# SAP/nested-hashing-psi

Measured on AMD Instinct MI355X. Metric: server PIE ciphertexts/sec, higher is better.
Workload: dtype u64

## Files before the change

### nested_hashing_psi_amd/csrc/kernels.hpp

```cpp
#pragma once
#include <hip/hip_runtime.h>

#include <atomic>
#include <vector>

#include "params.hpp"

namespace piehip {

struct PerDeviceOnce {
    std::atomic<unsigned long long> done{0};
    bool first_on_current_device()
    {
        int dev = 0;
        if (hipGetDevice(&dev) != hipSuccess || dev < 0 || dev > 63) return true;
        const unsigned long long bit = 1ULL << dev;
        return (done.fetch_or(bit) & bit) == 0;
    }
};

enum class NttKernel { radix2, blocked32, blocked16 };
struct NttRoute {
    NttKernel kernel;
    u32 s0;
    u32 global_stages;
    bool extra() const { return kernel != NttKernel::radix2 && !global_stages; }
};

struct NttPlan {
    const u64 *tables;
    const u64 *twp;
    const u64 *twc = nullptr;
    const u64 *twc_fold = nullptr;
    const u64 *twk16 = nullptr;
    const DevConsts *dc;
    u32 N, logN;
    u32 num_cus;
    u32 max_slots = 0;
    bool lane_order = false;
    bool fold = false;
    NttKernel lane_kernel = NttKernel::radix2;
    u32 lane_logn = 0;
    u32 lane_T = 0;
    u32 lane_kp = 16;
    bool small_moduli = false;
    bool xq_reuse = false;
    bool x_direct = false;
    bool fused_tensor = false;
    bool digits_with_d01 = false;
    bool digit_lift_lane = false;
    bool digit_lift_std = false;
    u32 transform_cus() const
    {
        if (!max_slots) return num_cus;
        const u32 c = (max_slots + 1) / 2;
        return c < num_cus ? (c ? c : 1u) : num_cus;
    }
};
void ntt_plan_decide(NttPlan &pl, bool lazy_ok, bool small_moduli);
NttRoute ntt_route(const NttPlan &pl, bool inverse, bool sigma, bool folded);

void build_twc_table(const u64 *nat_pairs, u32 logN, u32 s0, std::vector<u64> &out);
void build_twk16_table(const u64 *nat_pairs, u32 s0, u32 slice_log, std::vector<u64> &out);
void ntt_sigma_inverse_map(u32 logN, u32 s0, std::vector<u32> &map);
void ntt16_sigma_inverse_map(u32 logN, u32 s0, std::vector<u32> &map);
struct NttExtra {
    u64 *copy_out = nullptr;
    u32 copy_K = 1, copy_L = 1, copy_M = 1;
    u32 skip_L = 0, skip_M = 0;
    bool lazy_out = false;
    bool folded = false;
    bool x_lane_in = false;
};
void launch_ntt(const NttPlan &pl, u64 *data, u32 nlimbs, u32 mod_base, u32 mod_count, bool inverse, hipStream_t st,
                bool sigma = false, bool folded = false, const NttExtra *ex = nullptr);
void launch_ntt_fast(const NttPlan &pl, const u64 *twc, u32 s0, u64 *data, u32 nlimbs, u32 mod_base, u32 mod_count, bool inverse,
                     bool sigma, hipStream_t st, const u64 *lift_src = nullptr, u32 lift_L = 0, const NttExtra *ex = nullptr);
struct Ntt16Digits {
    const u64 *d2;
    size_t stride2;
    u64 *dig;
    u32 nb, L;
};
void launch_ntt16(const NttPlan &pl, u64 *data, u32 nlimbs, u32 mod_base, u32 mod_count, bool inverse, bool sigma, hipStream_t st,
                  const NttExtra *ex, const Ntt16Digits *dg = nullptr);
#ifndef PIEHIP_FUSE_TENSOR
#define PIEHIP_FUSE_TENSOR 1
#endif
void launch_ntt16_tensor(const NttPlan &pl, const u64 *e, u64 *d, u32 nb, u32 M, hipStream_t st);
void launch_ntt_digits(const NttPlan &pl, const u64 *d2, u64 *dig, u32 nb, u32 L, bool sigma, hipStream_t st);

struct StageAXOut {
    u64 *out = nullptr;
    u32 M = 0, logns = 0;
};
void launch_stage_a(const DevConsts *dc, u32 N, u32 L, u32 K, u32 b, u32 E, const u64 *idx, const u64 *minus,
                    const u64 *db, u64 *acc, hipStream_t st, bool small_moduli, u32 bstride = 0, u32 h0 = 0, u32 hn = 0, u32 nq = 1,
                    u32 q = 0, const StageAXOut *xo = nullptr);
static const u32 STAGE_A_MAX_QUERIES = 8;
struct StageAQueries {
    const u64 *idx[STAGE_A_MAX_QUERIES];
    const u64 *minus[STAGE_A_MAX_QUERIES];
};
void launch_stage_a_batch(const DevConsts *dc, u32 N, u32 L, u32 K, u32 b, u32 E, const StageAQueries &qs, u32 nq, const u64 *db,
                          u64 *acc, hipStream_t st, bool small_moduli, u32 bstride = 0, u32 h0 = 0, u32 hn = 0,
                          const StageAXOut *xo = nullptr);

void launch_expand_q_to_qp(const DevConsts *dc, u32 N, u32 L, const u64 *in, size_t in_stride_outer,
                           size_t in_stride_inner, u32 n_outer, u64 *out, u32 out_polys, u32 out_slot, hipStream_t st,
                           bool small_moduli, bool fold = false, bool skip_q = false);
void launch_scale_pq_expand(const DevConsts *dc, u32 N, u32 L, const u64 *in, size_t in_stride_outer,
                            size_t in_stride_inner, u32 n_outer, u64 *out, u32 out_polys, u32 out_slot, hipStream_t st,
                            bool small_moduli, bool fold = false);
void launch_expand_both(const DevConsts *dc, u32 N, u32 L, const u64 *x, size_t sx, const u64 *y, size_t sy, size_t si, u32 n_outer,
                        u64 *out, hipStream_t st, bool small_moduli, bool fold = false, bool skip_q = false);
void launch_tensor(const DevConsts *dc, u32 N, u32 M, const u64 *e, u64 *d, u32 nb, hipStream_t st, bool small_moduli);
void launch_scale_round(const DevConsts *dc, u32 N, u32 L, const u64 *d, u32 nb, u64 *out01, size_t stride01, u64 *out2,
                        size_t stride2, hipStream_t st, bool small_moduli, bool fold = false, bool fold_comp2 = false);
void launch_digits(const DevConsts *dc, u32 N, u32 L, const u64 *d2, size_t stride2, u32 nb, u64 *dig, hipStream_t st,
                   bool fold = false);
void launch_relin_mac(const DevConsts *dc, u32 N, u32 L, const u64 *d01, size_t stride01, const u64 *dig, const u64 *key,
                      const u64 *mask, u64 *out, u32 nb, hipStream_t st, bool small_moduli, const u32 *out_map = nullptr, size_t key_stride = 0,
                      u32 key_group = 1, u32 sigma_T = 0, u32 sigma_kp = 16, u32 mask_div = 1);
void launch_bcast_mul_plain(const DevConsts *dc, u32 N, u32 L, const u64 *x, size_t xs, u32 group, const u64 *pt, size_t ps_outer,
                            size_t ps_inner, u64 *out, u32 nct, hipStream_t st);
void launch_rot_prepare(const DevConsts *dc, u32 N, u32 L, const u64 *x, const u32 *maps, u32 map_group, bool acc, bool identity_first,
                        u64 *d01, u64 *d2, u32 nct, hipStream_t st);
void launch_sum_mul_plain(const DevConsts *dc, u32 N, u32 L, const u64 *x, u32 group, const u64 *pt, size_t pt_stride, u64 *out,
                          size_t out_stride, u32 ngroups, hipStream_t st);
void launch_host_flag(u64 *flag_dev, u64 value, hipStream_t st);
void launch_ct_add(const DevConsts *dc, u32 N, u32 L, const u64 *x, const u64 *y, u64 *out, u32 nct, hipStream_t st);
void launch_ct_mul_plain(const DevConsts *dc, u32 N, u32 L, const u64 *x, const u64 *pt, size_t pt_stride, u64 *out,
                         u32 nct, hipStream_t st, u32 pt_div = 1);
bool launch_limb_drop(const DevConsts *dc, u32 N, u32 L, u32 keep, const u64 *in, u64 *out, u32 npoly, hipStream_t st);
void launch_permute(u32 N, const u64 *in, const u32 *map, u64 *out, u32 nrows, hipStream_t st);
void launch_encode_scatter(const DevConsts *dc, u32 N, u32 M, const int64_t *slots, u32 B, const u32 *inv_pos, u64 *u,
                           u32 npt, hipStream_t st);
void launch_encode_lift(const DevConsts *dc, u32 N, u32 L, u32 M, const u64 *u, u64 *out, u32 npt, hipStream_t st);

size_t hash_sort_temp_bytes(u32 n, u32 e);
hipError_t launch_hash_build(const u64 *d_tab, const u64 *d_items, u32 n, u32 k, u32 e, u32 K, u32 b, u32 E, u64 evict_seed,
                             u64 shuffle_seed, u64 *d_tbl, u32 *d_keys, u32 *d_vals, u32 *d_start, void *d_temp, size_t temp_bytes,
                             u32 *d_fail, hipStream_t st);
void launch_shuffle_rows(u64 *d_tbl, u32 rows, u32 b, u32 E, u64 seed, hipStream_t st);
void launch_gather_slots(const u64 *d_tbl, u32 B, u32 K, u32 b, u32 E, u64 t, int64_t *d_slots, u32 *d_fail, hipStream_t st);
void launch_mask_slots(u64 t, u32 b, u32 B, u64 seed, int64_t *d_out, hipStream_t st);

void launch_enc_message(const DevConsts *dc, u32 N, u32 L, u32 M, const u64 *coeff_t, const int32_t *e, u64 *em, u32 nct, hipStream_t st);
void launch_enc_finish(const DevConsts *dc, u32 N, u32 L, const u64 *em, const u64 *sk, const u64 *a_in, u64 *out, u32 nct,
                       hipStream_t st);
void launch_ks_finish(const DevConsts *dc, u32 N, u32 L, const u64 *e, const u64 *sk, const u64 *s_from, u64 *ks, hipStream_t st);
void launch_square(const DevConsts *dc, u32 N, u32 L, const u64 *s, u64 *s2, hipStream_t st);
void launch_dec_dot(const DevConsts *dc, u32 N, u32 L, const u64 *ct, const u64 *sk, u64 *xs, u32 nct, hipStream_t st);
void launch_dec_round(const DevConsts *dc, u32 N, u32 L, u32 M, const u64 *xs, u64 *coeff_t, u32 nct, hipStream_t st);
void launch_decode_gather(const DevConsts *dc, u32 N, u32 M, const u64 *u, const u32 *slot_pos, u32 B, int64_t *slots, u32 nct,
                          hipStream_t st);

struct SeedJob {
    u64 *dst;
    u32 seed[8];
};
static const u32 SEED_MAX_JOBS_PER_LAUNCH = 65535;
void launch_expand_uniform(const DevConsts *dc, u32 N, u32 L, const SeedJob *jobs, u32 njobs, hipStream_t st);

}
```

### nested_hashing_psi_amd/csrc/kernels_ntt.hip

```cpp
#include "kernels.hpp"

#include <algorithm>
#include <cassert>

namespace piehip {

static const u32 NTT_LDS_MAX_LOG = 14;

struct NttArgs {
    u64 *data;
    const u64 *tables;
    const DevConsts *dc;
    u32 N, logN;
    u32 s0;
    u32 mod_base, mod_count;
};

template <bool INV>
__global__ void __launch_bounds__(1024) ntt_lds_generic(NttArgs a)
{
    extern __shared__ u64 s[];
    const u32 tid = threadIdx.x, nthr = blockDim.x;
    const u32 nl = a.N >> a.s0;
    const u32 limb = blockIdx.x >> a.s0, blk = blockIdx.x & ((1u << a.s0) - 1);
    const u32 mod = a.mod_base + limb % a.mod_count;
    const Mod m = a.dc->mod[mod];
    const u64 q = m.q, q2 = 2 * m.q;
    const u64 *tw = a.tables + (size_t)mod * 4 * a.N + (INV ? 2 * (size_t)a.N : 0);
    const u64 *tws = tw + a.N;
    u64 *g = a.data + (size_t)limb * a.N + (size_t)blk * nl;

    for (u32 i = tid; i < nl; i += nthr) s[i] = g[i];
    __syncthreads();

    if (!INV) {
        u32 logt = a.logN - a.s0 - 1;
        for (u32 ml = 1; ml < nl; ml <<= 1, logt--) {
            const u32 t = 1u << logt;
            for (u32 bi = tid; bi < nl / 2; bi += nthr) {
                const u32 i = bi >> logt, j = bi & (t - 1);
                const u32 x = (i << (logt + 1)) + j;
                const u32 k = (ml << a.s0) + blk * ml + i;
                const u64 w = tw[k], ws = tws[k];
                u64 u = s[x];
                u = u >= q2 ? u - q2 : u;
                const u64 v = mul_shoup_lazy(s[x + t], w, ws, q);
                s[x] = u + v;
                s[x + t] = u - v + q2;
            }
            __syncthreads();
        }
        for (u32 i = tid; i < nl; i += nthr) {
            u64 v = s[i];
            v = v >= q2 ? v - q2 : v;
            g[i] = v >= q ? v - q : v;
        }
    } else {
        u32 logt = 0;
        for (u32 hl = nl >> 1; hl >= 1; hl >>= 1, logt++) {
            const u32 t = 1u << logt;
            for (u32 bi = tid; bi < nl / 2; bi += nthr) {
                const u32 i = bi >> logt, j = bi & (t - 1);
                const u32 x = (i << (logt + 1)) + j;
                const u32 k = (hl << a.s0) + blk * hl + i;
                const u64 w = tw[k], ws = tws[k];
                const u64 u = s[x], v = s[x + t];
                const u64 sm = u + v;
                s[x] = sm >= q2 ? sm - q2 : sm;
                s[x + t] = mul_shoup_lazy(u - v + q2, w, ws, q);
            }
            __syncthreads();
        }
        if (a.s0 == 0) {
            for (u32 i = tid; i < nl; i += nthr) g[i] = mul_shoup(s[i], m.n_inv, m.n_inv_sh, q);
        } else {
            for (u32 i = tid; i < nl; i += nthr) {
                u64 v = s[i];
                g[i] = v >= q ? v - q : v;
            }
        }
    }
}

template <bool INV>
__global__ void __launch_bounds__(256) ntt_global_stage(NttArgs a, u32 mstage, u32 last_inverse)
{
    const u32 half = a.N >> 1;
    const u32 bi = blockIdx.x * 256 + threadIdx.x;
    const u32 limb = blockIdx.y;
    if (bi >= half) return;
    const u32 mod = a.mod_base + limb % a.mod_count;
    const Mod m = a.dc->mod[mod];
    const u64 q = m.q;
    const u64 *tw = a.tables + (size_t)mod * 4 * a.N + (INV ? 2 * (size_t)a.N : 0);
    const u64 *tws = tw + a.N;
    u32 logm = 0;
    while ((1u << logm) < mstage) logm++;
    const u32 logt = a.logN - 1 - logm, t = 1u << logt;
    const u32 i = bi >> logt, j = bi & (t - 1);
    const size_t x = (size_t)limb * a.N + ((size_t)i << (logt + 1)) + j;
    const u64 w = tw[mstage + i], ws = tws[mstage + i];
    const u64 u = a.data[x], v = a.data[x + t];
    if (!INV) {
        const u64 p = mul_shoup(v, w, ws, q);
        a.data[x] = addmod(u, p, q);
        a.data[x + t] = submod(u, p, q);
    } else {
        u64 sm = addmod(u, v, q);
        u64 df = mul_shoup(submod(u, v, q), w, ws, q);
        if (last_inverse) {
            sm = mul_shoup(sm, m.n_inv, m.n_inv_sh, q);
            df = mul_shoup(df, m.n_inv, m.n_inv_sh, q);
        }
        a.data[x] = sm;
        a.data[x + t] = df;
    }
}

static PerDeviceOnce g_attr_set[2];

NttRoute ntt_route(const NttPlan &pl, bool inverse, bool sigma, bool folded)
{
    assert((!sigma || pl.lane_order) && (!folded || pl.fold));
    const u32 s0 = pl.logN > NTT_LDS_MAX_LOG ? pl.logN - NTT_LDS_MAX_LOG : 0;
    if (!pl.lane_order) return {NttKernel::radix2, s0, s0};
    if (pl.lane_kernel == NttKernel::blocked16 && folded == pl.fold && (inverse || sigma)) return {NttKernel::blocked16, folded ? 1u : 0u, 0};
    if (folded) return {NttKernel::blocked32, 1, 0};
    return {NttKernel::blocked32, s0, s0};
}

void ntt_plan_decide(NttPlan &pl, bool lazy_ok, bool small_moduli)
{
    pl.lane_order = lazy_ok && pl.logN >= 12;
    pl.small_moduli = small_moduli;
    if (!pl.lane_order) return;
    const bool k16 = pl.logN >= 13 && pl.logN <= 15;
    pl.lane_kernel = k16 ? NttKernel::blocked16 : NttKernel::blocked32;
    pl.fold = pl.logN == 14 || pl.logN == 15;
    pl.lane_logn = pl.logN - ntt_route(pl, true, true, pl.fold).s0;
    pl.lane_T = (1u << pl.lane_logn) / (k16 ? 16 : 32);
    pl.lane_kp = k16 ? 8 : 16;
    pl.xq_reuse = ntt_route(pl, true, false, pl.fold).extra();
    pl.fused_tensor = PIEHIP_FUSE_TENSOR && k16 && small_moduli;
    pl.digits_with_d01 = k16 && small_moduli;
    pl.x_direct = pl.xq_reuse && k16 && small_moduli;
    const NttRoute std_fwd = ntt_route(pl, false, false, false);
    pl.digit_lift_std = std_fwd.kernel == NttKernel::blocked32 && std_fwd.s0 == 0;
    pl.digit_lift_lane = pl.digit_lift_std && !k16;
}

void launch_ntt_digits(const NttPlan &pl, const u64 *d2, u64 *dig, u32 nb, u32 L, bool sigma, hipStream_t st)
{
    assert(sigma ? pl.digit_lift_lane : pl.digit_lift_std);
    launch_ntt_fast(pl, pl.twc, 0, dig, nb * L * L, 0, L, false, sigma, st, d2, L);
}

void launch_ntt(const NttPlan &pl, u64 *data, u32 nlimbs, u32 mod_base, u32 mod_count, bool inverse, hipStream_t st, bool sigma,
                bool folded, const NttExtra *ex)
{
    if (!nlimbs) return;
    const NttRoute r = ntt_route(pl, inverse, sigma, folded);
    if (r.kernel == NttKernel::blocked16) {
        launch_ntt16(pl, data, nlimbs, mod_base, mod_count, inverse, sigma, st, ex);
        return;
    }
    if (folded) {
        NttExtra exf;
        if (ex) exf = *ex;
        exf.folded = true;
        launch_ntt_fast(pl, pl.twc_fold, 1, data, nlimbs, mod_base, mod_count, inverse, sigma, st, nullptr, 0, &exf);
        return;
    }
    NttArgs a;
    a.data = data;
    a.tables = pl.tables;
    a.dc = pl.dc;
    a.N = pl.N;
    a.logN = pl.logN;
    a.s0 = r.s0;
    a.mod_base = mod_base;
    a.mod_count = mod_count;
    const u32 nl = pl.N >> a.s0;
    const size_t lds = (size_t)nl * sizeof(u64);
    const u32 threads = std::min(std::max(nl / 2, 64u), 1024u);
    const bool radix2 = r.kernel == NttKernel::radix2;
    if (radix2 && g_attr_set[inverse ? 1 : 0].first_on_current_device())
        (void)hipFuncSetAttribute(inverse ? (const void *)ntt_lds_generic<true> : (const void *)ntt_lds_generic<false>,
                                  hipFuncAttributeMaxDynamicSharedMemorySize, (1 << NTT_LDS_MAX_LOG) * 8);
    const dim3 ggrid((pl.N / 2 + 255) / 256, nlimbs);
    if (!inverse) {
        for (u32 ms = 1; ms < (1u << r.global_stages); ms <<= 1)
            hipLaunchKernelGGL(ntt_global_stage<false>, ggrid, dim3(256), 0, st, a, ms, 0u);
        if (radix2) hipLaunchKernelGGL(ntt_lds_generic<false>, dim3(nlimbs << a.s0), dim3(threads), lds, st, a);
    } else if (radix2) {
        hipLaunchKernelGGL(ntt_lds_generic<true>, dim3(nlimbs << a.s0), dim3(threads), lds, st, a);
    }
    if (!radix2) launch_ntt_fast(pl, pl.twc, r.s0, data, nlimbs, mod_base, mod_count, inverse, sigma, st, nullptr, 0, ex);
    if (inverse)
        for (u32 ms = (1u << r.global_stages) >> 1; ms >= 1; ms >>= 1)
            hipLaunchKernelGGL(ntt_global_stage<true>, ggrid, dim3(256), 0, st, a, ms, ms == 1 ? 1u : 0u);
}

}
```

### nested_hashing_psi_amd/csrc/kernels_ntt16.hip

```cpp
#include <cassert>

#include "kernels.hpp"
#include "ntt16_kernel.h"

namespace piehip {

void build_twk16_table(const u64 *nat_pairs, u32 s0, u32 slice_log, std::vector<u64> &out)
{
    if (slice_log == 14)
        ntt16::build_twk_table_t<14>(nat_pairs, s0, out);
    else
        ntt16::build_twk_table_t<13>(nat_pairs, s0, out);
}

void ntt16_sigma_inverse_map(u32 logN, u32 s0, std::vector<u32> &map)
{
    const u32 N = 1u << logN, n = N >> s0;
    map.resize(N);
    for (u32 p = 0; p < N; p++) map[p] = (p / n) * n + ntt16::lane_to_std_t(p % n, n / 16);
}

template <u32 LOGNS>
static void launch_ntt16_t(const ntt16::Args &a, bool inverse, bool lift, u32 num_cus, hipStream_t st, bool tensor = false)
{
    typedef ntt16::Geo<LOGNS> G;
    constexpr size_t lds = (size_t)G::LDS_WORDS * sizeof(u64);
    static PerDeviceOnce attr[4];
    if (attr[tensor ? 3 : inverse ? 1 : (lift ? 2 : 0)].first_on_current_device()) {
        if (tensor)
            (void)hipFuncSetAttribute((const void *)ntt16::ntt16_kernel_t<LOGNS, true, false, true>, hipFuncAttributeMaxDynamicSharedMemorySize, (int)lds);
        else if (inverse)
            (void)hipFuncSetAttribute((const void *)ntt16::ntt16_kernel_t<LOGNS, true>, hipFuncAttributeMaxDynamicSharedMemorySize, (int)lds);
        else if (lift)
            (void)hipFuncSetAttribute((const void *)ntt16::ntt16_kernel_t<LOGNS, false, true>, hipFuncAttributeMaxDynamicSharedMemorySize, (int)lds);
        else
            (void)hipFuncSetAttribute((const void *)ntt16::ntt16_kernel_t<LOGNS, false>, hipFuncAttributeMaxDynamicSharedMemorySize, (int)lds);
    }
    const u32 slots = (LOGNS == 13 ? 2u : 1u) * num_cus;
    const u32 grid = a.nitems < slots ? a.nitems : slots;
    if (tensor)
        hipLaunchKernelGGL((ntt16::ntt16_kernel_t<LOGNS, true, false, true>), dim3(grid), dim3(G::T), lds, st, a);
    else if (inverse)
        hipLaunchKernelGGL((ntt16::ntt16_kernel_t<LOGNS, true>), dim3(grid), dim3(G::T), lds, st, a);
    else if (lift)
        hipLaunchKernelGGL((ntt16::ntt16_kernel_t<LOGNS, false, true>), dim3(grid), dim3(G::T), lds, st, a);
    else
        hipLaunchKernelGGL((ntt16::ntt16_kernel_t<LOGNS, false>), dim3(grid), dim3(G::T), lds, st, a);
}

void launch_ntt16(const NttPlan &pl, u64 *data, u32 nlimbs, u32 mod_base, u32 mod_count, bool inverse, bool sigma, hipStream_t st,
                  const NttExtra *ex, const Ntt16Digits *dg)
{
    const bool folded = pl.fold;
    const u32 s0 = folded ? 1u : 0u;
    assert(ntt_route(pl, inverse, sigma, folded).kernel == NttKernel::blocked16 && (!dg || pl.digits_with_d01));
    ntt16::Args a;
    a.data = data;
    a.twp = reinterpret_cast<const ntt16::u64x2 *>(pl.twp);
    a.twk = reinterpret_cast<const ntt16::u64x2 *>(pl.twk16);
    a.dc = pl.dc;
    a.N = pl.N;
    a.s0 = s0;
    a.nitems = nlimbs << s0;
    a.mod_base = mod_base;
    a.mod_count = mod_count;
    a.flags = 0;
    if (inverse && !sigma) a.flags |= ntt16::F_STD_IN;
    if (inverse && folded) a.flags |= ntt16::F_FOLDED;
    if (inverse && !sigma && ex && ex->copy_out && ex->x_lane_in) a.flags |= ntt16::F_X_LANE_IN;
    if (!inverse && ex && ex->lazy_out) a.flags |= ntt16::F_LAZY_OUT;
    a.skip_L = (ex && !inverse) ? ex->skip_L : 0;
    a.skip_M = ex ? ex->skip_M : 0;
    a.copy_out = (ex && inverse && !sigma) ? ex->copy_out : nullptr;
    a.copy_K = ex ? ex->copy_K : 1;
    a.copy_L = ex ? ex->copy_L : 1;
    a.copy_M = ex ? ex->copy_M : 1;
    a.lift_first = ~0u;
    a.data2 = nullptr;
    a.lift_src = nullptr;
    a.lift_stride = 0;
    a.lift_L = 1;
    a.tsrc = nullptr;
    if (dg && !inverse) {
        a.lift_first = a.nitems;
        a.nitems += (dg->nb * dg->L * dg->L) << s0;
        a.data2 = dg->dig;
        a.lift_src = dg->d2;
        a.lift_stride = dg->stride2;
        a.lift_L = dg->L;
    }
    const bool lift = a.lift_first != ~0u;
    if (pl.lane_logn == 14)
        launch_ntt16_t<14>(a, inverse, lift, pl.transform_cus(), st);
    else
        launch_ntt16_t<13>(a, inverse, lift, pl.transform_cus(), st);
}

void launch_ntt16_tensor(const NttPlan &pl, const u64 *e, u64 *d, u32 nb, u32 M, hipStream_t st)
{
    assert(pl.fused_tensor);
    const bool folded = pl.fold;
    const u32 s0 = folded ? 1u : 0u;
    ntt16::Args a = {};
    a.data = d;
    a.twp = reinterpret_cast<const ntt16::u64x2 *>(pl.twp);
    a.twk = reinterpret_cast<const ntt16::u64x2 *>(pl.twk16);
    a.dc = pl.dc;
    a.N = pl.N;
    a.s0 = s0;
    a.nitems = (nb * 3 * M) << s0;
    a.mod_base = 0;
    a.mod_count = M;
    a.flags = folded ? ntt16::F_FOLDED : 0;
    a.copy_K = a.copy_L = a.copy_M = 1;
    a.lift_first = ~0u;
    a.lift_L = 1;
    a.tsrc = e;
    if (pl.lane_logn == 14)
        launch_ntt16_t<14>(a, true, false, pl.transform_cus(), st, true);
    else
        launch_ntt16_t<13>(a, true, false, pl.transform_cus(), st, true);
}

}
```

### nested_hashing_psi_amd/csrc/kernels_pie.hip

```cpp
#include <stdlib.h>

#include <algorithm>

#include "kernels.hpp"
#include "madasm.h"

namespace piehip {

static const u32 TPB = 256;

typedef u64 u64x2 __attribute__((ext_vector_type(2)));

struct StageATile {
    u32 bx, l, hz, grp;
};
__device__ __forceinline__ bool stage_a_tile(u32 nx, u32 L, u32 tiles, u32 groups, StageATile &t)
{
    const u32 id = blockIdx.x, xcd = id & 7, slot = id >> 3;
    t.grp = slot % groups;
    const u32 tile = (slot / groups) * 8 + xcd;
    if (tile >= tiles) return false;
    t.bx = tile % nx;
    t.l = (tile / nx) % L;
    t.hz = tile / (nx * L);
    return true;
}
static dim3 stage_a_grid(u32 nx, u32 L, u32 hn, u32 groups) { return dim3(8 * ((nx * L * hn + 7) / 8) * groups); }

template <int BPT>
__global__ void __launch_bounds__(TPB) stage_a_kernel(const DevConsts *__restrict__ dc, u32 N, u32 L, u32 K, u32 b, u32 E,
                                                      const u64 *__restrict__ idx, const u64 *__restrict__ minus,
                                                      const u64 *__restrict__ db, u64 *__restrict__ acc, u32 bstride, u32 h0,
                                                      u32 nq, u32 q)
{
    const u32 n = 2 * (blockIdx.x * TPB + threadIdx.x);
    const u32 l = blockIdx.y;
    const u32 groups = b / BPT;
    const u32 h = h0 + blockIdx.z / groups, beta0 = (blockIdx.z % groups) * BPT;
    if (n >= N) return;
    const Mod m = dc->mod[l];
    const size_t LN = (size_t)L * N;
    const u64 *pi = idx + ((size_t)h * E) * 2 * LN + (size_t)l * N + n;
    const u64 *pd = db + (((size_t)h * bstride + beta0) * E) * LN + (size_t)l * N + n;
    const size_t bin_stride = (size_t)E * LN;
    U128 a[BPT][2][2];
#pragma unroll
    for (int t = 0; t < BPT; t++)
#pragma unroll
        for (int c = 0; c < 2; c++) a[t][c][0] = a[t][c][1] = U128{0, 0};
    for (u32 j = 0; j < E; j++) {
        const u64x2 i0 = *reinterpret_cast<const u64x2 *>(pi + (size_t)j * 2 * LN);
        const u64x2 i1 = *reinterpret_cast<const u64x2 *>(pi + (size_t)j * 2 * LN + LN);
        u64x2 d[BPT];
#pragma unroll
        for (int t = 0; t < BPT; t++) {
            typedef u64 u64v2 __attribute__((ext_vector_type(2)));
            const u64v2 v = __builtin_nontemporal_load(reinterpret_cast<const u64v2 *>(pd + (size_t)t * bin_stride + (size_t)j * LN));
            d[t].x = v.x, d[t].y = v.y;
        }
#pragma unroll
        for (int t = 0; t < BPT; t++) {
            mac128(a[t][0][0], i0.x, d[t].x);
            mac128(a[t][0][1], i0.y, d[t].y);
            mac128(a[t][1][0], i1.x, d[t].x);
            mac128(a[t][1][1], i1.y, d[t].y);
        }
        if ((j & 31) == 31) {
#pragma unroll
            for (int t = 0; t < BPT; t++)
#pragma unroll
                for (int c = 0; c < 2; c++)
#pragma unroll
                    for (int e = 0; e < 2; e++) a[t][c][e] = U128{reduce128(a[t][c][e], m), 0};
        }
    }
    const u64x2 m0 = *reinterpret_cast<const u64x2 *>(minus + (size_t)l * N + n);
    const u64x2 m1 = *reinterpret_cast<const u64x2 *>(minus + LN + (size_t)l * N + n);
#pragma unroll
    for (int t = 0; t < BPT; t++) {
        u64 *po = acc + ((((size_t)(beta0 + t) * nq + q) * K + h) * 2) * LN + (size_t)l * N + n;
        u64x2 r0, r1;
        r0.x = addmod(reduce128(a[t][0][0], m), m0.x, m.q);
        r0.y = addmod(reduce128(a[t][0][1], m), m0.y, m.q);
        r1.x = addmod(reduce128(a[t][1][0], m), m1.x, m.q);
        r1.y = addmod(reduce128(a[t][1][1], m), m1.y, m.q);
        *reinterpret_cast<u64x2 *>(po) = r0;
        *reinterpret_cast<u64x2 *>(po + LN) = r1;
    }
}

__device__ __forceinline__ u32 lane_home(u32 n, u32 logns)
{
    const u32 ns = 1u << logns, e = n & (ns - 1);
    return (n & ~(ns - 1)) + 2 * ((ns >> 4) * ((e >> 1) & 7) + (e >> 4)) + (e & 1);
}

__device__ __forceinline__ u64 addmod_nb(u64 a, u64 b, u64 q)
{
    const u64 s = a + b;
    u32 lo, hi;
    asm("v_lshl_add_u64 v[60:61], %[x], 0, %[nm]\n\t"
        "v_ashrrev_i32 v62, 31, v61\n\t"
        "v_bfi_b32 %[lo], v62, %[xl], v60\n\t"
        "v_bfi_b32 %[hi], v62, %[xh], v61"
        : [lo] "=&v"(lo), [hi] "=&v"(hi)
        : [x] "v"(s), [xl] "v"((u32)s), [xh] "v"((u32)(s >> 32)), [nm] "s"(0 - q)
        : "v62", "v60", "v61");
    return ((u64)hi << 32) | lo;
}

static const int SA_DEPTH = 4;
template <bool W124>
__device__ __forceinline__ u64 colacc_reduce(const ColAcc &a, const Mod &m, u64 nq);
__device__ __forceinline__ u64 colacc_reduce123_lazy(const ColAcc &a, const Mod &m, u64 nq);
template <int BPT>
__global__ void __launch_bounds__(TPB) stage_a_mad_kernel(const DevConsts *__restrict__ dc, u32 N, u32 L, u32 K, u32 b, u32 E,
                                                          const u64 *__restrict__ idx, const u64 *__restrict__ minus,
                                                          const u64 *__restrict__ db, u64 *__restrict__ acc, u32 bstride, u32 h0,
                                                          u32 nq, u32 q, StageAXOut xo)
{
    const u32 nl = threadIdx.x;
    const u32 n = blockIdx.x * TPB + nl;
    const u32 l = blockIdx.y;
    const u32 groups = b / BPT;
    const u32 h = h0 + blockIdx.z / groups, beta0 = (blockIdx.z % groups) * BPT;
    if (n >= N) return;
    const Mod m = dc->mod[l];
    const size_t LN = (size_t)L * N;
    const u64 *pi = idx + ((size_t)h * E) * 2 * LN + (size_t)l * N + blockIdx.x * TPB;
    const u64 *pd = db + (((size_t)h * bstride + beta0) * E) * LN + (size_t)l * N + blockIdx.x * TPB;
    const size_t bin_stride = (size_t)E * LN;
    ColAcc a[BPT][2];
#pragma unroll
    for (int t = 0; t < BPT; t++) a[t][0] = a[t][1] = ColAcc{0, 0, 0};
    auto load_term = [&](u32 j, u64 (&vi)[2], u64 (&vd)[BPT]) {
        const u64 *pij = pi + (size_t)j * 2 * LN, *pdj = pd + (size_t)j * LN;
        vi[0] = pij[nl];
        vi[1] = (pij + LN)[nl];
#pragma unroll
        for (int t = 0; t < BPT; t++) vd[t] = __builtin_nontemporal_load(pdj + (size_t)t * bin_stride + nl);
    };
    u64 qiv[SA_DEPTH][2], qdv[SA_DEPTH][BPT];
#pragma unroll
    for (int d = 0; d < SA_DEPTH; d++)
        if ((u32)d < E) load_term(d, qiv[d], qdv[d]);
    auto term = [&](u32 j, u64 (&vi)[2], u64 (&vd)[BPT]) {
        const Split30 i0 = split30(vi[0]), i1 = split30(vi[1]);
#pragma unroll
        for (int t = 0; t < BPT; t++) colacc_mac2(a[t][0], a[t][1], i0, i1, vd[t]);
        if (j + SA_DEPTH < E) load_term(j + SA_DEPTH, vi, vd);
        if ((j % COLACC_MAX_TERMS) == COLACC_MAX_TERMS - 1 && j + 1 < E) {
#pragma unroll
            for (int t = 0; t < BPT; t++) colacc_carry(a[t][0]), colacc_carry(a[t][1]);
        }
        if ((j % COLACC_MAX_TOTAL) == COLACC_MAX_TOTAL - 1 && j + 1 < E) {
#pragma unroll
            for (int t = 0; t < BPT; t++)
#pragma unroll
                for (int c = 0; c < 2; c++) {
                    const u64 r = reduce124(colacc_value(a[t][c]), m);
                    a[t][c] = ColAcc{r & 0x3FFFFFFFull, r >> 30, 0};
                }
        }
    };
    for (u32 j = 0; j < E; j += SA_DEPTH) {
#pragma unroll
        for (int d = 0; d < SA_DEPTH; d++)
            if (j + d < E) term(j + d, qiv[d], qdv[d]);
    }
    const bool xdir = h == 0 && xo.out != nullptr;
    const u32 noff = n + ((xdir ? ~0u : 0u) & (lane_home(n, xo.logns) - n));
#pragma unroll
    for (int t = 0; t < BPT; t++) {
        const size_t row = (size_t)(beta0 + t) * nq + q;
        u64 *const base = xdir ? xo.out + ((row * 4) * xo.M + l) * N : acc + ((row * K + h) * 2) * LN + (size_t)l * N;
        const size_t cstride = xdir ? (size_t)xo.M * N : LN;
        u64 *const po = base + noff;
#pragma unroll
        for (int c = 0; c < 2; c++)
            po[(size_t)c * cstride] = addmod_nb(colacc_reduce<true>(a[t][c], m, 0 - m.q), minus[(size_t)c * LN + (size_t)l * N + n], m.q);
    }
}

template <int BPT, int Q, int DEPTH>
__global__ void __launch_bounds__(TPB) stage_a_mad_batch_kernel(const DevConsts *__restrict__ dc, u32 N, u32 L, u32 K, u32 b, u32 E,
                                                                StageAQueries qs, const u64 *__restrict__ db, u64 *__restrict__ acc,
                                                                u32 bstride, u32 h0, u32 nq, u32 q0, u32 tiles, StageAXOut xo)
{
    StageATile tl;
    if (!stage_a_tile((N + TPB - 1) / TPB, L, tiles, (b + BPT - 1) / BPT, tl)) return;
    const u32 nl = threadIdx.x, n0 = tl.bx * TPB, l = tl.l, h = h0 + tl.hz, beta0 = tl.grp * BPT;
    const u32 n = n0 + nl;
    if (n >= N) return;
    const u32 tmax = __builtin_amdgcn_readfirstlane(min((u32)BPT, b - beta0) - 1);
    const Mod m = dc->mod[l];
    const size_t LN = (size_t)L * N;
    const size_t ioff = ((size_t)h * E) * 2 * LN + (size_t)l * N + n0;
    const u64 *pd = db + (((size_t)h * bstride + beta0) * E) * LN + (size_t)l * N + n0;
    const size_t bin_stride = (size_t)E * LN;
    ColAcc a[Q][BPT][2];
#pragma unroll
    for (int q = 0; q < Q; q++)
#pragma unroll
        for (int t = 0; t < BPT; t++) a[q][t][0] = a[q][t][1] = ColAcc{0, 0, 0};
    auto load_term = [&](u32 j, u64 (&vi)[Q][2], u64 (&vd)[BPT]) {
#pragma unroll
        for (int q = 0; q < Q; q++) {
            const u64 *pij = qs.idx[q] + ioff + (size_t)j * 2 * LN;
            vi[q][0] = pij[nl];
            vi[q][1] = (pij + LN)[nl];
        }
        const u64 *pdj = pd + (size_t)j * LN;
#pragma unroll
        for (int t = 0; t < BPT; t++) vd[t] = __builtin_nontemporal_load(pdj + (size_t)min((u32)t, tmax) * bin_stride + nl);
    };
    u64 qiv[DEPTH][Q][2], qdv[DEPTH][BPT];
#pragma unroll
    for (int d = 0; d < DEPTH; d++)
        if ((u32)d < E) load_term(d, qiv[d], qdv[d]);
    auto term = [&](u32 j, u64 (&vi)[Q][2], u64 (&vd)[BPT]) {
#pragma unroll
        for (int q = 0; q < Q; q++) {
            const Split30 i0 = split30(vi[q][0]), i1 = split30(vi[q][1]);
#pragma unroll
            for (int t = 0; t < BPT; t++) colacc_mac2(a[q][t][0], a[q][t][1], i0, i1, vd[t]);
        }
        if (j + DEPTH < E) load_term(j + DEPTH, vi, vd);
        if ((j % COLACC_MAX_TERMS) == COLACC_MAX_TERMS - 1 && j + 1 < E) {
#pragma unroll
            for (int q = 0; q < Q; q++)
#pragma unroll
                for (int t = 0; t < BPT; t++) colacc_carry(a[q][t][0]), colacc_carry(a[q][t][1]);
        }
        if ((j % COLACC_MAX_TOTAL) == COLACC_MAX_TOTAL - 1 && j + 1 < E) {
#pragma unroll
            for (int q = 0; q < Q; q++)
#pragma unroll
                for (int t = 0; t < BPT; t++)
#pragma unroll
                    for (int c = 0; c < 2; c++) {
                        const u64 r = colacc_reduce<true>(a[q][t][c], m, 0 - m.q);
                        a[q][t][c] = ColAcc{r & 0x3FFFFFFFull, r >> 30, 0};
                    }
        }
    };
    for (u32 j = 0; j < E; j += DEPTH) {
#pragma unroll
        for (int d = 0; d < DEPTH; d++)
            if (j + d < E) term(j + d, qiv[d], qdv[d]);
    }
    const bool xdir = h == 0 && xo.out != nullptr;
    const u32 noff = n + ((xdir ? ~0u : 0u) & (lane_home(n, xo.logns) - n));
#pragma unroll
    for (int q = 0; q < Q; q++) {
        u64 mi[2];
#pragma unroll
        for (int c = 0; c < 2; c++) mi[c] = qs.minus[q][(size_t)c * LN + (size_t)l * N + n];
#pragma unroll
        for (int t = 0; t < BPT; t++) {
            if ((u32)t > tmax) continue;
            const size_t row = (size_t)(beta0 + t) * nq + q0 + q;
            u64 *const base = xdir ? xo.out + ((row * 4) * xo.M + l) * N : acc + ((row * K + h) * 2) * LN + (size_t)l * N;
            const size_t cstride = xdir ? (size_t)xo.M * N : LN;
            u64 *const po = base + noff;
#pragma unroll
            for (int c = 0; c < 2; c++) po[(size_t)c * cstride] = addmod_nb(colacc_reduce<true>(a[q][t][c], m, 0 - m.q), mi[c], m.q);
        }
    }
}

static void launch_stage_a_uniform(const DevConsts *dc, u32 N, u32 L, u32 K, u32 b, u32 E, const u64 *idx, const u64 *minus,
                                   const u64 *db, u64 *acc, hipStream_t st, bool mad, u32 bstride, u32 h0, u32 hn, int bpt, u32 nq,
                                   u32 q, StageAXOut xo)
{
    const int cpt = mad ? 1 : 2;
    dim3 grid((N / cpt + TPB - 1) / TPB, L, hn * (b / bpt));
#define SA(B_)                                                                                                       \
    do {                                                                                                             \
        if (mad) hipLaunchKernelGGL(stage_a_mad_kernel<B_>, grid, dim3(TPB), 0, st, dc, N, L, K, b, E, idx, minus, db, acc, bstride, h0, nq, q, xo); \
        else hipLaunchKernelGGL(stage_a_kernel<B_>, grid, dim3(TPB), 0, st, dc, N, L, K, b, E, idx, minus, db, acc, bstride, h0, nq, q);  \
    } while (0)
    switch (bpt) {
        case 8: hipLaunchKernelGGL(stage_a_kernel<8>, grid, dim3(TPB), 0, st, dc, N, L, K, b, E, idx, minus, db, acc, bstride, h0, nq, q); break;
        case 7: SA(7); break;
        case 6: SA(6); break;
        case 5: SA(5); break;
        case 4: SA(4); break;
        case 3: SA(3); break;
        case 2: SA(2); break;
        default: SA(1); break;
    }
#undef SA
}

void launch_stage_a(const DevConsts *dc, u32 N, u32 L, u32 K, u32 b, u32 E, const u64 *idx, const u64 *minus,
                    const u64 *db, u64 *acc, hipStream_t st, bool small_moduli, u32 bstride, u32 h0, u32 hn, u32 nq, u32 q,
                    const StageAXOut *xop)
{
    StageAXOut xo;
    if (xop && small_moduli) xo = *xop;
    if (!bstride) bstride = b;
    if (!hn) hn = K - h0;
    if (!nq) nq = 1;
    const bool mad = small_moduli;
    const u32 cap = mad ? 7 : 8;
    u32 bpt = 0;
    for (u32 c = cap; c >= 4; c--)
        if (b % c == 0) {
            bpt = c;
            break;
        }
    if (b <= cap) bpt = b;
    const size_t LN = (size_t)L * N;
    if (bpt) {
        launch_stage_a_uniform(dc, N, L, K, b, E, idx, minus, db, acc, st, mad, bstride, h0, hn, (int)bpt, nq, q, xo);
        return;
    }
    const u32 full = (b / cap) * cap, rest = b - full;
    launch_stage_a_uniform(dc, N, L, K, full, E, idx, minus, db, acc, st, mad, bstride, h0, hn, (int)cap, nq, q, xo);
    StageAXOut xr = xo;
    if (xr.out) xr.out += (size_t)full * nq * 4 * xr.M * N;
    launch_stage_a_uniform(dc, N, L, K, rest, E, idx, minus, db + (size_t)full * E * LN, acc + (size_t)full * nq * K * 2 * LN, st, mad,
                           bstride, h0, hn, (int)rest, nq, q, xr);
}

template <int Q, int BPT>
static void launch_stage_a_batch_qb(const DevConsts *dc, u32 N, u32 L, u32 K, u32 nb, u32 E, const StageAQueries &qs, const u64 *db,
                                    u64 *acc, hipStream_t st, u32 bstride, u32 h0, u32 hn, u32 nq, u32 q0, StageAXOut xo)
{
    const u32 nx = (N + TPB - 1) / TPB;
    constexpr int DEPTH = (Q == 4 || Q * BPT >= 9) ? 2 : 3;
    hipLaunchKernelGGL((stage_a_mad_batch_kernel<BPT, Q, DEPTH>), stage_a_grid(nx, L, hn, (nb + BPT - 1) / BPT), dim3(TPB), 0, st, dc, N, L, K,
                       nb, E, qs, db, acc, bstride, h0, nq, q0, nx * L * hn, xo);
}
template <int Q>
static void launch_stage_a_batch_q(const DevConsts *dc, u32 N, u32 L, u32 K, u32 b, u32 E, const StageAQueries &qs, const u64 *db,
                                   u64 *acc, hipStream_t st, u32 bstride, u32 h0, u32 hn, u32 nq, u32 q0, StageAXOut xo)
{
    constexpr u32 cap = Q == 2 ? 4 : 3;
    u32 bpt = 1, best = ~0u;
    for (u32 g = 1; g <= cap && g <= b; g++) {
        const u32 loads = ((b + g - 1) / g) * (2 * Q + g);
        if (loads <= best) best = loads, bpt = g;
    }
    if constexpr (cap >= 4)
        if (bpt == 4) return launch_stage_a_batch_qb<Q, 4>(dc, N, L, K, b, E, qs, db, acc, st, bstride, h0, hn, nq, q0, xo);
    if constexpr (cap >= 3)
        if (bpt == 3) return launch_stage_a_batch_qb<Q, 3>(dc, N, L, K, b, E, qs, db, acc, st, bstride, h0, hn, nq, q0, xo);
    if (bpt == 2) return launch_stage_a_batch_qb<Q, 2>(dc, N, L, K, b, E, qs, db, acc, st, bstride, h0, hn, nq, q0, xo);
    return launch_stage_a_batch_qb<Q, 1>(dc, N, L, K, b, E, qs, db, acc, st, bstride, h0, hn, nq, q0, xo);
}
void launch_stage_a_batch(const DevConsts *dc, u32 N, u32 L, u32 K, u32 b, u32 E, const StageAQueries &qs, u32 nq, const u64 *db,
                          u64 *acc, hipStream_t st, bool small_moduli, u32 bstride, u32 h0, u32 hn, const StageAXOut *xop)
{
    StageAXOut xo;
    if (xop && small_moduli) xo = *xop;
    if (!bstride) bstride = b;
    if (!hn) hn = K - h0;
    u32 q0 = 0;
    while (small_moduli && nq - q0 >= 2) {
        const u32 left = nq - q0, g = left == 5 || left == 6 ? 3 : std::min(left, 4u);
        StageAQueries sub = {};
        for (u32 q = 0; q < g; q++) sub.idx[q] = qs.idx[q0 + q], sub.minus[q] = qs.minus[q0 + q];
        if (g == 2) launch_stage_a_batch_q<2>(dc, N, L, K, b, E, sub, db, acc, st, bstride, h0, hn, nq, q0, xo);
        else if (g == 3) launch_stage_a_batch_q<3>(dc, N, L, K, b, E, sub, db, acc, st, bstride, h0, hn, nq, q0, xo);
        else launch_stage_a_batch_q<4>(dc, N, L, K, b, E, sub, db, acc, st, bstride, h0, hn, nq, q0, xo);
        q0 += g;
    }
    for (; q0 < nq; q0++)
        launch_stage_a(dc, N, L, K, b, E, qs.idx[q0], qs.minus[q0], db, acc, st, small_moduli, bstride, h0, hn, nq, q0, xop);
}

#define PIE_ITER_FENCE() __builtin_amdgcn_sched_barrier(0)
typedef const __attribute__((address_space(4))) DevConsts *DcC;
__device__ __forceinline__ DcC dc_iter(const DevConsts *dc)
{
    u64 v = (u64)dc;
    asm volatile("" : "+s"(v));
    return (DcC)v;
}
__device__ __forceinline__ Mod ld_mod(DcC c, u32 i)
{
    Mod m;
    m.q = c->mod[i].q, m.r0 = c->mod[i].r0, m.r1 = c->mod[i].r1, m.n_inv = 0, m.n_inv_sh = 0;
    m.fconst = c->mod[i].fconst, m.fshift = c->mod[i].fshift, m.pad = 0;
    return m;
}

__device__ __forceinline__ u64 neg_u(u64 m)
{
    u64 n = 0 - m;
    asm("" : "+s"(n));
    return n;
}
__device__ __forceinline__ u64 sel_neg(u64 x, u64 t, u32 &mask)
{
    u32 lo, hi, k;
    asm("v_ashrrev_i32 %[k], 31, %[th]\n\t"
        "v_bfi_b32 %[lo], %[k], %[xl], %[tl]\n\t"
        "v_bfi_b32 %[hi], %[k], %[xh], %[th]"
        : [lo] "=&v"(lo), [hi] "=&v"(hi), [k] "=&v"(k)
        : [xl] "v"((u32)x), [xh] "v"((u32)(x >> 32)), [tl] "v"((u32)t), [th] "v"((u32)(t >> 32)));
    mask = k;
    return ((u64)hi << 32) | lo;
}
__device__ __forceinline__ u64 csub_u(u64 x, u64 negm)
{
    u32 k;
    return sel_neg(x, x + negm, k);
}
__device__ __forceinline__ u64 mul_shoup_lazy_u(u64 a, u64 w, u64 wsh, u64 q) { return a * w - mulhi(a, wsh) * q; }
__device__ __forceinline__ u64 mul_shoup_u(u64 a, u64 w, u64 wsh, u64 q, u64 negq) { return csub_u(mul_shoup_lazy_u(a, w, wsh, q), negq); }
__device__ __forceinline__ u64 fixfrac_u(u64 y, const Mod &m) { return mulhi(y << m.fshift, m.fconst) >> 3; }
__device__ __forceinline__ void divmod_shoup_u(u64 a, u64 w, u64 wsh, u64 q, u64 negq, u64 &quot, u64 &rem)
{
    const u64 qe = mulhi(a, wsh);
    const u64 r = a * w - qe * q;
    u32 k;
    rem = sel_neg(r, r + negq, k);
    quot = qe + 1 + (u64)(int64_t)(int32_t)k;
}
__device__ __forceinline__ u64 reduce123_u(U128 z, const Mod &m, u64 negq, u64 neg2q)
{
    const u64 mu = (m.r1 << 59) | (m.r0 >> 5);
    const u64 zh = (z.hi << 5) | (z.lo >> 59);
    const u64 qhat = mulhi(zh, mu);
    return csub_u(csub_u(z.lo - qhat * m.q, neg2q), negq);
}

#define PIE_ASM_CLOB "vcc", "v60", "v61", "v62", "v63", "v64", "v65", "v66", "v67", "v68", "v69", "v70", "v71"
#define PIE_SHOUP63_HEAD                                        \
    "v_mad_u64_u32 v[60:61], vcc, %[al], %[sh], 0\n\t"          \
    "v_mad_u64_u32 v[64:65], vcc, %[al], %[wl], 0\n\t"          \
    "v_mad_u64_u32 v[60:61], vcc, %[ah], %[sl], v[60:61]\n\t"   \
    "v_mad_u64_u32 v[66:67], vcc, %[al], %[wh], 0\n\t"          \
    "v_lshlrev_b32 v70, 1, %[ah]\n\t"                           \
    "v_mad_u64_u32 v[66:67], vcc, %[ah], %[wl], v[66:67]\n\t"   \
    "v_lshrrev_b64 v[60:61], 31, v[60:61]\n\t"                  \
    "v_mad_u64_u32 v[62:63], vcc, v70, %[sh], v[60:61]\n\t"     \
    "v_mad_u64_u32 v[66:67], vcc, v62, %[nqh], v[66:67]\n\t"    \
    "v_mad_u64_u32 v[66:67], vcc, v63, %[nql], v[66:67]\n\t"    \
    "v_add_u32 v65, v65, v66\n\t"
#define PIE_SHOUP63_IN(a, w, wsh, nq)                                                                                        \
    [al] "v"((u32)(a)), [ah] "v"((u32)((a) >> 32)), [wl] "s"((u32)(w)), [wh] "s"((u32)((w) >> 32)), [sl] "s"((u32)((wsh) >> 1)), \
        [sh] "s"((u32)((wsh) >> 33)), [nql] "s"((u32)(nq)), [nqh] "s"((u32)((nq) >> 32))
__device__ __forceinline__ u64 shoup63_lazy(u64 a, u64 w, u64 wsh, u64 nq)
{
    u64 r;
    asm(PIE_SHOUP63_HEAD
        "v_mad_u64_u32 %[r], vcc, v62, %[nql], v[64:65]"
        : [r] "=v"(r)
        : PIE_SHOUP63_IN(a, w, wsh, nq)
        : PIE_ASM_CLOB);
    return r;
}
__device__ __forceinline__ u64 shoup63(u64 a, u64 w, u64 wsh, u64 nq)
{
    u32 lo, hi;
    const u64 n2q = 2 * nq;
    asm(PIE_SHOUP63_HEAD
        "v_mad_u64_u32 v[64:65], vcc, v62, %[nql], v[64:65]\n\t"
        "v_lshl_add_u64 v[68:69], v[64:65], 0, %[n2q]\n\t"
        "v_ashrrev_i32 v71, 31, v69\n\t"
        "v_bfi_b32 v64, v71, v64, v68\n\t"
        "v_bfi_b32 v65, v71, v65, v69\n\t"
        "v_lshl_add_u64 v[68:69], v[64:65], 0, %[n1q]\n\t"
        "v_ashrrev_i32 v71, 31, v69\n\t"
        "v_bfi_b32 %[lo], v71, v64, v68\n\t"
        "v_bfi_b32 %[hi], v71, v65, v69"
        : [lo] "=v"(lo), [hi] "=v"(hi)
        : PIE_SHOUP63_IN(a, w, wsh, nq), [n2q] "s"(n2q), [n1q] "s"(nq)
        : PIE_ASM_CLOB);
    return ((u64)hi << 32) | lo;
}
__device__ __forceinline__ void divmod63(u64 a, u64 w, u64 wsh, u64 nq, u64 &quot, u64 &rem)
{
    u32 lo, hi;
    u64 qt;
    const u64 n2q = 2 * nq;
    asm(PIE_SHOUP63_HEAD
        "v_mad_u64_u32 v[64:65], vcc, v62, %[nql], v[64:65]\n\t"
        "v_lshl_add_u64 v[68:69], v[64:65], 0, %[n2q]\n\t"
        "v_ashrrev_i64 v[60:61], 63, v[68:69]\n\t"
        "v_bfi_b32 v64, v60, v64, v68\n\t"
        "v_bfi_b32 v65, v60, v65, v69\n\t"
        "v_lshl_add_u64 v[62:63], v[60:61], 1, v[62:63]\n\t"
        "v_lshl_add_u64 v[68:69], v[64:65], 0, %[n1q]\n\t"
        "v_ashrrev_i64 v[60:61], 63, v[68:69]\n\t"
        "v_bfi_b32 %[lo], v60, v64, v68\n\t"
        "v_bfi_b32 %[hi], v60, v65, v69\n\t"
        "v_lshl_add_u64 v[62:63], v[60:61], 0, v[62:63]\n\t"
        "v_lshl_add_u64 %[qt], v[62:63], 0, 3"
        : [lo] "=v"(lo), [hi] "=v"(hi), [qt] "=v"(qt)
        : PIE_SHOUP63_IN(a, w, wsh, nq), [n2q] "s"(n2q), [n1q] "s"(nq)
        : PIE_ASM_CLOB);
    quot = qt;
    rem = ((u64)hi << 32) | lo;
}
__device__ __forceinline__ u64 mulhi_sb(u64 a, u64 b)
{
    u64 r;
    asm("v_mul_hi_u32 v60, %[al], %[bl]\n\t"
        "v_mov_b32 v61, 0\n\t"
        "v_mad_u64_u32 v[62:63], vcc, %[al], %[bh], v[60:61]\n\t"
        "v_mad_u64_u32 v[62:63], vcc, %[ah], %[bl], v[62:63]\n\t"
        "v_mad_u64_u32 v[66:67], s[96:97], %[ah], %[bh], 0\n\t"
        "v_lshrrev_b64 v[64:65], 32, v[62:63]\n\t"
        "v_addc_co_u32 v65, vcc, 0, v65, vcc\n\t"
        "v_lshl_add_u64 %[r], v[66:67], 0, v[64:65]"
        : [r] "=v"(r)
        : [al] "v"((u32)a), [ah] "v"((u32)(a >> 32)), [bl] "s"((u32)b), [bh] "s"((u32)(b >> 32))
        : PIE_ASM_CLOB, "s96", "s97");
    return r;
}
#define PIE_COLACC123_TO_4Q \
    "v_lshrrev_b64 v[60:61], 30, %[c0]\n\t" \
    "v_lshl_add_u64 v[60:61], v[60:61], 0, %[c1]\n\t" \
    "v_lshrrev_b64 v[62:63], 30, v[60:61]\n\t" \
    "v_lshl_add_u64 v[62:63], v[62:63], 0, %[c2]\n\t" \
    "v_lshlrev_b64 v[64:65], 1, v[62:63]\n\t" \
    "v_bfe_u32 v68, v60, 29, 1\n\t" \
    "v_and_b32 v66, 0x3fffffff, %[c0l]\n\t" \
    "v_bfe_u32 v67, v60, 2, 28\n\t" \
    "v_or_b32 v64, v64, v68\n\t" \
    "v_lshl_or_b32 v66, v60, 30, v66\n\t" \
    "v_lshl_or_b32 v67, v62, 28, v67\n\t" \
    "v_mul_hi_u32 v68, v64, %[mul]\n\t" \
    "v_mov_b32 v69, 0\n\t" \
    "v_mad_u64_u32 v[68:69], vcc, v64, %[muh], v[68:69]\n\t" \
    "v_mad_u64_u32 v[68:69], vcc, v65, %[mul], v[68:69]\n\t" \
    "v_mad_u64_u32 v[70:71], s[96:97], v65, %[muh], 0\n\t" \
    "v_lshrrev_b64 v[68:69], 32, v[68:69]\n\t" \
    "v_addc_co_u32 v69, vcc, 0, v69, vcc\n\t" \
    "v_lshl_add_u64 v[68:69], v[70:71], 0, v[68:69]\n\t" \
    "v_mad_u64_u32 v[70:71], vcc, v68, %[nqh], 0\n\t" \
    "v_mad_u64_u32 v[70:71], vcc, v69, %[nql], v[70:71]\n\t" \
    "v_add_u32 v67, v67, v70\n\t" \
    "v_mad_u64_u32 v[66:67], vcc, v68, %[nql], v[66:67]\n\t"
__device__ __forceinline__ u64 colacc_reduce123_lazy(const ColAcc &a, const Mod &m, u64 nq)
{
    const u64 mu = (m.r1 << 59) | (m.r0 >> 5);
    u64 r;
    asm(PIE_COLACC123_TO_4Q
        "v_lshl_add_u64 %[r], v[66:67], 0, 0"
        : [r] "=v"(r)
        : [c0] "v"(a.c0), [c1] "v"(a.c1), [c2] "v"(a.c2), [c0l] "v"((u32)a.c0), [mul] "s"((u32)mu), [muh] "s"((u32)(mu >> 32)),
          [nql] "s"((u32)nq), [nqh] "s"((u32)(nq >> 32))
        : PIE_ASM_CLOB, "s96", "s97");
    return r;
}
template <bool W124>
__device__ __forceinline__ u64 colacc_reduce(const ColAcc &a, const Mod &m, u64 nq)
{
    const u64 mu = (m.r1 << 59) | (m.r0 >> 5);
    const u64 n2q = 2 * nq, n4q = 4 * nq;
    u64 r;
    if (!W124) {
        asm(PIE_COLACC123_TO_4Q
            "v_lshl_add_u64 v[60:61], v[66:67], 0, %[n2q]\n\t"
            "v_ashrrev_i32 v62, 31, v61\n\t"
            "v_bfi_b32 v66, v62, v66, v60\n\t"
            "v_bfi_b32 v67, v62, v67, v61\n\t"
            "v_lshl_add_u64 v[60:61], v[66:67], 0, %[n1q]\n\t"
            "v_ashrrev_i32 v62, 31, v61\n\t"
            "v_and_b32 v64, %[ql], v62\n\t"
            "v_and_b32 v65, %[qh], v62\n\t"
            "v_lshl_add_u64 %[r], v[60:61], 0, v[64:65]"
            : [r] "=v"(r)
            : [c0] "v"(a.c0), [c1] "v"(a.c1), [c2] "v"(a.c2), [c0l] "v"((u32)a.c0), [mul] "s"((u32)mu), [muh] "s"((u32)(mu >> 32)),
              [nql] "s"((u32)nq), [nqh] "s"((u32)(nq >> 32)), [n2q] "s"(n2q), [n1q] "s"(nq), [ql] "s"((u32)m.q), [qh] "s"((u32)(m.q >> 32))
            : PIE_ASM_CLOB, "s96", "s97");
    } else {
        asm("v_lshrrev_b64 v[60:61], 30, %[c0]\n\t"
            "v_lshl_add_u64 v[60:61], v[60:61], 0, %[c1]\n\t"
            "v_lshrrev_b64 v[64:65], 30, v[60:61]\n\t"
            "v_lshl_add_u64 v[64:65], v[64:65], 0, %[c2]\n\t"
            "v_and_b32 v66, 0x3fffffff, %[c0l]\n\t"
            "v_bfe_u32 v67, v60, 2, 28\n\t"
            "v_lshl_or_b32 v66, v60, 30, v66\n\t"
            "v_lshl_or_b32 v67, v64, 28, v67\n\t"
            "v_mul_hi_u32 v68, v64, %[mul]\n\t"
            "v_mov_b32 v69, 0\n\t"
            "v_mad_u64_u32 v[68:69], vcc, v64, %[muh], v[68:69]\n\t"
            "v_mad_u64_u32 v[68:69], vcc, v65, %[mul], v[68:69]\n\t"
            "v_mad_u64_u32 v[70:71], s[96:97], v65, %[muh], 0\n\t"
            "v_lshrrev_b64 v[68:69], 32, v[68:69]\n\t"
            "v_addc_co_u32 v69, vcc, 0, v69, vcc\n\t"
            "v_lshl_add_u64 v[68:69], v[70:71], 0, v[68:69]\n\t"
            "v_lshlrev_b64 v[68:69], 1, v[68:69]\n\t"
            "v_mad_u64_u32 v[70:71], vcc, v68, %[nqh], 0\n\t"
            "v_mad_u64_u32 v[70:71], vcc, v69, %[nql], v[70:71]\n\t"
            "v_add_u32 v67, v67, v70\n\t"
            "v_mad_u64_u32 v[66:67], vcc, v68, %[nql], v[66:67]\n\t"
            "v_lshl_add_u64 v[60:61], v[66:67], 0, %[n4q]\n\t"
            "v_ashrrev_i32 v62, 31, v61\n\t"
            "v_bfi_b32 v66, v62, v66, v60\n\t"
            "v_bfi_b32 v67, v62, v67, v61\n\t"
            "v_lshl_add_u64 v[60:61], v[66:67], 0, %[n2q]\n\t"
            "v_ashrrev_i32 v62, 31, v61\n\t"
            "v_bfi_b32 v66, v62, v66, v60\n\t"
            "v_bfi_b32 v67, v62, v67, v61\n\t"
            "v_lshl_add_u64 v[60:61], v[66:67], 0, %[n1q]\n\t"
            "v_ashrrev_i32 v62, 31, v61\n\t"
            "v_and_b32 v64, %[ql], v62\n\t"
            "v_and_b32 v65, %[qh], v62\n\t"
            "v_lshl_add_u64 %[r], v[60:61], 0, v[64:65]"
            : [r] "=v"(r)
            : [c0] "v"(a.c0), [c1] "v"(a.c1), [c2] "v"(a.c2), [c0l] "v"((u32)a.c0), [mul] "s"((u32)mu), [muh] "s"((u32)(mu >> 32)),
              [nql] "s"((u32)nq), [nqh] "s"((u32)(nq >> 32)), [n4q] "s"(n4q), [n2q] "s"(n2q), [n1q] "s"(nq), [ql] "s"((u32)m.q),
              [qh] "s"((u32)(m.q >> 32))
            : PIE_ASM_CLOB, "s96", "s97");
    }
    return r;
}
__device__ __forceinline__ void colacc_mac_small(ColAcc &a, u32 v, u64 c)
{
    const Split30 s = split30(c);
    a.c0 = mad_u(v, s.lo, a.c0);
    a.c1 = mad_u(v, s.hi, a.c1);
}

template <bool ASM>
__device__ __forceinline__ u64 mshoup(u64 a, u64 w, u64 wsh, u64 q, u64 negq)
{
    return ASM ? shoup63(a, w, wsh, negq) : mul_shoup_u(a, w, wsh, q, negq);
}
template <bool ASM>
__device__ __forceinline__ void mdivmod(u64 a, u64 w, u64 wsh, u64 q, u64 negq, u64 &quot, u64 &rem)
{
    if (ASM)
        divmod63(a, w, wsh, negq, quot, rem);
    else
        divmod_shoup_u(a, w, wsh, q, negq, quot, rem);
}
template <bool ASM>
__device__ __forceinline__ u64 mfixfrac(u64 y, const Mod &m)
{
    return ASM ? (mulhi_sb(y << m.fshift, m.fconst) >> 3) : fixfrac_u(y, m);
}

template <u32 NS, bool MAD>
__device__ __forceinline__ U128 dot128(const u64 *y, const u64 (&c)[NS])
{
    if (MAD) {
        ColAcc a = {0, 0, 0};
#pragma unroll
        for (u32 i = 0; i < NS; i++) colacc_mac(a, split30(y[i]), split30(c[i]));
        return colacc_value(a);
    }
    U128 acc = {0, 0};
#pragma unroll
    for (u32 i = 0; i < NS; i++) mac128(acc, y[i], c[i]);
    return acc;
}

template <u32 NS, bool MAD, bool LZ = false>
__device__ __forceinline__ u64 crt_out(const u64 *y, const u64 (&hat)[NS], u64 v, u64 prodmod, const Mod &tm, u64 negq, u64 neg2q)
{
    if (MAD && NS <= 7) {
        ColAcc a = {0, 0, 0};
#pragma unroll
        for (u32 i = 0; i < NS; i++) colacc_mac(a, split30(y[i]), split30(hat[i]));
        colacc_mac_small(a, (u32)v, tm.q - prodmod);
        return LZ ? colacc_reduce123_lazy(a, tm, negq) : colacc_reduce<false>(a, tm, negq);
    }
    U128 acc = dot128<NS, MAD>(y, hat);
    mac128(acc, v, tm.q - prodmod);
    return reduce128(acc, tm);
}

__device__ __forceinline__ void fold_load(const DevConsts *dc, u32 a, u64 u, u64 v, u64 &x0, u64 &x1)
{
    PIE_ITER_FENCE();
    const DcC c = dc_iter(dc);
    const u64 q = c->mod[a].q, nq = neg_u(q);
    x0 = shoup63(u + v, c->fold_ia[a], c->fold_ia_sh[a], nq);
    x1 = shoup63(u + (4 * q - v), c->fold_ib[a], c->fold_ib_sh[a], nq);
}
__device__ __forceinline__ void fold_store(const DevConsts *dc, u32 a, u64 u, u64 v, u64 &y0, u64 &y1)
{
    const DcC c = dc_iter(dc);
    const u64 q = c->mod[a].q;
    const u64 t = shoup63_lazy(v, c->fold_w[a], c->fold_w_sh[a], neg_u(q));
    y0 = u + t;
    y1 = u + (4 * q - t);
}

template <u32 L, bool MAD, bool YIN, int NP, bool LZ = false>
__device__ __forceinline__ void expand_core(const DevConsts *dc, const u64 (&x)[NP][L], u64 (&out)[NP][2 * L + 1])
{
    constexpr u32 Lp = L + 1;
    u64 y[NP][L];
    u64 fsum[NP];
#pragma unroll
    for (int p = 0; p < NP; p++) fsum[p] = 0;
#pragma unroll
    for (u32 i = 0; i < L; i++) {
        PIE_ITER_FENCE();
        const DcC c = dc_iter(dc);
        const Mod mi = ld_mod(c, i);
        const u64 w = c->qhat_inv[i], wsh = c->qhat_inv_sh[i], nq = neg_u(mi.q);
#pragma unroll
        for (int p = 0; p < NP; p++) {
            out[p][i] = x[p][i];
            y[p][i] = YIN ? x[p][i] : mshoup<MAD>(x[p][i], w, wsh, mi.q, nq);
            fsum[p] += mfixfrac<MAD>(y[p][i], mi);
        }
    }
#pragma unroll
    for (u32 j = 0; j < Lp; j++) {
        PIE_ITER_FENCE();
        const DcC c = dc_iter(dc);
        const Mod pj = ld_mod(c, L + j);
        u64 hat[L];
#pragma unroll
        for (u32 i = 0; i < L; i++) hat[i] = c->qhat_modp[i][j];
        const u64 prodmod = c->Q_modp[j], nq = neg_u(pj.q), n2q = neg_u(2 * pj.q);
#pragma unroll
        for (int p = 0; p < NP; p++) out[p][L + j] = crt_out<L, MAD, LZ>(y[p], hat, (fsum[p] + FIX_HALF) >> 60, prodmod, pj, nq, n2q);
    }
}

template <u32 L, bool MAD, bool YIN, int NP, bool LZ = false>
__device__ __forceinline__ void scale_pq_core(const DevConsts *dc, const u64 (&x)[NP][L], u64 (&out)[NP][2 * L + 1])
{
    constexpr u32 Lp = L + 1;
    u64 y[NP][L];
    u64 fsum[NP];
    U128 itot[NP];
#pragma unroll
    for (int p = 0; p < NP; p++) fsum[p] = 0, itot[p] = U128{0, 0};
#pragma unroll
    for (u32 i = 0; i < L; i++) {
        PIE_ITER_FENCE();
        const DcC c = dc_iter(dc);
        const Mod mi = ld_mod(c, i);
        const u64 w = c->qhat_inv[i], wsh = c->qhat_inv_sh[i], pw = c->P_modq[i], pwsh = c->P_modq_sh[i], nq = neg_u(mi.q);
#pragma unroll
        for (int p = 0; p < NP; p++) {
            y[p][i] = YIN ? x[p][i] : mshoup<MAD>(x[p][i], w, wsh, mi.q, nq);
            u64 fl, z;
            mdivmod<MAD>(y[p][i], pw, pwsh, mi.q, nq, fl, z);
            add128(itot[p], U128{fl, 0});
            fsum[p] += mfixfrac<MAD>(z, mi);
        }
    }
    u64 yp[NP][Lp];
    u64 fs2[NP];
#pragma unroll
    for (int p = 0; p < NP; p++) {
        add128(itot[p], U128{(fsum[p] + FIX_HALF) >> 60, 0});
        fs2[p] = 0;
    }
#pragma unroll
    for (u32 j = 0; j < Lp; j++) {
        PIE_ITER_FENCE();
        const DcC c = dc_iter(dc);
        const Mod pj = ld_mod(c, L + j);
        u64 col[L];
#pragma unroll
        for (u32 i = 0; i < L; i++) col[i] = c->PI_modp[i][j];
        const u64 w = c->phat_inv[j], wsh = c->phat_inv_sh[j], nq = neg_u(pj.q);
#pragma unroll
        for (int p = 0; p < NP; p++) {
            u64 r;
            if (MAD) {
                ColAcc a = {itot[p].lo, 0, 0};
#pragma unroll
                for (u32 i = 0; i < L; i++) colacc_mac(a, split30(y[p][i]), split30(col[i]));
                r = LZ ? colacc_reduce123_lazy(a, pj, nq) : colacc_reduce<false>(a, pj, nq);
            } else {
                U128 acc = dot128<L, MAD>(y[p], col);
                add128(acc, itot[p]);
                r = reduce128(acc, pj);
            }
            out[p][L + j] = r;
            yp[p][j] = mshoup<MAD>(r, w, wsh, pj.q, nq);
            fs2[p] += mfixfrac<MAD>(yp[p][j], pj);
        }
    }
#pragma unroll
    for (u32 i = 0; i < L; i++) {
        PIE_ITER_FENCE();
        const DcC c = dc_iter(dc);
        const Mod mi = ld_mod(c, i);
        u64 hat[Lp];
#pragma unroll
        for (u32 j = 0; j < Lp; j++) hat[j] = c->phat_modq[j][i];
        const u64 prodmod = c->P_modq[i], nq = neg_u(mi.q), n2q = neg_u(2 * mi.q);
#pragma unroll
        for (int p = 0; p < NP; p++) out[p][i] = crt_out<Lp, MAD, LZ>(yp[p], hat, (fs2[p] + FIX_HALF) >> 60, prodmod, mi, nq, n2q);
    }
}

template <bool SCALE, bool FOLD, u32 L, bool MAD, bool SKIPQ>
__device__ __forceinline__ void expand_body(const DevConsts *__restrict__ dc, u32 N, const u64 *__restrict__ in, size_t so, size_t si,
                                            u64 *__restrict__ out, u32 out_polys, u32 out_slot, u32 by)
{
    constexpr bool YIN = FOLD && (SCALE || SKIPQ);
    const u32 n = blockIdx.x * TPB + threadIdx.x;
    const u32 H = N / 2;
    if (n >= (FOLD ? H : N)) return;
    const u32 o = by >> 1, c = by & 1;
    constexpr u32 M = 2 * L + 1;
    const u64 *pin = in + (size_t)o * so + (size_t)c * si + n;
    u64 *pout = out + ((size_t)(o * out_polys + out_slot + c) * M) * N + n;
    constexpr int NP = FOLD ? 2 : 1;
    u64 x[NP][L], y[NP][M];
#pragma unroll
    for (u32 i = 0; i < L; i++) {
        if (YIN) {
            PIE_ITER_FENCE();
            const DcC c = dc_iter(dc);
            const u64 q = c->mod[i].q, nq = neg_u(q), u = pin[(size_t)i * N], v = pin[(size_t)i * N + H];
            x[0][i] = shoup63(u + v, c->fold_iaq[i], c->fold_iaq_sh[i], nq);
            x[NP - 1][i] = shoup63(u + (4 * q - v), c->fold_ibq[i], c->fold_ibq_sh[i], nq);
        } else if (FOLD) {
            fold_load(dc, i, pin[(size_t)i * N], pin[(size_t)i * N + H], x[0][i], x[NP - 1][i]);
        } else {
            x[0][i] = pin[(size_t)i * N];
        }
    }
    constexpr bool LZ = FOLD && MAD;
    if (SCALE)
        scale_pq_core<L, MAD, YIN, NP, LZ>(dc, x, y);
    else
        expand_core<L, MAD, YIN, NP, LZ>(dc, x, y);
#pragma unroll
    for (u32 a = 0; a < M; a++) {
        if (!SCALE && a < L && SKIPQ) continue;
        PIE_ITER_FENCE();
        if (FOLD) {
            u64 y0, y1;
            fold_store(dc, a, y[0][a], y[NP - 1][a], y0, y1);
            pout[(size_t)a * N] = y0;
            pout[(size_t)a * N + H] = y1;
        } else {
            pout[(size_t)a * N] = y[0][a];
        }
    }
}

template <bool SCALE, bool FOLD, u32 L, bool MAD, bool SKIPQ>
__global__ void __launch_bounds__(TPB) expand_kernel(const DevConsts *__restrict__ dc, u32 N, const u64 *__restrict__ in,
                                                     size_t so, size_t si, u64 *__restrict__ out, u32 out_polys, u32 out_slot)
{
    expand_body<SCALE, FOLD, L, MAD, SKIPQ>(dc, N, in, so, si, out, out_polys, out_slot, blockIdx.y);
}
template <bool FOLD, u32 L, bool MAD, bool SKIPQ>
__global__ void __launch_bounds__(TPB) expand_both_kernel(const DevConsts *__restrict__ dc, u32 N, const u64 *__restrict__ x, size_t sx,
                                                          const u64 *__restrict__ y, size_t sy, size_t si, u64 *__restrict__ out,
                                                          u32 n_outer)
{
    if (blockIdx.y < 2 * n_outer)
        expand_body<true, FOLD, L, MAD, false>(dc, N, y, sy, si, out, 4, 2, blockIdx.y);
    else
        expand_body<false, FOLD, L, MAD, SKIPQ>(dc, N, x, sx, si, out, 4, 0, blockIdx.y - 2 * n_outer);
}
void launch_expand_both(const DevConsts *dc, u32 N, u32 L, const u64 *x, size_t sx, const u64 *y, size_t sy, size_t si, u32 n_outer,
                        u64 *out, hipStream_t st, bool small_moduli, bool fold, bool skip_q)
{
    dim3 grid(((fold ? N / 2 : N) + TPB - 1) / TPB, n_outer * 4);
#define EB(F_, L_, M_, Q_) hipLaunchKernelGGL((expand_both_kernel<F_, L_, M_, Q_>), grid, dim3(TPB), 0, st, dc, N, x, sx, y, sy, si, out, n_outer)
#define EBL(L_)                                                                          \
    case L_:                                                                             \
        if (fold && small_moduli) { if (skip_q) EB(true, L_, true, true); else EB(true, L_, true, false); }      \
        else if (fold) { if (skip_q) EB(true, L_, false, true); else EB(true, L_, false, false); }                 \
        else if (small_moduli) { if (skip_q) EB(false, L_, true, true); else EB(false, L_, true, false); }       \
        else { if (skip_q) EB(false, L_, false, true); else EB(false, L_, false, false); }                         \
        break;
    switch (L) { EBL(1) EBL(2) EBL(3) EBL(4) EBL(5) EBL(6) EBL(7) }
#undef EBL
#undef EB
}

static void launch_expand_common(bool scale, bool fold, const DevConsts *dc, u32 N, u32 L, const u64 *in, size_t so, size_t si,
                                 u32 n_outer, u64 *out, u32 out_polys, u32 out_slot, hipStream_t st, bool small_moduli, bool skip_q = false)
{
    dim3 grid(((fold ? N / 2 : N) + TPB - 1) / TPB, n_outer * 2);
#define EX(S_, F_, L_, Q_)                                                                                                    \
    do {                                                                                                                      \
        if (small_moduli)                                                                                                   \
            hipLaunchKernelGGL((expand_kernel<S_, F_, L_, true, Q_>), grid, dim3(TPB), 0, st, dc, N, in, so, si, out, out_polys, out_slot); \
        else                                                                                                                  \
            hipLaunchKernelGGL((expand_kernel<S_, F_, L_, false, Q_>), grid, dim3(TPB), 0, st, dc, N, in, so, si, out, out_polys, out_slot); \
    } while (0)
#define EXL(L_)                                                         \
    case L_:                                                            \
        if (scale) {                                                    \
            if (fold) EX(true, true, L_, false); else EX(true, false, L_, false); \
        } else if (skip_q) {                                            \
            if (fold) EX(false, true, L_, true); else EX(false, false, L_, true); \
        } else {                                                        \
            if (fold) EX(false, true, L_, false); else EX(false, false, L_, false); \
        }                                                               \
        break;
    switch (L) { EXL(1) EXL(2) EXL(3) EXL(4) EXL(5) EXL(6) EXL(7) }
#undef EXL
#undef EX
}
void launch_expand_q_to_qp(const DevConsts *dc, u32 N, u32 L, const u64 *in, size_t so, size_t si, u32 n_outer, u64 *out,
                           u32 out_polys, u32 out_slot, hipStream_t st, bool small_moduli, bool fold, bool skip_q)
{
    launch_expand_common(false, fold, dc, N, L, in, so, si, n_outer, out, out_polys, out_slot, st, small_moduli, skip_q);
}
void launch_scale_pq_expand(const DevConsts *dc, u32 N, u32 L, const u64 *in, size_t so, size_t si, u32 n_outer, u64 *out,
                            u32 out_polys, u32 out_slot, hipStream_t st, bool small_moduli, bool fold)
{
    launch_expand_common(true, fold, dc, N, L, in, so, si, n_outer, out, out_polys, out_slot, st, small_moduli);
}

template <bool MAD>
__global__ void __launch_bounds__(TPB) tensor_kernel(const DevConsts *dc, u32 N, u32 M, const u64 *__restrict__ e,
                                                     u64 *__restrict__ d)
{
    const u32 n = 2 * (blockIdx.x * TPB + threadIdx.x);
    if (n >= N) return;
    const u32 a = blockIdx.y, bin = blockIdx.z;
    const Mod m = dc->mod[a];
    const size_t MN = (size_t)M * N;
    const u64 *pe = e + (size_t)bin * 4 * MN + (size_t)a * N + n;
    u64 *pd = d + (size_t)bin * 3 * MN + (size_t)a * N + n;
    const u64x2 va0 = *reinterpret_cast<const u64x2 *>(pe), va1 = *reinterpret_cast<const u64x2 *>(pe + MN),
                vb0 = *reinterpret_cast<const u64x2 *>(pe + 2 * MN), vb1 = *reinterpret_cast<const u64x2 *>(pe + 3 * MN);
    u64x2 r0, r1, r2;
#pragma unroll
    for (int k = 0; k < 2; k++) {
        u64 a0 = k ? va0.y : va0.x, a1 = k ? va1.y : va1.x, b0 = k ? vb0.y : vb0.x, b1 = k ? vb1.y : vb1.x;
        u64 d0, d1, d2;
        if (MAD) {
            const u64 nq = neg_u(m.q), n2q = neg_u(2 * m.q), n4q = neg_u(4 * m.q);
            a0 = csub_u(csub_u(a0, n4q), n2q), a1 = csub_u(csub_u(a1, n4q), n2q);
            b0 = csub_u(csub_u(b0, n4q), n2q), b1 = csub_u(csub_u(b1, n4q), n2q);
            const Split30 sa0 = split30(a0), sa1 = split30(a1), sb0 = split30(b0), sb1 = split30(b1);
            ColAcc c = {0, 0, 0};
            colacc_mac(c, sa0, sb0);
            d0 = colacc_reduce<false>(c, m, nq);
            c = ColAcc{0, 0, 0};
            colacc_mac(c, sa0, sb1);
            colacc_mac(c, sa1, sb0);
            d1 = colacc_reduce<false>(c, m, nq);
            c = ColAcc{0, 0, 0};
            colacc_mac(c, sa1, sb1);
            d2 = colacc_reduce<false>(c, m, nq);
        } else {
            d0 = mulmod(a0, b0, m);
            U128 x = mul128(a0, b1);
            mac128(x, a1, b0);
            d1 = reduce128(x, m);
            d2 = mulmod(a1, b1, m);
        }
        if (k) r0.y = d0, r1.y = d1, r2.y = d2;
        else r0.x = d0, r1.x = d1, r2.x = d2;
    }
    *reinterpret_cast<u64x2 *>(pd) = r0;
    *reinterpret_cast<u64x2 *>(pd + MN) = r1;
    *reinterpret_cast<u64x2 *>(pd + 2 * MN) = r2;
}
void launch_tensor(const DevConsts *dc, u32 N, u32 M, const u64 *e, u64 *d, u32 nb, hipStream_t st, bool small_moduli)
{
    dim3 grid((N / 2 + TPB - 1) / TPB, M, nb);
    if (small_moduli)
        hipLaunchKernelGGL(tensor_kernel<true>, grid, dim3(TPB), 0, st, dc, N, M, e, d);
    else
        hipLaunchKernelGGL(tensor_kernel<false>, grid, dim3(TPB), 0, st, dc, N, M, e, d);
}

template <u32 L, bool MAD, int NP, bool PRE = false>
__device__ __forceinline__ void scale_round_core(const DevConsts *dc, const u64 (&d)[NP][2 * L + 1], u64 (&out)[NP][L], bool lz = false)
{
    constexpr u32 Lp = L + 1;
    u64 yp[NP][Lp];
    u64 fsum[NP];
    U128 itot[NP];
#pragma unroll
    for (int p = 0; p < NP; p++) fsum[p] = 0, itot[p] = U128{0, 0};
#pragma unroll
    for (u32 j = 0; j < Lp; j++) {
        PIE_ITER_FENCE();
        const DcC c = dc_iter(dc);
        const Mod pj = ld_mod(c, L + j);
        const u64 w = c->qp_hat_inv[L + j], wsh = c->qp_hat_inv_sh[L + j], tw = c->tQ_modp[j], twsh = c->tQ_modp_sh[j], nq = neg_u(pj.q);
#pragma unroll
        for (int p = 0; p < NP; p++) {
            yp[p][j] = PRE ? d[p][L + j] : mshoup<MAD>(d[p][L + j], w, wsh, pj.q, nq);
            u64 fl, z;
            mdivmod<MAD>(yp[p][j], tw, twsh, pj.q, nq, fl, z);
            add128(itot[p], U128{fl, 0});
            fsum[p] += mfixfrac<MAD>(z, pj);
        }
    }
#pragma unroll
    for (int p = 0; p < NP; p++) add128(itot[p], U128{(fsum[p] + FIX_HALF) >> 60, 0});
#pragma unroll
    for (u32 k = 0; k < L; k++) {
        PIE_ITER_FENCE();
        const DcC c = dc_iter(dc);
        const Mod qk = ld_mod(c, k);
        u64 col[Lp];
#pragma unroll
        for (u32 j = 0; j < Lp; j++) col[j] = c->tQF_modq[j][k];
        const u64 tp = c->tPinv_modq[k], nq = neg_u(qk.q);
#pragma unroll
        for (int p = 0; p < NP; p++) {
            if (MAD && L <= 6) {
                ColAcc a = {itot[p].lo, 0, 0};
#pragma unroll
                for (u32 j = 0; j < Lp; j++) colacc_mac(a, split30(yp[p][j]), split30(col[j]));
                if (PRE)
                    a.c0 += d[p][k];
                else
                    colacc_mac(a, split30(d[p][k]), split30(tp));
                out[p][k] = (L <= 5 && lz) ? colacc_reduce123_lazy(a, qk, nq) : colacc_reduce<(L > 5)>(a, qk, nq);
            } else {
                U128 acc = dot128<Lp, MAD>(yp[p], col);
                if (PRE)
                    add128(acc, U128{d[p][k], 0});
                else
                    mac128(acc, d[p][k], tp);
                add128(acc, itot[p]);
                out[p][k] = reduce128(acc, qk);
            }
        }
    }
}

template <bool FOLD, u32 L, bool MAD>
__global__ void __launch_bounds__(TPB) scale_round_kernel(const DevConsts *__restrict__ dc, u32 N, const u64 *__restrict__ d,
                                                          u64 *__restrict__ out01, size_t stride01,
                                                          u64 *__restrict__ out2, size_t stride2, u32 fold_comp2)
{
    const u32 n = blockIdx.x * TPB + threadIdx.x;
    const u32 H = N / 2;
    if (n >= (FOLD ? H : N)) return;
    const u32 comp = blockIdx.y, bin = blockIdx.z;
    constexpr u32 M = 2 * L + 1;
    const u64 *pin = d + ((size_t)(bin * 3 + comp) * M) * N + n;
    u64 *pout = comp < 2 ? out01 + (size_t)bin * stride01 + (size_t)comp * L * N + n : out2 + (size_t)bin * stride2 + n;
    constexpr int NP = FOLD ? 2 : 1;
    u64 x[NP][M], y[NP][L];
#pragma unroll
    for (u32 a = 0; a < M; a++) {
        if (FOLD) {
            PIE_ITER_FENCE();
            const DcC c = dc_iter(dc);
            const u32 ak = a < L ? a : 0, aj = a < L ? 0 : a - L;
            const u64 q = c->mod[a].q, nq = neg_u(q), u = pin[(size_t)a * N], v = pin[(size_t)a * N + H];
            const u64 wa = a < L ? c->fold_iat[ak] : c->fold_iap[aj], was = a < L ? c->fold_iat_sh[ak] : c->fold_iap_sh[aj];
            const u64 wb = a < L ? c->fold_ibt[ak] : c->fold_ibp[aj], wbs = a < L ? c->fold_ibt_sh[ak] : c->fold_ibp_sh[aj];
            x[0][a] = shoup63(u + v, wa, was, nq);
            x[NP - 1][a] = shoup63(u + (4 * q - v), wb, wbs, nq);
        } else {
            x[0][a] = pin[(size_t)a * N];
        }
    }
    scale_round_core<L, MAD, NP, FOLD>(dc, x, y, FOLD && MAD && comp < 2 && !fold_comp2);
#pragma unroll
    for (u32 k = 0; k < L; k++) {
        PIE_ITER_FENCE();
        if (FOLD) {
            u64 y0 = y[0][k], y1 = y[NP - 1][k];
            if (comp < 2 || fold_comp2) fold_store(dc, k, y[0][k], y[NP - 1][k], y0, y1);
            pout[(size_t)k * N] = y0;
            pout[(size_t)k * N + H] = y1;
        } else {
            pout[(size_t)k * N] = y[0][k];
        }
    }
}
void launch_scale_round(const DevConsts *dc, u32 N, u32 L, const u64 *d, u32 nb, u64 *out01, size_t stride01, u64 *out2,
                        size_t stride2, hipStream_t st, bool small_moduli, bool fold, bool fold_comp2)
{
    dim3 grid(((fold ? N / 2 : N) + TPB - 1) / TPB, 3, nb);
#define SRL(L_)                                                                                                              \
    case L_:                                                                                                                 \
        if (fold && small_moduli)                                                                                          \
            hipLaunchKernelGGL((scale_round_kernel<true, L_, true>), grid, dim3(TPB), 0, st, dc, N, d, out01, stride01, out2, stride2, \
                               fold_comp2 ? 1u : 0u);                                                                        \
        else if (fold)                                                                                                       \
            hipLaunchKernelGGL((scale_round_kernel<true, L_, false>), grid, dim3(TPB), 0, st, dc, N, d, out01, stride01, out2, stride2, \
                               fold_comp2 ? 1u : 0u);                                                                        \
        else if (small_moduli)                                                                                             \
            hipLaunchKernelGGL((scale_round_kernel<false, L_, true>), grid, dim3(TPB), 0, st, dc, N, d, out01, stride01, out2, stride2, 0u); \
        else                                                                                                                 \
            hipLaunchKernelGGL((scale_round_kernel<false, L_, false>), grid, dim3(TPB), 0, st, dc, N, d, out01, stride01, out2, stride2, 0u); \
        break;
    switch (L) { SRL(1) SRL(2) SRL(3) SRL(4) SRL(5) SRL(6) SRL(7) }
#undef SRL
}

__device__ __forceinline__ u64 digit_lift(const DevConsts *dc, u32 i, u32 j, u64 v)
{
    const Mod &mj = dc->mod[j];
    const u64 qi = dc->mod[i].q;
    u64 r = (qi < 2 * mj.q) ? (v >= mj.q ? v - mj.q : v) : barrett128(0, v, mj);
    if (v > qi / 2) r = submod(r, dc->qi_modqj[i][j], mj.q);
    return r;
}
template <bool FOLD>
__global__ void __launch_bounds__(TPB) digits_kernel(const DevConsts *__restrict__ dc, u32 N, u32 L, const u64 *__restrict__ d2,
                                                     size_t stride2, u64 *__restrict__ dig)
{
    const u32 n = blockIdx.x * TPB + threadIdx.x;
    const u32 H = N / 2;
    if (n >= (FOLD ? H : N)) return;
    const u32 i = blockIdx.y / L, j = blockIdx.y % L, bin = blockIdx.z;
    const u64 *pin = d2 + (size_t)bin * stride2 + (size_t)i * N + n;
    u64 *pout = dig + (((size_t)bin * L + i) * L + j) * N + n;
    if (FOLD) {
        u64 y0, y1;
        fold_store(dc, j, digit_lift(dc, i, j, pin[0]), digit_lift(dc, i, j, pin[H]), y0, y1);
        pout[0] = y0;
        pout[H] = y1;
    } else {
        pout[0] = digit_lift(dc, i, j, pin[0]);
    }
}
void launch_digits(const DevConsts *dc, u32 N, u32 L, const u64 *d2, size_t stride2, u32 nb, u64 *dig, hipStream_t st, bool fold)
{
    dim3 grid(((fold ? N / 2 : N) + TPB - 1) / TPB, L * L, nb);
    if (fold)
        hipLaunchKernelGGL(digits_kernel<true>, grid, dim3(TPB), 0, st, dc, N, L, d2, stride2, dig);
    else
        hipLaunchKernelGGL(digits_kernel<false>, grid, dim3(TPB), 0, st, dc, N, L, d2, stride2, dig);
}

template <bool MAD, int KP, int RPT = 1>
__global__ void __launch_bounds__(TPB) relin_mac_kernel(const DevConsts *__restrict__ dc, u32 N, u32 L, const u64 *__restrict__ d01,
                                                        size_t stride01, const u64 *__restrict__ dig,
                                                        const u64 *__restrict__ key0, const u64 *__restrict__ mask,
                                                        u64 *__restrict__ out, const u32 *__restrict__ out_map,
                                                        size_t key_stride, u32 key_group, u32 T, u32 mask_div, u32 nb)
{
    static_assert(RPT == 1 || MAD, "two rows per thread: the column-accumulator path");
    constexpr bool TILE = KP > 0;
    constexpr u32 TT = TILE ? TPB / (KP ? KP : 1) : 1;
    __shared__ u64x2 s_tile[TILE ? 2 * RPT : 1][TILE ? TPB : 1];
    u32 n = 2 * (blockIdx.x * TPB + threadIdx.x);
    u32 std_pair = 0;
    if (TILE) {
        const u32 tiles = T / TT, slice = blockIdx.x / tiles, tau0 = (blockIdx.x % tiles) * TT;
        const u32 k = threadIdx.x / TT, tt = threadIdx.x % TT;
        n = 2 * (slice * KP * T + k * T + tau0 + tt);
        std_pair = slice * KP * T + KP * tau0;
    }
    if (n >= N) return;
    const u32 j = blockIdx.y;
    u32 rows[RPT];
    bool has[RPT];
    if (RPT == 1) {
        rows[0] = blockIdx.z, has[0] = true;
    } else {
        const u32 k = blockIdx.z / key_group, q = blockIdx.z % key_group;
        rows[0] = 2 * k * key_group + q, has[0] = rows[0] < nb;
        rows[RPT - 1] = rows[0] + key_group, has[RPT - 1] = rows[RPT - 1] < nb;
        if (!has[0]) return;
    }
    const u32 bin = rows[0];
    const u64 *key = key0 + (size_t)(bin % key_group) * key_stride;
    const Mod m = dc->mod[j];
    const size_t LN = (size_t)L * N;
    const u32 po = TILE ? 0 : (out_map ? out_map[n] : n);
    u64x2 res[RPT][2];
    if (MAD) {
        ColAcc a[RPT][2][2];
#pragma unroll
        for (int r = 0; r < RPT; r++)
#pragma unroll
            for (int c = 0; c < 2; c++) a[r][c][0] = a[r][c][1] = ColAcc{0, 0, 0};
        for (u32 i = 0; i < L; i++) {
            const u64x2 k0 = *reinterpret_cast<const u64x2 *>(key + (((size_t)i * 2 + 0) * L + j) * N + n);
            const u64x2 k1 = *reinterpret_cast<const u64x2 *>(key + (((size_t)i * 2 + 1) * L + j) * N + n);
            const Split30 k0x = split30(k0.x), k0y = split30(k0.y), k1x = split30(k1.x), k1y = split30(k1.y);
#pragma unroll
            for (int r = 0; r < RPT; r++) {
                if (r && !has[r]) continue;
                const u64x2 d = *reinterpret_cast<const u64x2 *>(dig + (((size_t)rows[r] * L + i) * L + j) * N + n);
                const Split30 dx = split30(d.x), dy = split30(d.y);
                colacc_mac(a[r][0][0], dx, k0x);
                colacc_mac(a[r][0][1], dy, k0y);
                colacc_mac(a[r][1][0], dx, k1x);
                colacc_mac(a[r][1][1], dy, k1y);
            }
        }
        const u64 nq = 0 - m.q;
#pragma unroll
        for (int r = 0; r < RPT; r++) {
            if (r && !has[r]) continue;
            u64x2 mk;
            if (mask) mk = *reinterpret_cast<const u64x2 *>(mask + (size_t)(rows[r] / mask_div) * LN + (size_t)j * N + n);
#pragma unroll
            for (int c = 0; c < 2; c++) {
                const u64x2 s = *reinterpret_cast<const u64x2 *>(d01 + (size_t)rows[r] * stride01 + (size_t)c * LN + (size_t)j * N + n);
                a[r][c][0].c0 += s.x;
                a[r][c][1].c0 += s.y;
                res[r][c].x = colacc_reduce<false>(a[r][c][0], m, nq);
                res[r][c].y = colacc_reduce<false>(a[r][c][1], m, nq);
                if (mask) {
                    ColAcc p0 = {0, 0, 0}, p1 = {0, 0, 0};
                    colacc_mac(p0, split30(res[r][c].x), split30(mk.x));
                    colacc_mac(p1, split30(res[r][c].y), split30(mk.y));
                    res[r][c].x = colacc_reduce<false>(p0, m, nq);
                    res[r][c].y = colacc_reduce<false>(p1, m, nq);
                }
            }
        }
    } else {
        u64x2 mk;
        if (mask) mk = *reinterpret_cast<const u64x2 *>(mask + (size_t)(bin / mask_div) * LN + (size_t)j * N + n);
        U128 acc[2][2];
#pragma unroll
        for (int c = 0; c < 2; c++)
#pragma unroll
            for (int e = 0; e < 2; e++) acc[c][e] = U128{0, 0};
        for (u32 i = 0; i < L; i++) {
            const u64x2 d = *reinterpret_cast<const u64x2 *>(dig + (((size_t)bin * L + i) * L + j) * N + n);
            const u64x2 k0 = *reinterpret_cast<const u64x2 *>(key + (((size_t)i * 2 + 0) * L + j) * N + n);
            const u64x2 k1 = *reinterpret_cast<const u64x2 *>(key + (((size_t)i * 2 + 1) * L + j) * N + n);
            mac128(acc[0][0], d.x, k0.x);
            mac128(acc[0][1], d.y, k0.y);
            mac128(acc[1][0], d.x, k1.x);
            mac128(acc[1][1], d.y, k1.y);
        }
#pragma unroll
        for (int c = 0; c < 2; c++) {
            const u64x2 s = *reinterpret_cast<const u64x2 *>(d01 + (size_t)bin * stride01 + (size_t)c * LN + (size_t)j * N + n);
            add128(acc[c][0], U128{s.x, 0});
            add128(acc[c][1], U128{s.y, 0});
            res[0][c].x = reduce128(acc[c][0], m);
            res[0][c].y = reduce128(acc[c][1], m);
            if (mask) {
                res[0][c].x = mulmod(res[0][c].x, mk.x, m);
                res[0][c].y = mulmod(res[0][c].y, mk.y, m);
            }
        }
    }
#pragma unroll
    for (int r = 0; r < RPT; r++)
#pragma unroll
        for (int c = 0; c < 2; c++) {
            if (r && !has[r]) continue;
            const u64x2 v = res[r][c];
            if (TILE)
                s_tile[2 * r + c][KP * (threadIdx.x % TT) + threadIdx.x / TT] = v;
            else
                *reinterpret_cast<u64x2 *>(out + ((size_t)rows[r] * 2 + c) * LN + (size_t)j * N + po) = v;
        }
    if (TILE) {
        __syncthreads();
#pragma unroll
        for (int r = 0; r < RPT; r++)
#pragma unroll
            for (int c = 0; c < 2; c++) {
                if (r && !has[r]) continue;
                *reinterpret_cast<u64x2 *>(out + ((size_t)rows[r] * 2 + c) * LN + (size_t)j * N + 2 * (std_pair + threadIdx.x)) = s_tile[2 * r + c][threadIdx.x];
            }
    }
}
void launch_relin_mac(const DevConsts *dc, u32 N, u32 L, const u64 *d01, size_t stride01, const u64 *dig, const u64 *key,
                      const u64 *mask, u64 *out, u32 nb, hipStream_t st, bool small_moduli, const u32 *out_map, size_t key_stride,
                      u32 key_group, u32 sigma_T, u32 sigma_kp, u32 mask_div)
{
    if (!key_group) key_group = 1;
    if (!mask_div) mask_div = 1;
    const bool tile = out_map && (sigma_kp == 16 || sigma_kp == 8) && sigma_T >= TPB / sigma_kp && sigma_T % (TPB / sigma_kp) == 0 &&
                      (N / 2) % TPB == 0;
    const int kp = tile ? (int)sigma_kp : 0;
    const bool two = small_moduli && nb >= 2 * key_group;
    const u32 zrows = two ? ((nb + 2 * key_group - 1) / (2 * key_group)) * key_group : nb;
    dim3 grid((N / 2 + TPB - 1) / TPB, L, zrows);
#define RM(M_, K_, R_)                                                                                                              \
    hipLaunchKernelGGL((relin_mac_kernel<M_, K_, R_>), grid, dim3(TPB), 0, st, dc, N, L, d01, stride01, dig, key, mask, out, out_map, \
                       key_stride, key_group, sigma_T, mask_div, nb)
    if (two) {
        if (kp == 16) RM(true, 16, 2); else if (kp == 8) RM(true, 8, 2); else RM(true, 0, 2);
    } else if (small_moduli) {
        if (kp == 16) RM(true, 16, 1); else if (kp == 8) RM(true, 8, 1); else RM(true, 0, 1);
    } else {
        if (kp == 16) RM(false, 16, 1); else if (kp == 8) RM(false, 8, 1); else RM(false, 0, 1);
    }
#undef RM
}

__global__ void host_flag_kernel(volatile u64 *flag, u64 value)
{
    *flag = value;
    __threadfence_system();
}
void launch_host_flag(u64 *flag_dev, u64 value, hipStream_t st)
{
    hipLaunchKernelGGL(host_flag_kernel, dim3(1), dim3(1), 0, st, (volatile u64 *)flag_dev, value);
}

__global__ void __launch_bounds__(TPB) ct_add_kernel(const DevConsts *dc, u32 N, u32 L, const u64 *__restrict__ x,
                                                     const u64 *__restrict__ y, u64 *__restrict__ out)
{
    const u32 n = blockIdx.x * TPB + threadIdx.x;
    if (n >= N) return;
    const u32 l = blockIdx.y % L;
    const size_t o = ((size_t)blockIdx.z * 2 * L + blockIdx.y) * N + n;
    out[o] = addmod(x[o], y[o], dc->mod[l].q);
}
void launch_ct_add(const DevConsts *dc, u32 N, u32 L, const u64 *x, const u64 *y, u64 *out, u32 nct, hipStream_t st)
{
    dim3 grid((N + TPB - 1) / TPB, 2 * L, nct);
    hipLaunchKernelGGL(ct_add_kernel, grid, dim3(TPB), 0, st, dc, N, L, x, y, out);
}
__global__ void __launch_bounds__(TPB) ct_mul_plain_kernel(const DevConsts *dc, u32 N, u32 L, const u64 *__restrict__ x,
                                                           const u64 *__restrict__ pt, size_t pt_stride,
                                                           u64 *__restrict__ out, u32 pt_div)
{
    const u32 n = blockIdx.x * TPB + threadIdx.x;
    if (n >= N) return;
    const u32 l = blockIdx.y % L;
    const size_t o = ((size_t)blockIdx.z * 2 * L + blockIdx.y) * N + n;
    out[o] = mulmod(x[o], pt[(size_t)(blockIdx.z / pt_div) * pt_stride + (size_t)l * N + n], dc->mod[l]);
}
void launch_ct_mul_plain(const DevConsts *dc, u32 N, u32 L, const u64 *x, const u64 *pt, size_t pt_stride, u64 *out,
                         u32 nct, hipStream_t st, u32 pt_div)
{
    dim3 grid((N + TPB - 1) / TPB, 2 * L, nct);
    hipLaunchKernelGGL(ct_mul_plain_kernel, grid, dim3(TPB), 0, st, dc, N, L, x, pt, pt_stride, out, pt_div ? pt_div : 1);
}

template <int L, int KEEP>
__global__ void __launch_bounds__(TPB) limb_drop_kernel(const DevConsts *__restrict__ dc, u32 N, u32 blocks_per_poly,
                                                        const u64 *__restrict__ in, u64 *__restrict__ out)
{
    const u32 poly = blockIdx.x / blocks_per_poly;
    const u32 n = (blockIdx.x % blocks_per_poly) * TPB + threadIdx.x;
    if (n >= N) return;
    const u64 *pin = in + (size_t)poly * L * N + n;
    u64 c[L];
#pragma unroll
    for (int i = 0; i < L; i++) c[i] = pin[(size_t)i * N];
#pragma unroll
    for (int l = L - 1; l >= KEEP; l--) {
        const u64 ql = dc->mod[l].q;
        const u64 v = c[l];
        const u64 s = (u64)((int64_t)((ql >> 1) - v) >> 63);
#pragma unroll
        for (int i = 0; i < l; i++) {
            const u64 off = dc->drop_off[l][i];
            const u64 x = c[i] - v + off + (s & (ql - off));
            c[i] = mul_shoup_u(x, dc->drop_inv[l][i], dc->drop_inv_sh[l][i], dc->mod[i].q, dc->drop_negq[i]);
        }
    }
    u64 *pout = out + (size_t)poly * KEEP * N + n;
#pragma unroll
    for (int i = 0; i < KEEP; i++) pout[(size_t)i * N] = c[i];
}
bool launch_limb_drop(const DevConsts *dc, u32 N, u32 L, u32 keep, const u64 *in, u64 *out, u32 npoly, hipStream_t st)
{
    if (keep < 1 || keep >= L || L > MAX_L || !npoly) return false;
    const u32 bpp = (N + TPB - 1) / TPB;
    const dim3 grid(bpp * npoly), block(TPB);
#define DROP_(L_, K_)                                                                                          \
    case (L_) * 8 + (K_):                                                                                      \
        hipLaunchKernelGGL((limb_drop_kernel<L_, K_>), grid, block, 0, st, dc, N, bpp, in, out);               \
        return true
    switch (L * 8 + keep) {
        DROP_(2, 1);
        DROP_(3, 1); DROP_(3, 2);
        DROP_(4, 1); DROP_(4, 2); DROP_(4, 3);
        DROP_(5, 1); DROP_(5, 2); DROP_(5, 3); DROP_(5, 4);
        DROP_(6, 1); DROP_(6, 2); DROP_(6, 3); DROP_(6, 4); DROP_(6, 5);
        DROP_(7, 1); DROP_(7, 2); DROP_(7, 3); DROP_(7, 4); DROP_(7, 5); DROP_(7, 6);
    }
#undef DROP_
    return false;
}

__global__ void __launch_bounds__(TPB) permute_kernel(u32 N, const u64 *__restrict__ in, const u32 *__restrict__ map,
                                                      u64 *__restrict__ out)
{
    const u32 p = blockIdx.x * TPB + threadIdx.x;
    if (p >= N) return;
    const size_t r = (size_t)blockIdx.y * N;
    out[r + p] = in[r + map[p]];
}
void launch_permute(u32 N, const u64 *in, const u32 *map, u64 *out, u32 nrows, hipStream_t st)
{
    dim3 grid((N + TPB - 1) / TPB, nrows);
    hipLaunchKernelGGL(permute_kernel, grid, dim3(TPB), 0, st, N, in, map, out);
}

__global__ void __launch_bounds__(TPB) bcast_mul_plain_kernel(const DevConsts *dc, u32 N, u32 L, const u64 *__restrict__ x,
                                                              size_t xs, u32 group, const u64 *__restrict__ pt, size_t ps_outer,
                                                              size_t ps_inner, u64 *__restrict__ out)
{
    const u32 n = blockIdx.x * TPB + threadIdx.x;
    if (n >= N) return;
    const u32 l = blockIdx.y % L, i = blockIdx.z, g = i / group, r = i % group;
    const size_t LN = (size_t)L * N;
    const size_t o = (size_t)blockIdx.y * N + n;
    out[(size_t)i * 2 * LN + o] = mulmod(x[(size_t)g * xs + o], pt[(size_t)g * ps_outer + (size_t)r * ps_inner + (size_t)l * N + n], dc->mod[l]);
}
void launch_bcast_mul_plain(const DevConsts *dc, u32 N, u32 L, const u64 *x, size_t xs, u32 group, const u64 *pt, size_t ps_outer,
                            size_t ps_inner, u64 *out, u32 nct, hipStream_t st)
{
    dim3 grid((N + TPB - 1) / TPB, 2 * L, nct);
    hipLaunchKernelGGL(bcast_mul_plain_kernel, grid, dim3(TPB), 0, st, dc, N, L, x, xs, group, pt, ps_outer, ps_inner, out);
}
__global__ void __launch_bounds__(TPB) rot_prepare_kernel(const DevConsts *dc, u32 N, u32 L, const u64 *__restrict__ x,
                                                          const u32 *__restrict__ maps, u32 map_group, u32 acc, u32 identity_first,
                                                          u64 *__restrict__ d01, u64 *__restrict__ d2)
{
    const u32 p = blockIdx.x * TPB + threadIdx.x;
    if (p >= N) return;
    const u32 l = blockIdx.y, i = blockIdx.z, r = i % map_group;
    const size_t LN = (size_t)L * N;
    const u64 *c0 = x + (size_t)i * 2 * LN + (size_t)l * N, *c1 = c0 + LN;
    u64 *o0 = d01 + (size_t)i * 2 * LN + (size_t)l * N, *o1 = o0 + LN, *o2 = d2 + (size_t)i * LN + (size_t)l * N;
    if (identity_first && r == 0) {
        o0[p] = c0[p];
        o1[p] = c1[p];
        o2[p] = 0;
        return;
    }
    const u32 s = maps[(size_t)r * N + p];
    const u64 q = dc->mod[l].q;
    o0[p] = acc ? addmod(c0[p], c0[s], q) : c0[s];
    o1[p] = acc ? c1[p] : 0;
    o2[p] = c1[s];
}
void launch_rot_prepare(const DevConsts *dc, u32 N, u32 L, const u64 *x, const u32 *maps, u32 map_group, bool acc, bool identity_first,
                        u64 *d01, u64 *d2, u32 nct, hipStream_t st)
{
    dim3 grid((N + TPB - 1) / TPB, L, nct);
    hipLaunchKernelGGL(rot_prepare_kernel, grid, dim3(TPB), 0, st, dc, N, L, x, maps, map_group ? map_group : 1u, acc ? 1u : 0u,
                       identity_first ? 1u : 0u, d01, d2);
}
__global__ void __launch_bounds__(TPB) sum_mul_plain_kernel(const DevConsts *dc, u32 N, u32 L, const u64 *__restrict__ x, u32 group,
                                                            const u64 *__restrict__ pt, size_t pt_stride, u64 *__restrict__ out,
                                                            size_t out_stride)
{
    const u32 n = blockIdx.x * TPB + threadIdx.x;
    if (n >= N) return;
    const u32 l = blockIdx.y % L, g = blockIdx.z;
    const size_t LN = (size_t)L * N;
    const size_t o = (size_t)blockIdx.y * N + n;
    const Mod m = dc->mod[l];
    u64 s = 0;
    for (u32 r = 0; r < group; r++) s = addmod(s, x[((size_t)g * group + r) * 2 * LN + o], m.q);
    out[(size_t)g * out_stride + o] = mulmod(s, pt[(size_t)g * pt_stride + (size_t)l * N + n], m);
}
void launch_sum_mul_plain(const DevConsts *dc, u32 N, u32 L, const u64 *x, u32 group, const u64 *pt, size_t pt_stride, u64 *out,
                          size_t out_stride, u32 ngroups, hipStream_t st)
{
    dim3 grid((N + TPB - 1) / TPB, 2 * L, ngroups);
    hipLaunchKernelGGL(sum_mul_plain_kernel, grid, dim3(TPB), 0, st, dc, N, L, x, group, pt, pt_stride, out, out_stride);
}

__global__ void __launch_bounds__(TPB) encode_scatter_kernel(const DevConsts *dc, u32 N, u32 M,
                                                             const int64_t *__restrict__ slots, u32 B,
                                                             const u32 *__restrict__ inv_pos, u64 *__restrict__ u)
{
    const u32 p = blockIdx.x * TPB + threadIdx.x;
    if (p >= N) return;
    const u64 t = dc->mod[M].q;
    const u32 s = inv_pos[p];
    u64 val = 0;
    if (s < B) {
        const int64_t v = slots[(size_t)blockIdx.y * B + s];
        const u64 mag = v < 0 ? (u64)(-v) : (u64)v;
        val = v < 0 ? (mag ? t - mag : 0) : mag;
    }
    u[(size_t)blockIdx.y * N + p] = val;
}
void launch_encode_scatter(const DevConsts *dc, u32 N, u32 M, const int64_t *slots, u32 B, const u32 *inv_pos, u64 *u,
                           u32 npt, hipStream_t st)
{
    dim3 grid((N + TPB - 1) / TPB, npt);
    hipLaunchKernelGGL(encode_scatter_kernel, grid, dim3(TPB), 0, st, dc, N, M, slots, B, inv_pos, u);
}
__global__ void __launch_bounds__(TPB) encode_lift_kernel(const DevConsts *dc, u32 N, u32 L, u32 M,
                                                          const u64 *__restrict__ u, u64 *__restrict__ out)
{
    const u32 n = blockIdx.x * TPB + threadIdx.x;
    if (n >= N) return;
    const u64 t = dc->mod[M].q;
    const u64 v = u[(size_t)blockIdx.z * N + n];
    const u64 q = dc->mod[blockIdx.y].q;
    out[((size_t)blockIdx.z * L + blockIdx.y) * N + n] = v > t / 2 ? q - (t - v) : v;
}
void launch_encode_lift(const DevConsts *dc, u32 N, u32 L, u32 M, const u64 *u, u64 *out, u32 npt, hipStream_t st)
{
    dim3 grid((N + TPB - 1) / TPB, L, npt);
    hipLaunchKernelGGL(encode_lift_kernel, grid, dim3(TPB), 0, st, dc, N, L, M, u, out);
}

}
```

### nested_hashing_psi_amd/csrc/ntt16_kernel.h

```cpp
#pragma once
#include <vector>

#include "madasm.h"
#include "params.hpp"

namespace piehip {
namespace ntt16 {

typedef u64 u64x2 __attribute__((ext_vector_type(2)));

template <u32 LOGNS>
struct Geo {
    static constexpr u32 LOGN = LOGNS;
    static constexpr u32 NS = 1u << LOGNS;
    static constexpr u32 T = NS / 16;
    static constexpr u32 W = T / 64;
    static constexpr u32 R = NS / 1024;
    static constexpr u32 LOGR = LOGNS - 10;
    static constexpr u32 CPT = 16 / R;
    static constexpr u32 LDS_WORDS = NS + NS / 16;
    static constexpr u32 TWK_PER_SLICE = W * 15 * 16 + W * 12 * 64;
};
static constexpr u32 LOGN = Geo<13>::LOGN, NS = Geo<13>::NS, T = Geo<13>::T, LDS_WORDS = Geo<13>::LDS_WORDS,
                     TWK_PER_SLICE = Geo<13>::TWK_PER_SLICE;

__device__ __forceinline__ u32 phi(u32 e) { return e + 2 * (e >> 5); }

struct Tw {
    u32 wl, wh, sl, sh, sh2;
};
__device__ __forceinline__ Tw make_tw(u64x2 p)
{
    Tw t;
    t.wl = (u32)p.x, t.wh = (u32)(p.x >> 32), t.sl = (u32)p.y, t.sh = (u32)(p.y >> 32);
    t.sh2 = t.sh << 1;
    return t;
}

struct ModC {
    u32 nql, nqh;
    u64 nq4;
    u64 q4;
};

#define NTT16_S(x) "s"(x)
#define NTT16_V(x) "v"(x)
#include "ntt16_bfly.inc"

#ifndef NTT16_INV_H2
#define NTT16_INV_H2 1
#endif
template <bool INV, bool SC, bool H2 = SC && (!INV || NTT16_INV_H2)>
__device__ __forceinline__ void bfly(u64 &x0, u64 &y0, const Tw &t0, const ModC &m)
{
    const u64 a0 = x0, b0 = y0;
    if (INV) {
        u32 aol0, aoh0;
        u64 bo0;
        if (SC && H2)
            NTT16_GS1H(NTT16_S);
        else if (SC)
            NTT16_GS1(NTT16_S);
        else if (H2)
            NTT16_GS1H(NTT16_V);
        else
            NTT16_GS1(NTT16_V);
        x0 = ((u64)aoh0 << 32) | aol0, y0 = bo0;
    } else {
        u64 ao0;
        u32 bol0, boh0;
        if (SC && H2)
            NTT16_CT1H(NTT16_S);
        else if (SC)
            NTT16_CT1(NTT16_S);
        else if (H2)
            NTT16_CT1H(NTT16_V);
        else
            NTT16_CT1(NTT16_V);
        x0 = ao0, y0 = ((u64)boh0 << 32) | bol0;
    }
}
template <bool INV, bool SC, bool H2 = SC && !INV>
__device__ __forceinline__ void bfly2(u64 &x0, u64 &y0, const Tw &t0, u64 &x1, u64 &y1, const Tw &t1, const ModC &m)
{
    bfly<INV, SC, H2>(x0, y0, t0, m);
    bfly<INV, SC, H2>(x1, y1, t1, m);
}
__device__ __forceinline__ constexpr int bfly_lo(int m, int d) { return ((m & ~(d - 1)) << 1) | (m & (d - 1)); }

typedef const __attribute__((address_space(4))) u64x2 *TwS;
typedef const __attribute__((address_space(4))) DevConsts *DcS;
__device__ __forceinline__ u64 uniform_addr(const void *p)
{
    const u64 v = (u64)p;
    const u32 lo = __builtin_amdgcn_readfirstlane((u32)v), hi = __builtin_amdgcn_readfirstlane((u32)(v >> 32));
    return ((u64)hi << 32) | lo;
}

__device__ __forceinline__ u64 csub_neg(u64 x, u64 negm)
{
    u32 lo, hi;
    asm("v_lshl_add_u64 v[126:127], %[x], 0, %[nm]\n\t"
        "v_ashrrev_i32 v125, 31, v127\n\t"
        "v_bfi_b32 %[lo], v125, %[xl], v126\n\t"
        "v_bfi_b32 %[hi], v125, %[xh], v127"
        : [lo] "=&v"(lo), [hi] "=&v"(hi)
        : [x] "v"(x), [xl] "v"((u32)x), [xh] "v"((u32)(x >> 32)), [nm] "s"(negm)
        : "v125", "v126", "v127");
    return ((u64)hi << 32) | lo;
}

__device__ __forceinline__ const u64 *at_bytes(const u64 *ubase, u32 boff)
{
    return reinterpret_cast<const u64 *>(reinterpret_cast<const char *>(ubase) + boff);
}
__device__ __forceinline__ u64 *at_bytes(u64 *ubase, u32 boff) { return reinterpret_cast<u64 *>(reinterpret_cast<char *>(ubase) + boff); }
__device__ __forceinline__ const u64x2 *at_bytes(const u64x2 *ubase, u32 boff)
{
    return reinterpret_cast<const u64x2 *>(reinterpret_cast<const char *>(ubase) + boff);
}

template <u32 CPT>
__device__ __forceinline__ void row_get(u64 *x, int r, const u64 *p)
{
    if (CPT == 2) {
        const u64x2 v = *reinterpret_cast<const u64x2 *>(p);
        x[2 * r] = v.x, x[2 * r + 1] = v.y;
    } else {
        x[r] = *p;
    }
}
template <u32 CPT>
__device__ __forceinline__ void row_put(const u64 *x, int r, u64 *p)
{
    if (CPT == 2) {
        u64x2 v;
        v.x = x[2 * r], v.y = x[2 * r + 1];
        *reinterpret_cast<u64x2 *>(p) = v;
    } else {
        *p = x[r];
    }
}
typedef __attribute__((address_space(1))) u64 g_u64;
typedef __attribute__((address_space(1))) u64x2 g_u64x2;
__device__ __forceinline__ u64x2 pair_get_global(const u64 *p) { return *(const g_u64x2 *)p; }
__device__ __forceinline__ void pair_put_global(u64x2 v, u64 *p) { *(g_u64x2 *)p = v; }
template <u32 CPT>
__device__ __forceinline__ void row_put_global(const u64 *x, int r, u64 *p)
{
    if (CPT == 2) {
        u64x2 v;
        v.x = x[2 * r], v.y = x[2 * r + 1];
        pair_put_global(v, p);
    } else {
        *(g_u64 *)p = x[r];
    }
}
template <u32 CPT>
__device__ __forceinline__ void row_get_global(u64 *x, int r, const u64 *p)
{
    if (CPT == 2) {
        const u64x2 v = pair_get_global(p);
        x[2 * r] = v.x, x[2 * r + 1] = v.y;
    } else {
        x[r] = *(const g_u64 *)p;
    }
}

__device__ __forceinline__ void wave_sync()
{
    asm volatile("s_waitcnt lgkmcnt(0)" ::: "memory");
    __builtin_amdgcn_wave_barrier();
}

struct Args {
    u64 *data;
    const u64x2 *twp;
    const u64x2 *twk;
    const DevConsts *dc;
    u32 N;
    u32 s0;
    u32 nitems;
    u32 mod_base, mod_count;
    u32 flags;
    u32 skip_L, skip_M;
    u64 *copy_out;
    u32 copy_K, copy_L, copy_M;
    u64 *data2;
    const u64 *lift_src;
    size_t lift_stride;
    u32 lift_first, lift_L;
    const u64 *tsrc;
};
enum : u32 {
    F_STD_IN = 1,
    F_LAZY_OUT = 2,
    F_FOLDED = 4,
    F_X_LANE_IN = 8,
};

template <u32 LOGNS>
inline void build_twk_table_t(const u64 *nat, u32 s0, std::vector<u64> &out)
{
    typedef Geo<LOGNS> G;
    out.assign((size_t)(1u << s0) * G::TWK_PER_SLICE * 2, 0);
    for (u32 blk = 0; blk < (1u << s0); blk++) {
        u64 *o = &out[(size_t)blk * G::TWK_PER_SLICE * 2];
        auto put = [&](size_t dst, size_t src) {
            o[2 * dst] = nat[2 * src];
            o[2 * dst + 1] = nat[2 * src + 1];
        };
        for (u32 w = 0; w < G::W; w++) {
            for (u32 sc = 0; sc < 4; sc++)
                for (u32 jj = 0; jj < (1u << sc); jj++)
                    for (u32 la = 0; la < 16; la++) {
                        const u32 ml = (16 * G::W) << sc;
                        put(((size_t)w * 15 + ((1u << sc) - 1 + jj)) * 16 + la, ((size_t)ml << s0) + (size_t)blk * ml + (((16 * w + la) << sc) + jj));
                    }
            for (u32 l = 0; l < 64; l++) {
                const u32 m11 = 256 * G::W, m12 = 512 * G::W;
                for (u32 jj = 0; jj < 4; jj++)
                    put(G::W * 15 * 16 + ((size_t)w * 12 + jj) * 64 + l, ((size_t)m11 << s0) + (size_t)blk * m11 + 256 * w + 4 * l + jj);
                for (u32 jj = 0; jj < 8; jj++)
                    put(G::W * 15 * 16 + ((size_t)w * 12 + 4 + jj) * 64 + l, ((size_t)m12 << s0) + (size_t)blk * m12 + 512 * w + 8 * l + jj);
            }
        }
    }
}
inline void build_twk_table(const u64 *nat, u32 s0, std::vector<u64> &out) { build_twk_table_t<13>(nat, s0, out); }
inline u32 lane_to_std_t(u32 p, u32 threads)
{
    const u32 tau = (p >> 1) % threads, j = (p >> 1) / threads;
    return 16 * tau + 2 * j + (p & 1);
}
inline u32 lane_to_std(u32 p) { return lane_to_std_t(p, T); }

#ifndef NTT16_STAMP
#define NTT16_STAMP(i)
#endif

#define NTT16_TWL(ml, i) tw[(((u32)(ml)) << a.s0) + blk * (u32)(ml) + (i)]
#define NTT16_FENCE() __builtin_amdgcn_sched_barrier(0)
#define NTT16_PASS_PRIO(p) __builtin_amdgcn_s_setprio(p)
#ifndef NTT16_PF
#define NTT16_PF 3, 0, 3, 2, 1
#endif
#ifndef NTT16_PI
#define NTT16_PI 3, 3, 2, 0, 1
#endif
#define NTT16_PRIO_PICK_(i, a0, a1, a2, a3, a4) ((i) == 0 ? (a0) : (i) == 1 ? (a1) : (i) == 2 ? (a2) : (i) == 3 ? (a3) : (a4))
#define NTT16_PRIO_PICK(i, ...) NTT16_PRIO_PICK_(i, __VA_ARGS__)
#define NTT16_PRIO_F(i) NTT16_PASS_PRIO(NTT16_PRIO_PICK(i, NTT16_PF))
#define NTT16_PRIO_I(i) NTT16_PASS_PRIO(NTT16_PRIO_PICK(i, NTT16_PI))

#ifndef NTT16_LIFT_XCD
#define NTT16_LIFT_XCD 1
#endif
#ifndef NTT16_TENSOR_XCD
#define NTT16_TENSOR_XCD 1
#endif
__device__ __forceinline__ u64 csub2_neg(u64 x, u64 negm4, u64 negm2)
{
    u32 lo, hi;
    asm("v_lshl_add_u64 v[126:127], %[x], 0, %[n4]\n\t"
        "v_ashrrev_i32 v125, 31, v127\n\t"
        "v_bfi_b32 v122, v125, %[xl], v126\n\t"
        "v_bfi_b32 v123, v125, %[xh], v127\n\t"
        "v_lshl_add_u64 v[126:127], v[122:123], 0, %[n2]\n\t"
        "v_ashrrev_i32 v125, 31, v127\n\t"
        "v_bfi_b32 %[lo], v125, v122, v126\n\t"
        "v_bfi_b32 %[hi], v125, v123, v127"
        : [lo] "=&v"(lo), [hi] "=&v"(hi)
        : [x] "v"(x), [xl] "v"((u32)x), [xh] "v"((u32)(x >> 32)), [n4] "s"(negm4), [n2] "s"(negm2)
        : "v122", "v123", "v125", "v126", "v127");
    return ((u64)hi << 32) | lo;
}
__device__ __forceinline__ u64 colacc123_to_4q(u64 c0, u64 c1, u64 c2, u64 mu, u64 nq)
{
    u64 r;
    asm("v_lshrrev_b64 v[118:119], 30, %[c0]\n\t"
        "v_lshl_add_u64 v[118:119], v[118:119], 0, %[c1]\n\t"
        "v_lshrrev_b64 v[120:121], 30, v[118:119]\n\t"
        "v_lshl_add_u64 v[120:121], v[120:121], 0, %[c2]\n\t"
        "v_lshlrev_b64 v[122:123], 1, v[120:121]\n\t"
        "v_bfe_u32 v126, v118, 29, 1\n\t"
        "v_and_b32 v124, 0x3fffffff, %[c0l]\n\t"
        "v_bfe_u32 v125, v118, 2, 28\n\t"
        "v_or_b32 v122, v122, v126\n\t"
        "v_lshl_or_b32 v124, v118, 30, v124\n\t"
        "v_lshl_or_b32 v125, v120, 28, v125\n\t"
        "v_mul_hi_u32 v126, v122, %[mul]\n\t"
        "v_mov_b32 v127, 0\n\t"
        "v_mad_u64_u32 v[126:127], vcc, v122, %[muh], v[126:127]\n\t"
        "v_mad_u64_u32 v[126:127], vcc, v123, %[mul], v[126:127]\n\t"
        "v_mad_u64_u32 v[118:119], s[96:97], v123, %[muh], 0\n\t"
        "v_lshrrev_b64 v[126:127], 32, v[126:127]\n\t"
        "v_addc_co_u32 v127, vcc, 0, v127, vcc\n\t"
        "v_lshl_add_u64 v[126:127], v[118:119], 0, v[126:127]\n\t"
        "v_mad_u64_u32 v[118:119], vcc, v126, %[nqh], 0\n\t"
        "v_mad_u64_u32 v[118:119], vcc, v127, %[nql], v[118:119]\n\t"
        "v_add_u32 v125, v125, v118\n\t"
        "v_mad_u64_u32 %[r], vcc, v126, %[nql], v[124:125]"
        : [r] "=v"(r)
        : [c0] "v"(c0), [c1] "v"(c1), [c2] "v"(c2), [c0l] "v"((u32)c0), [mul] "s"((u32)mu), [muh] "s"((u32)(mu >> 32)),
          [nql] "s"((u32)nq), [nqh] "s"((u32)(nq >> 32))
        : "vcc", "s96", "s97", "v118", "v119", "v120", "v121", "v122", "v123", "v124", "v125", "v126", "v127");
    return r;
}
#ifndef NTT16_TENSOR_DEPTH
#define NTT16_TENSOR_DEPTH 3
#endif
template <u32 T, bool TWO>
__device__ __forceinline__ void tensor_load(u64 (&x)[16], const u64 *pa, const u64 *pb, const u64 *pc, const u64 *pd, u32 voffb, u64 q,
                                            u64 mu)
{
    constexpr int DEPTH = NTT16_TENSOR_DEPTH;
    const u64 nq = 0 - q, nq2 = 0 - 2 * q, nq4 = 0 - 4 * q;
    u64x2 va[8], vb[8], vc[8], vd[8];
#define NTT16_TLOAD(j)                                                           \
    do {                                                                         \
        va[j] = pair_get_global(at_bytes(pa + 2 * T * (j), voffb));              \
        vb[j] = pair_get_global(at_bytes(pb + 2 * T * (j), voffb));              \
        if (TWO) {                                                               \
            vc[j] = pair_get_global(at_bytes(pc + 2 * T * (j), voffb));          \
            vd[j] = pair_get_global(at_bytes(pd + 2 * T * (j), voffb));          \
        }                                                                        \
    } while (0)
#pragma unroll
    for (int j = 0; j < DEPTH; j++) NTT16_TLOAD(j);
#pragma unroll
    for (int j = 0; j < 8; j++) {
        NTT16_FENCE();
#pragma unroll
        for (int k = 0; k < 2; k++) {
            const u64 fa = csub2_neg(k ? va[j].y : va[j].x, nq4, nq2);
            const u64 fb = TWO ? csub2_neg(k ? vb[j].y : vb[j].x, nq4, nq2) : csub_neg(k ? vb[j].y : vb[j].x, nq4);
            const Split30 sa = split30(fa), sb = split30(fb);
            ColAcc c;
            c.c0 = mul_u(sa.lo, sb.lo);
            c.c1 = mad_u(sa.hi, sb.lo, mul_u(sa.lo, sb.hi));
            c.c2 = mul_u(sa.hi, sb.hi);
            if (TWO) {
                const u64 fc = csub2_neg(k ? vc[j].y : vc[j].x, nq4, nq2);
                const u64 fd = csub2_neg(k ? vd[j].y : vd[j].x, nq4, nq2);
                colacc_mac(c, split30(fc), split30(fd));
            }
            x[2 * j + k] = colacc123_to_4q(c.c0, c.c1, c.c2, mu, nq);
        }
        NTT16_FENCE();
        if (j + DEPTH < 8) NTT16_TLOAD(j + DEPTH);
    }
#undef NTT16_TLOAD
}

template <u32 LOGNS, bool INV, bool LIFT = false, bool TENSOR = false>
__global__ void __launch_bounds__(Geo<LOGNS>::T, 4) ntt16_kernel_t(Args a)
{
    typedef Geo<LOGNS> G;
    constexpr u32 NS = G::NS, T = G::T, R = G::R, LOGR = G::LOGR, CPT = G::CPT, TWK_PER_SLICE = G::TWK_PER_SLICE;
    extern __shared__ __attribute__((aligned(16))) u64 lds[];
    const u32 tau = threadIdx.x;
    const u32 w = __builtin_amdgcn_readfirstlane(tau >> 6), l = tau & 63;
    const u32 la = l >> 2, lc = l & 3;
    u64 *const p1 = lds + phi(CPT * tau);
    u64 *const p2 = lds + phi(1024 * w + l);
    u64 *const p3 = lds + 1088 * w + 68 * la + lc;
    u64 *const p4 = lds + phi(1024 * w + 16 * l);

    u64 x[16];
    auto limb_of = [&](u32 it) -> u32 {
        u32 lb = it >> a.s0;
        if (!INV && a.skip_L) {
            const u32 P = a.skip_M - a.skip_L, per = 2 * P + 2 * a.skip_M;
            const u32 cb = lb / per, r = lb % per;
            lb = cb * 4 * a.skip_M + (r < 2 * P ? (r / P) * a.skip_M + a.skip_L + r % P : 2 * a.skip_M + (r - 2 * P));
        }
        return lb;
    };
    for (u32 item = blockIdx.x; item < a.nitems; item += gridDim.x) {
        u32 tau_ = tau;
        asm volatile("" : "+v"(tau_));
        const u32 voffb = 16 * tau_;
        const u32 coffb = 8 * CPT * tau_;
        const u32 lab = 4 * (tau_ & 60), lb = 16 * (tau_ & 63);
        const bool lift = LIFT && !INV && item >= a.lift_first;
        u32 item_l = item;
        if (lift) {
            item_l = item - a.lift_first;
#if NTT16_LIFT_XCD
            const u32 G = a.lift_L << a.s0, blk8 = 8 * G, within = item_l % blk8;
            if (item_l - within + blk8 <= a.nitems - a.lift_first) item_l = item_l - within + (within & 7) * G + (within >> 3);
#endif
        }
        u32 t_d = 0, t_row = 0, t_blk = 0, t_limb = 0;
        if (TENSOR) {
            const u32 M_ = a.mod_count;
#if NTT16_TENSOR_XCD
            u32 il = item;
            const u32 within = il % 24;
            if (il - within + 24 <= a.nitems) il = il - within + (within & 7) * 3 + (within >> 3);
            const u32 u = il / 3, lm = u >> a.s0;
            t_d = il % 3, t_blk = u & ((1u << a.s0) - 1), t_row = lm / M_;
            t_limb = (t_row * 3 + t_d) * M_ + lm % M_;
#else
            t_limb = item >> a.s0, t_blk = item & ((1u << a.s0) - 1);
            t_row = t_limb / (3 * M_), t_d = (t_limb / M_) % 3;
#endif
            t_d = __builtin_amdgcn_readfirstlane(t_d), t_row = __builtin_amdgcn_readfirstlane(t_row);
            t_blk = __builtin_amdgcn_readfirstlane(t_blk), t_limb = __builtin_amdgcn_readfirstlane(t_limb);
        }
        const u32 blk = TENSOR ? t_blk : item_l & ((1u << a.s0) - 1);
        const u32 limb = TENSOR ? t_limb : lift ? item_l >> a.s0 : limb_of(item);
        u64 *g = (lift ? a.data2 : a.data) + (((size_t)limb << a.s0) + blk) * NS;
        asm("" : "+s"(g));
        const u32 mod = __builtin_amdgcn_readfirstlane(a.mod_base + limb % a.mod_count);
        const DcS dcs = (DcS)(u64)a.dc;
        const u64 q = dcs->mod[mod].q;
        const u64 q2 = 2 * q, q4 = 4 * q;
        ModC mc;
        mc.nql = (u32)(0 - q), mc.nqh = (u32)((0 - q) >> 32), mc.nq4 = 0 - q4, mc.q4 = q4;
        const TwS tw = (TwS)(u64)(a.twp + ((size_t)mod * 2 + (INV ? 1 : 0)) * a.N);
        const u64x2 *__restrict__ twk = a.twk + (((size_t)mod * 2 + (INV ? 1 : 0)) << a.s0) * TWK_PER_SLICE + (size_t)blk * TWK_PER_SLICE;
        const u64x2 *__restrict__ tw3 = twk + (size_t)w * 15 * 16;
        const u64x2 *__restrict__ tw4 = twk + G::W * 15 * 16 + (size_t)w * 12 * 64;
        u64x2 t7[1], t8[2], t9[4], t10[8], t11[4], t12[8];
#define NTT16_LOAD3(dst, sc)                                                       \
    _Pragma("unroll") for (int j_ = 0; j_ < (1 << (sc)); j_++) dst[j_] = *at_bytes(tw3 + 16 * ((1 << (sc)) - 1 + j_), lab)
#define NTT16_LOAD3H(dst, sc, from)                                                \
    _Pragma("unroll") for (int j_ = (from); j_ < (from) + 4; j_++) dst[j_] = *at_bytes(tw3 + 16 * ((1 << (sc)) - 1 + j_), lab)
#define NTT16_LOAD4(dst, first, n)                                                 \
    _Pragma("unroll") for (int j_ = 0; j_ < (n); j_++) dst[j_] = *at_bytes(tw4 + 64 * ((first) + j_), lb)

        if (!INV) {
            NTT16_STAMP(0);
            NTT16_PRIO_F(0);
            if (lift) {
                const u32 LL = a.lift_L, li = __builtin_amdgcn_readfirstlane((limb / LL) % LL), lj = __builtin_amdgcn_readfirstlane(limb % LL);
                const u64 *src = a.lift_src + (size_t)(limb / (LL * LL)) * a.lift_stride + (size_t)li * a.N;
                const u64 qi = dcs->mod[li].q;
                const u64 nqh1 = 0 - (qi / 2 + 1), dq = q - qi;
                auto lift1 = [&](u64 v) -> u64 {
                    u64 r;
                    asm("v_lshl_add_u64 v[126:127], %[v], 0, %[nqh1]\n\t"
                        "v_ashrrev_i32 v125, 31, v127\n\t"
                        "v_bfi_b32 v126, v125, 0, %[dql]\n\t"
                        "v_bfi_b32 v127, v125, 0, %[dqh]\n\t"
                        "v_lshl_add_u64 %[r], %[v], 0, v[126:127]"
                        : [r] "=v"(r)
                        : [v] "v"(v), [nqh1] "s"(nqh1), [dql] "s"((u32)dq), [dqh] "s"((u32)(dq >> 32))
                        : "v125", "v126", "v127");
                    return r;
                };
                if (a.s0 == 1) {
                    u64x2 fw;
                    fw.x = dcs->fold_w[lj];
                    fw.y = dcs->fold_w_sh[lj] >> 1;
                    const Tw t = make_tw(fw);
                    u64 y[16];
#pragma unroll
                    for (int r = 0; r < (int)R; r++) {
                        row_get_global<CPT>(x, r, at_bytes(src + 1024 * r, coffb));
                        row_get_global<CPT>(y, r, at_bytes(src + NS + 1024 * r, coffb));
                    }
#pragma unroll
                    for (int k = 0; k < 16; k++) {
                        u64 u0 = lift1(x[k]), v0 = lift1(y[k]);
                        bfly<false, true>(u0, v0, t, mc);
                        x[k] = blk ? v0 : u0;
                    }
                } else {
#pragma unroll
                    for (int r = 0; r < (int)R; r++) row_get_global<CPT>(x, r, at_bytes(src + 1024 * r, coffb));
#pragma unroll
                    for (int k = 0; k < 16; k++) x[k] = lift1(x[k]);
                }
            } else {
#pragma unroll
                for (int r = 0; r < (int)R; r++) row_get_global<CPT>(x, r, at_bytes(g + 1024 * r, coffb));
            }
            NTT16_PRIO_F(1);
#pragma unroll
            for (int s = 0; s < (int)LOGR; s++) {
                const int d = (int)(R >> 1) >> s;
#pragma unroll
                for (int r = 0; r < (int)R; r++) {
                    if (r & d) continue;
                    const Tw t = make_tw(NTT16_TWL(1u << s, (u32)r >> (LOGR - s)));
#pragma unroll
                    for (int c = 0; c < (int)CPT; c++) bfly<false, true>(x[CPT * r + c], x[CPT * (r + d) + c], t, mc);
                }
            }
            NTT16_STAMP(1);
            __syncthreads();
            NTT16_STAMP(2);
#pragma unroll
            for (int r = 0; r < (int)R; r++) row_put<CPT>(x, r, p1 + 1088 * r);
            NTT16_STAMP(3);
            __syncthreads();
            NTT16_STAMP(4);
            NTT16_PRIO_F(2);
#pragma unroll
            for (int k = 0; k < 16; k++) x[k] = p2[68 * k];
#pragma unroll
            for (int sb = 0; sb < 4; sb++) {
                const int d = 8 >> sb;
#pragma unroll
                for (int mm = 0; mm < 8; mm += 2) {
                    const int k0 = bfly_lo(mm, d), k1 = bfly_lo(mm + 1, d);
                    const Tw t0 = make_tw(NTT16_TWL(G::W << sb, (w << sb) + ((u32)k0 >> (4 - sb))));
                    const Tw t1 = make_tw(NTT16_TWL(G::W << sb, (w << sb) + ((u32)k1 >> (4 - sb))));
                    bfly2<false, true>(x[k0], x[k0 + d], t0, x[k1], x[k1 + d], t1, mc);
                }
            }
            NTT16_LOAD3(t7, 0);
            NTT16_LOAD3(t8, 1);
#pragma unroll
            for (int k = 0; k < 16; k++) p2[68 * k] = x[k];
            NTT16_STAMP(5);
            wave_sync();
            NTT16_PRIO_F(3);
#pragma unroll
            for (int k = 0; k < 16; k++) x[k] = p3[4 * k + 2 * (k >> 3)];
            NTT16_LOAD3(t9, 2);
            NTT16_FENCE();
            {
                const Tw t = make_tw(t7[0]);
#pragma unroll
                for (int k = 0; k < 8; k += 2) bfly2<false, false, true>(x[k], x[k + 8], t, x[k + 1], x[k + 9], t, mc);
            }
            NTT16_LOAD3H(t10, 3, 0);
            NTT16_FENCE();
#pragma unroll
            for (int mm = 0; mm < 8; mm += 2) {
                const int k0 = bfly_lo(mm, 4), k1 = bfly_lo(mm + 1, 4);
                bfly2<false, false, true>(x[k0], x[k0 + 4], make_tw(t8[k0 >> 3]), x[k1], x[k1 + 4], make_tw(t8[k1 >> 3]), mc);
            }
            NTT16_LOAD3H(t10, 3, 4);
            NTT16_FENCE();
#pragma unroll
            for (int mm = 0; mm < 8; mm += 2) {
                const int k0 = bfly_lo(mm, 2), k1 = bfly_lo(mm + 1, 2);
                bfly2<false, false>(x[k0], x[k0 + 2], make_tw(t9[k0 >> 2]), x[k1], x[k1 + 2], make_tw(t9[k1 >> 2]), mc);
            }
            NTT16_LOAD4(t11, 0, 4);
            NTT16_FENCE();
#pragma unroll
            for (int k = 0; k < 16; k += 4)
                bfly2<false, false>(x[k], x[k + 1], make_tw(t10[k >> 1]), x[k + 2], x[k + 3], make_tw(t10[(k >> 1) + 1]), mc);
#pragma unroll
            for (int k = 0; k < 16; k++) p3[4 * k + 2 * (k >> 3)] = x[k];
            NTT16_STAMP(6);
            wave_sync();
            NTT16_PRIO_F(4);
#pragma unroll
            for (int j = 0; j < 8; j++) {
                const u64x2 v = *reinterpret_cast<const u64x2 *>(p4 + 2 * j);
                x[2 * j] = v.x;
                x[2 * j + 1] = v.y;
            }
            NTT16_LOAD4(t12, 4, 4);
            NTT16_FENCE();
#pragma unroll
            for (int g4 = 0; g4 < 4; g4++) {
                const Tw t = make_tw(t11[g4]);
                bfly2<false, false>(x[4 * g4], x[4 * g4 + 2], t, x[4 * g4 + 1], x[4 * g4 + 3], t, mc);
                if (g4 == 1) {
                    NTT16_FENCE();
                    _Pragma("unroll") for (int j_ = 4; j_ < 8; j_++) t12[j_] = *at_bytes(tw4 + 64 * (4 + j_), lb);
                    NTT16_FENCE();
                }
            }
            NTT16_FENCE();
#pragma unroll
            for (int k = 0; k < 16; k += 4)
                bfly2<false, false>(x[k], x[k + 1], make_tw(t12[k >> 1]), x[k + 2], x[k + 3], make_tw(t12[(k >> 1) + 1]), mc);
            NTT16_STAMP(7);
            const bool lazy = (a.flags & F_LAZY_OUT) != 0 && !lift;
            if (!lazy) {
#pragma unroll
                for (int k = 0; k < 16; k++) x[k] = csub_neg(csub_neg(csub_neg(x[k], 0 - q4), 0 - q2), 0 - q);
            }
#pragma unroll
            for (int j = 0; j < 8; j++) {
                u64x2 v;
                v.x = x[2 * j], v.y = x[2 * j + 1];
                pair_put_global(v, at_bytes(g + 2 * T * j, voffb));
            }
            NTT16_STAMP(8);
        } else {
            NTT16_STAMP(0);
            NTT16_PRIO_I(0);
            NTT16_LOAD4(t12, 4, 4);
            const bool is_x = !TENSOR && (a.flags & F_STD_IN) && a.copy_out && (limb / (2 * a.copy_L)) % a.copy_K == 0;
            u64 *co = nullptr;
            if (is_x) {
                const u32 bin = limb / (2 * a.copy_L * a.copy_K), cc = (limb / a.copy_L) & 1, i = limb % a.copy_L;
                co = a.copy_out + (((((size_t)bin * 4 + cc) * a.copy_M + i) << a.s0) + blk) * NS;
                asm("" : "+s"(co));
            }
            const bool x_in = is_x && (a.flags & F_X_LANE_IN);
            if (!TENSOR && (a.flags & F_STD_IN) && !x_in) {
                u64 yv[16];
                const u64 *gw = g + 1024 * w;
#pragma unroll
                for (int j = 0; j < 8; j++) {
                    const u64x2 v = pair_get_global(at_bytes(gw + 128 * j, lb));
                    yv[2 * j] = v.x, yv[2 * j + 1] = v.y;
                }
                {
                    u64 *const pw = lds + phi(1024 * w + 2 * l);
#pragma unroll
                    for (int j = 0; j < 8; j++) {
                        u64x2 v;
                        v.x = yv[2 * j], v.y = yv[2 * j + 1];
                        *reinterpret_cast<u64x2 *>(pw + 136 * j) = v;
                    }
                }
                wave_sync();
#pragma unroll
                for (int j = 0; j < 8; j++) {
                    const u64x2 v = *reinterpret_cast<const u64x2 *>(p4 + 2 * j);
                    x[2 * j] = v.x;
                    x[2 * j + 1] = v.y;
                }
                if (is_x) {
#pragma unroll
                    for (int j = 0; j < 8; j++) {
                        u64x2 v;
                        v.x = x[2 * j], v.y = x[2 * j + 1];
                        pair_put_global(v, at_bytes(co + 2 * T * j, voffb));
                    }
                }
            } else if (TENSOR) {
                const u32 M_ = a.mod_count;
                const size_t ss = ((size_t)M_ << a.s0) * NS;
                const u64 *e0 = a.tsrc + ((((size_t)t_row * 4 * M_ + limb % M_) << a.s0) + blk) * NS;
                const u64 *pa = e0 + (t_d == 2 ? ss : 0), *pb = e0 + (t_d == 0 ? 2 : 3) * ss, *pc = e0 + ss, *pd = e0 + 2 * ss;
                asm("" : "+s"(pa), "+s"(pb), "+s"(pc), "+s"(pd));
                const u64 mu = (dcs->mod[mod].r1 << 59) | (dcs->mod[mod].r0 >> 5);
                if (t_d == 1)
                    tensor_load<T, true>(x, pa, pb, pc, pd, voffb, q, mu);
                else
                    tensor_load<T, false>(x, pa, pb, pc, pd, voffb, q, mu);
            } else {
                const u64 *src = x_in ? co : g;
                asm("" : "+s"(src));
#pragma unroll
                for (int j = 0; j < 8; j++) {
                    const u64x2 v = pair_get_global(at_bytes(src + 2 * T * j, voffb));
                    x[2 * j] = v.x, x[2 * j + 1] = v.y;
                }
            }
            NTT16_FENCE();
            _Pragma("unroll") for (int j_ = 4; j_ < 8; j_++) t12[j_] = *at_bytes(tw4 + 64 * (4 + j_), lb);
            NTT16_FENCE();
            NTT16_PRIO_I(1);
#pragma unroll
            for (int k = 0; k < 16; k += 4) {
                bfly2<true, false>(x[k], x[k + 1], make_tw(t12[k >> 1]), x[k + 2], x[k + 3], make_tw(t12[(k >> 1) + 1]), mc);
                if (k == 4) {
                    NTT16_FENCE();
                    NTT16_LOAD4(t11, 0, 4);
                    NTT16_FENCE();
                }
            }
            NTT16_LOAD3(t10, 3);
            NTT16_FENCE();
#pragma unroll
            for (int g4 = 0; g4 < 4; g4++) {
                const Tw t = make_tw(t11[g4]);
                bfly2<true, false>(x[4 * g4], x[4 * g4 + 2], t, x[4 * g4 + 1], x[4 * g4 + 3], t, mc);
            }
            NTT16_STAMP(1);
            NTT16_STAMP(2);
#pragma unroll
            for (int j = 0; j < 8; j++) {
                u64x2 v;
                v.x = x[2 * j];
                v.y = x[2 * j + 1];
                *reinterpret_cast<u64x2 *>(p4 + 2 * j) = v;
            }
            wave_sync();
            NTT16_STAMP(3);
            NTT16_PRIO_I(2);
#pragma unroll
            for (int k = 0; k < 16; k++) x[k] = p3[4 * k + 2 * (k >> 3)];
            NTT16_LOAD3(t9, 2);
            NTT16_FENCE();
#pragma unroll
            for (int k = 0; k < 16; k += 4)
                bfly2<true, false>(x[k], x[k + 1], make_tw(t10[k >> 1]), x[k + 2], x[k + 3], make_tw(t10[(k >> 1) + 1]), mc);
            NTT16_LOAD3(t8, 1);
            NTT16_LOAD3(t7, 0);
            NTT16_FENCE();
#pragma unroll
            for (int mm = 0; mm < 8; mm += 2) {
                const int k0 = bfly_lo(mm, 2), k1 = bfly_lo(mm + 1, 2);
                bfly2<true, false>(x[k0], x[k0 + 2], make_tw(t9[k0 >> 2]), x[k1], x[k1 + 2], make_tw(t9[k1 >> 2]), mc);
            }
            NTT16_FENCE();
#pragma unroll
            for (int mm = 0; mm < 8; mm += 2) {
                const int k0 = bfly_lo(mm, 4), k1 = bfly_lo(mm + 1, 4);
                bfly2<true, false>(x[k0], x[k0 + 4], make_tw(t8[k0 >> 3]), x[k1], x[k1 + 4], make_tw(t8[k1 >> 3]), mc);
            }
            {
                const Tw t = make_tw(t7[0]);
#pragma unroll
                for (int k = 0; k < 8; k += 2) bfly2<true, false>(x[k], x[k + 8], t, x[k + 1], x[k + 9], t, mc);
            }
#pragma unroll
            for (int k = 0; k < 16; k++) p3[4 * k + 2 * (k >> 3)] = x[k];
            wave_sync();
            NTT16_STAMP(4);
            NTT16_PRIO_I(3);
#pragma unroll
            for (int k = 0; k < 16; k++) x[k] = p2[68 * k];
#pragma unroll
            for (int sb = 3; sb >= 0; sb--) {
                const int d = 8 >> sb;
#pragma unroll
                for (int mm = 0; mm < 8; mm += 2) {
                    const int k0 = bfly_lo(mm, d), k1 = bfly_lo(mm + 1, d);
                    const Tw t0 = make_tw(NTT16_TWL(G::W << sb, (w << sb) + ((u32)k0 >> (4 - sb))));
                    const Tw t1 = make_tw(NTT16_TWL(G::W << sb, (w << sb) + ((u32)k1 >> (4 - sb))));
                    bfly2<true, true>(x[k0], x[k0 + d], t0, x[k1], x[k1 + d], t1, mc);
                }
            }
#pragma unroll
            for (int k = 0; k < 16; k++) p2[68 * k] = x[k];
            NTT16_STAMP(5);
            __syncthreads();
            NTT16_STAMP(6);
            NTT16_PRIO_I(4);
#pragma unroll
            for (int r = 0; r < (int)R; r++) row_get<CPT>(x, r, p1 + 1088 * r);
            __syncthreads();
#pragma unroll
            for (int s = (int)LOGR - 1; s >= 0; s--) {
                const int d = (int)(R >> 1) >> s;
#pragma unroll
                for (int r = 0; r < (int)R; r++) {
                    if (r & d) continue;
                    const Tw t = make_tw(NTT16_TWL(1u << s, (u32)r >> (LOGR - s)));
#pragma unroll
                    for (int c = 0; c < (int)CPT; c++) bfly<true, true>(x[CPT * r + c], x[CPT * (r + d) + c], t, mc);
                }
            }
            NTT16_STAMP(7);
            const u64 n_inv = dcs->mod[mod].n_inv, n_inv_sh = dcs->mod[mod].n_inv_sh;
            if (!(a.flags & F_FOLDED)) {
#pragma unroll
                for (int k = 0; k < 16; k++) {
                    if (a.s0 == 0)
                        x[k] = csub_neg(mul_shoup_lazy(x[k], n_inv, n_inv_sh, q), 0 - q);
                    else
                        x[k] = csub_neg(csub_neg(x[k], 0 - q2), 0 - q);
                }
            }
#pragma unroll
            for (int r = 0; r < (int)R; r++) row_put_global<CPT>(x, r, at_bytes(g + 1024 * r, coffb));
            NTT16_STAMP(8);
        }
    }
}
#undef NTT16_LOAD3
#undef NTT16_LOAD3H
#undef NTT16_LOAD4
#undef NTT16_FENCE
#undef NTT16_TWL

}
}
```

### nested_hashing_psi_amd/csrc/params.cpp

```cpp
#include "params.hpp"

#include <string.h>

namespace piehip {

typedef unsigned __int128 u128;

static inline u64 mm(u64 a, u64 b, u64 q) { return (u64)(((u128)a * b) % q); }

u64 powmod(u64 a, u64 e, u64 q)
{
    u64 r = 1 % q;
    a %= q;
    for (; e; e >>= 1) {
        if (e & 1) r = mm(r, a, q);
        a = mm(a, a, q);
    }
    return r;
}
u64 invmod(u64 a, u64 q) { return powmod(a % q, q - 2, q); }

u32 bitrev32(u32 x, u32 bits)
{
    u32 r = 0;
    for (u32 i = 0; i < bits; i++, x >>= 1) r = (r << 1) | (x & 1);
    return r;
}

bool is_prime_u64(u64 n)
{
    static const u64 B[] = {2, 3, 5, 7, 11, 13, 17, 19, 23, 29, 31, 37};
    if (n < 2) return false;
    for (u64 b : B) {
        if (n == b) return true;
        if (n % b == 0) return false;
    }
    u64 d = n - 1;
    int s = 0;
    for (; !(d & 1); d >>= 1) s++;
    for (u64 b : B) {
        u64 x = powmod(b, d, n);
        if (x == 1 || x == n - 1) continue;
        bool witness = true;
        for (int r = 1; r < s && witness; r++) {
            x = mm(x, x, n);
            if (x == n - 1) witness = false;
        }
        if (witness) return false;
    }
    return true;
}

bool prime_chain(u32 N, u64 below, u32 count, u64 *out)
{
    const u64 step = 2ULL * N;
    if (below <= step + 1) return false;
    u64 c = ((below - 2) / step) * step + 1;
    u32 got = 0;
    for (; got < count && c > step; c -= step)
        if (is_prime_u64(c)) out[got++] = c;
    return got == count;
}

u64 min_primitive_root(u64 q, u32 N)
{
    const u64 m = 2ULL * N;
    if ((q - 1) % m) return 0;
    u64 root = 0;
    for (u64 g = 2; g < 1000 && !root; g++) {
        u64 x = powmod(g, (q - 1) / m, q);
        if (powmod(x, N, q) == q - 1) root = x;
    }
    if (!root) return 0;
    const u64 sq = mm(root, root, q);
    u64 cur = root, best = root;
    for (u32 k = 1; k < N; k++) {
        cur = mm(cur, sq, q);
        if (cur < best) best = cur;
    }
    return best;
}

static inline u64 shoup(u64 w, u64 q) { return (u64)(((u128)w << 64) / q); }

static Mod make_mod(u64 q, u32 N)
{
    Mod m;
    memset(&m, 0, sizeof(m));
    m.q = q;
    u128 ratio = (~(u128)0) / q;
    m.r0 = (u64)ratio;
    m.r1 = (u64)(ratio >> 64);
    m.fshift = (u32)__builtin_clzll(q);
    m.fconst = (u64)((((u128)1) << (127 - m.fshift)) / q);
    m.n_inv = invmod(N, q);
    m.n_inv_sh = shoup(m.n_inv, q);
    return m;
}

static u64 prod_mod(const u64 *ms, u32 n, int skip, u64 q)
{
    u64 r = 1 % q;
    for (u32 k = 0; k < n; k++)
        if ((int)k != skip) r = mm(r, ms[k] % q, q);
    return r;
}

std::string HostParams::init(u32 N_, u32 L_, u64 t_, const u64 *q, const u64 *p)
{
    if (N_ < 8 || (N_ & (N_ - 1)) || N_ > (1u << 16)) return "N must be a power of two in [8, 65536]";
    if (L_ < 1 || L_ > MAX_L) return "L must be in [1, 7]";
    if ((t_ - 1) % (2ULL * N_) || !is_prime_u64(t_)) return "plaintext modulus t must be prime and = 1 (mod 2N)";
    N = N_;
    L = L_;
    M = 2 * L + 1;
    t = t_;
    logN = 0;
    while ((1u << logN) < N) logN++;
    moduli.assign(M + 1, 0);
    if (q && p) {
        for (u32 i = 0; i < L; i++) moduli[i] = q[i];
        for (u32 j = 0; j <= L; j++) moduli[L + j] = p[j];
    } else if (!q && !p) {
        if (!prime_chain(N, 1ULL << 60, M, moduli.data())) return "prime chain exhausted";
    } else {
        return "pass both q and p, or neither";
    }
    moduli[M] = t;
    for (u32 a = 0; a < M; a++) {
        const u64 m = moduli[a];
        if (m >> 61) return "RNS primes must be < 2^61";
        if (m <= t) return "RNS primes must exceed the plaintext modulus";
        if ((m - 1) % (2ULL * N) || !is_prime_u64(m)) return "RNS moduli must be prime and = 1 (mod 2N)";
        for (u32 b = 0; b < a; b++)
            if (moduli[b] == m) return "RNS moduli must be distinct";
    }

    psi.assign(M + 1, 0);
    tw.assign(M + 1, {});
    tw_sh.assign(M + 1, {});
    itw.assign(M + 1, {});
    itw_sh.assign(M + 1, {});
    memset(&dc, 0, sizeof(dc));
    dc.N = N;
    dc.logN = logN;
    dc.L = L;
    dc.M = M;
    for (u32 a = 0; a <= M; a++) {
        const u64 m = moduli[a];
        dc.mod[a] = make_mod(m, N);
        psi[a] = min_primitive_root(m, N);
        if (!psi[a]) return "no primitive 2N-th root";
        const u64 ipsi = invmod(psi[a], m);
        tw[a].assign(N, 0);
        itw[a].assign(N, 0);
        tw_sh[a].assign(N, 0);
        itw_sh[a].assign(N, 0);
        u64 pw = 1, ipw = 1;
        for (u32 e = 0; e < N; e++) {
            const u32 k = bitrev32(e, logN);
            tw[a][k] = pw;
            itw[a][k] = ipw;
            tw_sh[a][k] = shoup(pw, m);
            itw_sh[a][k] = shoup(ipw, m);
            pw = mm(pw, psi[a], m);
            ipw = mm(ipw, ipsi, m);
        }
        dc.fold_w[a] = tw[a][1];
        dc.fold_w_sh[a] = tw_sh[a][1];
        dc.fold_ia[a] = dc.mod[a].n_inv;
        dc.fold_ia_sh[a] = dc.mod[a].n_inv_sh;
        dc.fold_ib[a] = mm(itw[a][1], dc.mod[a].n_inv, m);
        dc.fold_ib_sh[a] = shoup(dc.fold_ib[a], m);
    }

    slot_pos.assign(N, 0);
    {
        const u64 m2 = 2ULL * N;
        u64 e = 1;
        for (u32 i = 0; i < N / 2; i++) {
            slot_pos[i] = bitrev32((u32)((e - 1) / 2), logN);
            slot_pos[N / 2 + i] = bitrev32((u32)((m2 - e - 1) / 2), logN);
            e = (e * 5) % m2;
        }
    }

    const u64 *Q = moduli.data();
    const u64 *P = moduli.data() + L;
    const u32 Lp = L + 1;
    for (u32 i = 0; i < L; i++) {
        const u64 qi = Q[i];
        dc.qhat_inv[i] = invmod(prod_mod(Q, L, (int)i, qi), qi);
        dc.qhat_inv_sh[i] = shoup(dc.qhat_inv[i], qi);
        dc.P_modq[i] = prod_mod(P, Lp, -1, qi);
        dc.P_modq_sh[i] = shoup(dc.P_modq[i], qi);
        dc.tPinv_modq[i] = mm(t % qi, invmod(dc.P_modq[i], qi), qi);
        for (u32 j = 0; j < Lp; j++) {
            const u64 pj = P[j];
            dc.qhat_modp[i][j] = prod_mod(Q, L, (int)i, pj);
            const u64 v = mm(dc.P_modq[i] % pj, invmod(qi, pj), pj);
            dc.PI_modp[i][j] = v ? pj - v : 0;
        }
        for (u32 j = 0; j < L; j++) dc.qi_modqj[i][j] = qi % Q[j];
        dc.t_inv_modq[i] = invmod(t % qi, qi);
        dc.fold_iaq[i] = mm(dc.fold_ia[i], dc.qhat_inv[i], qi);
        dc.fold_iaq_sh[i] = shoup(dc.fold_iaq[i], qi);
        dc.fold_ibq[i] = mm(dc.fold_ib[i], dc.qhat_inv[i], qi);
        dc.fold_ibq_sh[i] = shoup(dc.fold_ibq[i], qi);
        dc.t_modq_sh[i] = shoup(t % qi, qi);
    }
    for (u32 j = 0; j < Lp; j++) {
        const u64 pj = P[j];
        dc.Q_modp[j] = prod_mod(Q, L, -1, pj);
        dc.phat_inv[j] = invmod(prod_mod(P, Lp, (int)j, pj), pj);
        dc.phat_inv_sh[j] = shoup(dc.phat_inv[j], pj);
        dc.tQ_modp[j] = mm(t % pj, dc.Q_modp[j], pj);
        dc.tQ_modp_sh[j] = shoup(dc.tQ_modp[j], pj);
        for (u32 i = 0; i < L; i++) {
            const u64 qi = Q[i];
            dc.phat_modq[j][i] = prod_mod(P, Lp, (int)j, qi);
            const u64 v = mm(dc.tQ_modp[j] % qi, invmod(pj, qi), qi);
            dc.tQF_modq[j][i] = v ? qi - v : 0;
        }
    }
    dc.Q_modt = prod_mod(Q, L, -1, t);
    for (u32 a = 0; a < M; a++) {
        dc.qp_hat_inv[a] = invmod(prod_mod(moduli.data(), M, (int)a, moduli[a]), moduli[a]);
        dc.qp_hat_inv_sh[a] = shoup(dc.qp_hat_inv[a], moduli[a]);
    }
    for (u32 j = 0; j < Lp; j++) {
        const u64 pj = P[j];
        dc.fold_iap[j] = mm(dc.fold_ia[L + j], dc.qp_hat_inv[L + j], pj);
        dc.fold_iap_sh[j] = shoup(dc.fold_iap[j], pj);
        dc.fold_ibp[j] = mm(dc.fold_ib[L + j], dc.qp_hat_inv[L + j], pj);
        dc.fold_ibp_sh[j] = shoup(dc.fold_ibp[j], pj);
    }
    for (u32 k = 0; k < L; k++) {
        const u64 qk = Q[k];
        dc.fold_iat[k] = mm(dc.fold_ia[k], dc.tPinv_modq[k], qk);
        dc.fold_iat_sh[k] = shoup(dc.fold_iat[k], qk);
        dc.fold_ibt[k] = mm(dc.fold_ib[k], dc.tPinv_modq[k], qk);
        dc.fold_ibt_sh[k] = shoup(dc.fold_ibt[k], qk);
    }
    for (u32 l = 0; l < L; l++) {
        const u64 half = (Q[l] - 1) / 2;
        dc.drop_negq[l] = 0 - Q[l];
        for (u32 i = 0; i < l; i++) {
            const u64 qi = Q[i];
            dc.drop_inv[l][i] = invmod(Q[l] % qi, qi);
            dc.drop_inv_sh[l][i] = shoup(dc.drop_inv[l][i], qi);
            dc.drop_off[l][i] = (half + qi - 1) / qi * qi;
        }
    }
    return "";
}

std::vector<u32> HostParams::automorph_map(u32 g) const
{
    std::vector<u32> map(N);
    const u64 m2 = 2ULL * N;
    for (u32 p = 0; p < N; p++) {
        const u64 e = ((2ULL * bitrev32(p, logN) + 1) * g) % m2;
        map[p] = bitrev32((u32)((e - 1) / 2), logN);
    }
    return map;
}

}
```

### nested_hashing_psi_amd/csrc/params.hpp

```cpp
#pragma once
#include <stdint.h>

#include <string>
#include <vector>

#include "modarith.h"

namespace piehip {

static const u32 MAX_L = 7;
static const u32 MAX_M = 2 * MAX_L + 1;

struct DevConsts {
    Mod mod[MAX_M + 1];
    u64 qhat_inv[8];
    u64 qhat_inv_sh[8];
    u64 qhat_modp[8][8];
    u64 Q_modp[8];
    u64 P_modq[8];
    u64 P_modq_sh[8];
    u64 PI_modp[8][8];
    u64 phat_inv[8];
    u64 phat_inv_sh[8];
    u64 phat_modq[8][8];
    u64 qp_hat_inv[16];
    u64 qp_hat_inv_sh[16];
    u64 tPinv_modq[8];
    u64 tQ_modp[8];
    u64 tQ_modp_sh[8];
    u64 tQF_modq[8][8];
    u64 qi_modqj[8][8];
    u64 fold_w[MAX_M + 1], fold_w_sh[MAX_M + 1];
    u64 fold_ia[MAX_M + 1], fold_ia_sh[MAX_M + 1];
    u64 fold_ib[MAX_M + 1], fold_ib_sh[MAX_M + 1];
    u64 fold_iaq[8], fold_iaq_sh[8], fold_ibq[8], fold_ibq_sh[8];
    u64 fold_iap[8], fold_iap_sh[8], fold_ibp[8], fold_ibp_sh[8];
    u64 fold_iat[8], fold_iat_sh[8], fold_ibt[8], fold_ibt_sh[8];
    u64 t_inv_modq[8];
    u64 t_modq_sh[8];
    u64 Q_modt;
    u64 drop_inv[8][8], drop_inv_sh[8][8];
    u64 drop_off[8][8];
    u64 drop_negq[8];
    u32 N, logN, L, M;
};

struct HostParams {
    u32 N = 0, logN = 0, L = 0, M = 0;
    u64 t = 0;
    std::vector<u64> moduli;
    std::vector<u64> psi;
    std::vector<std::vector<u64>> tw, tw_sh, itw, itw_sh;
    std::vector<u32> slot_pos;
    DevConsts dc;

    std::string init(u32 N, u32 L, u64 t, const u64 *q, const u64 *p);
    std::vector<u32> automorph_map(u32 g) const;
};

bool is_prime_u64(u64 n);
bool prime_chain(u32 N, u64 below, u32 count, u64 *out);
u64 min_primitive_root(u64 q, u32 N);
u64 powmod(u64 a, u64 e, u64 q);
u64 invmod(u64 a, u64 q);
u32 bitrev32(u32 x, u32 bits);

}
```

### nested_hashing_psi_amd/csrc/piehip_ctx.hpp

```cpp
#pragma once
#include "../../include/piehip.h"

#include <hip/hip_runtime.h>
#include <stdio.h>
#include <stdlib.h>
#include <string.h>

#include <algorithm>
#include <map>
#include <memory>
#include <string>
#include <vector>

#include "kernels.hpp"
#include "params.hpp"

namespace piehip {
int fail(int code, const std::string &msg);
}
#define HIPCHK(expr)                                                                                   \
    do {                                                                                               \
        hipError_t e_ = (expr);                                                                        \
        if (e_ != hipSuccess)                                                                          \
            return piehip::fail(PIEHIP_EHIP, std::string(#expr) + ": " + hipGetErrorString(e_));       \
    } while (0)
struct piehip_ctx;
namespace piehip {
void join_pending(piehip_ctx *h);
void mark_dirty(piehip_ctx *h);
}
#define NEED_RO(h)                                                       \
    do {                                                                 \
        if (!(h)) return piehip::fail(PIEHIP_EINVAL, "null handle");     \
        piehip::join_pending(h);                                         \
    } while (0)
#define NEED(h)                                                 \
    do {                                                        \
        NEED_RO(h);                                             \
        piehip::mark_dirty(h);                                  \
    } while (0)

namespace piehip {

struct ProfRec {
    hipEvent_t a, b;
    int k;
    double bytes;
};

struct MulWs {
    u32 nb = 0;
    u64 *eqp = nullptr;
    u64 *dqp = nullptr;
    u64 *d01 = nullptr;
    u64 *d2c = nullptr;
    u64 *dig = nullptr;
};

struct Query {
    const u64 *idx = nullptr, *minus = nullptr;
    u64 *idx_own = nullptr, *minus_own = nullptr;
    u64 *pin_idx = nullptr, *pin_minus = nullptr;
    std::vector<bool> rows;
    std::vector<bool> cts;
    bool minus_staged = false;
    std::vector<bool> seeded;
    std::vector<u32> seeds;
};

}
using piehip::u32;
using piehip::u64;

struct piehip_ctx {
    piehip::HostParams hp;
    int device = 0;
    hipStream_t stream = nullptr;
    bool own_stream = false;
    std::vector<hipStream_t> side_streams;
    std::vector<hipEvent_t> ev_join;
    hipEvent_t ev_fork = nullptr;
    hipEvent_t ev_chain = nullptr;
    bool chain_armed = false;
    u32 run_streams = 0;
    bool inputs_dirty = true;
    hipEvent_t wait_before_results = nullptr;
    bool pending_join = false;
    bool use_graph = false;
    hipGraphExec_t gexec = nullptr;
    const void *g_idx = nullptr, *g_minus = nullptr, *g_res = nullptr;
    u32 g_ng = 0;
    bool stage_open = false;
    u64 *pin_up_flag = nullptr;
    u64 up_seq = 0;
    u64 up_turn_wait_ns = 0;
    u64 up_turn_wait_total_ns = 0, up_turn_waits = 0;
    bool hp_timing = false;
    hipEvent_t hp_ev[3] = {nullptr, nullptr, nullptr};
    int hp_ev_state = 0;
    u64 *host_results = nullptr;
    piehip::SeedJob *pin_seed_jobs = nullptr;
    piehip::SeedJob *d_seed_jobs = nullptr;
    size_t seed_jobs_cap = 0;
    u64 *pin_res = nullptr;
    size_t pin_idx_words = 0, pin_res_words = 0;
    piehip::DevConsts *d_dc = nullptr;
    std::vector<void *> dev_tables;
    u32 *d_inv_pos = nullptr;
    u32 *d_sigma_inv = nullptr;
    u64 *d_evk_sigma = nullptr, *d_masks_sigma = nullptr;
    u64 *d_hash_tbl = nullptr;
    size_t hash_tbl_words = 0;
    u64 *arena = nullptr;
    size_t arena_words = 0, arena_used = 0;
    u32 hk = 0, he = 0, hb = 0;
    piehip::NttPlan plan;
    bool db_borrowed = false;
    piehip_ctx *db_owner = nullptr;
    u32 db_borrowers = 0;
    u64 *d_evk = nullptr;
    u32 K = 0, b = 0, E = 0;
    u64 *d_db = nullptr, *d_masks = nullptr;
    piehip::Query query[piehip::STAGE_A_MAX_QUERIES];
    u32 nq = 1;
    u32 mask_div = 1;
    u32 key_group = 1;
    u64 *d_evkq = nullptr, *d_evkq_sigma = nullptr;
    u32 evkq_n = 0, evkq_loaded = 0;
    u64 *d_acc = nullptr;
    u64 *d_prod = nullptr;
    u64 *d_out = nullptr;
    u32 res_limbs = 0;
    u64 *d_full = nullptr;
    piehip::MulWs ws;
    size_t ws_cap_rows = 0;
    u32 ws_cap_K = 0;
    void *comm = nullptr;
    bool comm_owned = false;
    int comm_ranks = 0, comm_rank = 0;
    u64 *d_gather = nullptr, *pin_gather = nullptr;
    size_t gather_words = 0;
    std::map<int32_t, u64 *> rotkeys;
    std::map<int32_t, u32 *> rotmaps;
    u32 fp_npie = 0, fp_K = 0, fp_b = 0, fp_E = 0;
    u64 *fp_pt = nullptr;
    u64 *fp_mask = nullptr;
    u64 *fp_e0 = nullptr;
    u64 *fp_idx = nullptr;
    u64 *fp_out = nullptr;
    u64 *fp_negkeys = nullptr;
    u32 *fp_negmaps = nullptr;
    bool profiling = false;
    std::vector<piehip::ProfRec> recs;
    std::vector<hipEvent_t> pool;
    size_t pool_used = 0;

    size_t LN() const { return (size_t)hp.L * hp.N; }
    size_t res_ct_words() const { return 2 * (size_t)res_limbs * hp.N; }
};

namespace piehip {

inline bool run_keys_loaded(const piehip_ctx *h)
{
    return h->K <= 1 || h->d_evk || (h->d_evkq && h->evkq_n == h->nq && h->evkq_loaded == (1u << h->nq) - 1);
}

hipEvent_t prof_event(piehip_ctx *h);
struct ProfScope {
    piehip_ctx *h;
    ProfRec r;
    bool on;
    ProfScope(piehip_ctx *h_, int k, double bytes) : h(h_), on(h_->profiling)
    {
        if (!on) return;
        r.k = k;
        r.bytes = bytes;
        r.a = prof_event(h);
        r.b = prof_event(h);
        if (!r.a || !r.b) {
            on = false;
            return;
        }
        (void)hipEventRecord(r.a, h->stream);
    }
    ~ProfScope()
    {
        if (!on) return;
        (void)hipEventRecord(r.b, h->stream);
        h->recs.push_back(r);
    }
};

void drop_graph(piehip_ctx *h);
int dev_alloc(u64 **p, size_t words);
void dev_free(u64 **p);

struct Tmp {
    piehip_ctx *h = nullptr;
    size_t mark = 0;
    std::vector<u64 *> ptrs;
    Tmp() {}
    explicit Tmp(piehip_ctx *h_) : h(h_), mark(h_->arena_used) {}
    ~Tmp()
    {
        for (u64 *p : ptrs) (void)hipFree(p);
        if (h) h->arena_used = mark;
    }
    u64 *get(size_t words)
    {
        if (!words) words = 1;
        const size_t w32 = (words + 31) & ~(size_t)31;
        if (h && h->arena && h->arena_used + w32 <= h->arena_words) {
            u64 *p = h->arena + h->arena_used;
            h->arena_used += w32;
            return p;
        }
        u64 *p = nullptr;
        if (hipMalloc((void **)&p, words * sizeof(u64)) != hipSuccess) return nullptr;
        ptrs.push_back(p);
        return p;
    }
};
#define TMPGET(var, words)                                          \
    piehip::u64 *var = tmp.get(words);                              \
    if (!var) return piehip::fail(PIEHIP_ENOMEM, "hipMalloc failed (scratch)")

int ws_alloc(piehip_ctx *h, MulWs &w, u32 nb);
void ws_free(MulWs &w);

void ntt(piehip_ctx *h, u64 *data, u32 nlimbs, u32 mod_base, u32 mod_count, bool inv, bool sigma = false, bool fold = false,
         const NttExtra *ex = nullptr);
void enqueue_keyswitch(piehip_ctx *h, MulWs &w, u32 nb, const u64 *key, const u64 *mask, u64 *out, bool lane = false,
                       size_t key_stride = 0, u32 key_group = 1, bool out_is_result = false, bool digits_ready = false);
void enqueue_mul(piehip_ctx *h, MulWs &w, const u64 *x, size_t sx, const u64 *y, size_t sy, u32 nb, bool relin,
                 const u64 *mask, u64 *out, bool xq_ready = false, bool out_is_result = false);
int encode_on_device(piehip_ctx *h, const int64_t *d_slots, u32 npt, u32 B, u64 *d_out);
void enqueue_mod_reduce(piehip_ctx *h, u64 *full, u32 rows, u32 keep, u64 *out, bool out_is_result = false);
int ensure_full_rows(piehip_ctx *h);
int query_input_buffers(piehip_ctx *h, u32 q, u64 **d_idx, u64 **d_minus);
void use_owned_inputs(piehip_ctx *h);
void free_host_path(piehip_ctx *h);
int expand_seeded_sync(piehip_ctx *h, const std::vector<SeedJob> &jobs);
SeedJob seed_job(u64 *dst, const uint8_t *seed);
bool stage_has_seeded(const piehip_ctx *h);
u32 run_queue_count(const piehip_ctx *h);
int ensure_run_queues(piehip_ctx *h, u32 ng);
u32 run_group_size(u32 b, u32 ng, u32 g);

}
```

### nested_hashing_psi_amd/csrc/piehip_run.cpp

```cpp
#include "piehip_ctx.hpp"

using namespace piehip;

namespace piehip {

void ntt(piehip_ctx *h, u64 *data, u32 nlimbs, u32 mod_base, u32 mod_count, bool inv, bool sigma, bool fold, const NttExtra *ex)
{
    ProfScope ps(h, inv ? PIEHIP_K_NTT_INV : PIEHIP_K_NTT_FWD, 16.0 * h->hp.N * nlimbs);
    launch_ntt(h->plan, data, nlimbs, mod_base, mod_count, inv, h->stream, sigma && h->plan.lane_order, fold && h->plan.fold, ex);
}

void enqueue_keyswitch(piehip_ctx *h, MulWs &w, u32 nb, const u64 *key, const u64 *mask, u64 *out, bool lane, size_t key_stride,
                       u32 key_group, bool out_is_result, bool digits_ready)
{
    const NttPlan &pl = h->plan;
    const u32 N = h->hp.N, L = h->hp.L;
    const size_t LN = h->LN();
    const double W = 8.0 * N;
    lane = lane && pl.lane_order;
    if (digits_ready) {
    } else if (lane ? pl.digit_lift_lane : pl.digit_lift_std) {
        ProfScope ps(h, PIEHIP_K_NTT_FWD, 16.0 * N * nb * L * L);
        launch_ntt_digits(pl, w.d2c, w.dig, nb, L, lane, h->stream);
    } else {
        {
            ProfScope ps(h, PIEHIP_K_DIGITS, W * nb * (L + (double)L * L));
            launch_digits(h->d_dc, N, L, w.d2c, LN, nb, w.dig, h->stream, lane && pl.fold);
        }
        ntt(h, w.dig, nb * L * L, 0, L, false, lane, lane);
    }
    {
        if (h->wait_before_results && out_is_result) (void)hipStreamWaitEvent(h->stream, h->wait_before_results, 0);
        if (h->chain_armed && out_is_result) {
            h->chain_armed = false;
            (void)hipEventRecord(h->ev_chain, h->stream);
        }
        ProfScope ps(h, PIEHIP_K_RELIN, W * (nb * ((double)L * L + 2 * L + 2 * L + (mask ? L : 0)) + 2.0 * L * L));
        launch_relin_mac(h->d_dc, N, L, w.d01, 2 * LN, w.dig, key, mask, out, nb, h->stream, pl.small_moduli,
                         lane ? h->d_sigma_inv : nullptr, key_stride, key_group, lane ? pl.lane_T : 0, pl.lane_kp, mask ? h->mask_div : 1);
    }
}

struct RunKey {
    const u64 *key;
    size_t stride;
    u32 group;
};
static RunKey run_key(const piehip_ctx *h)
{
    const bool lane = h->plan.lane_order;
    if (h->key_group > 1) return {lane ? h->d_evkq_sigma : h->d_evkq, (size_t)h->hp.L * 2 * h->LN(), h->key_group};
    return {lane ? h->d_evk_sigma : h->d_evk, 0, 1};
}

void enqueue_mul(piehip_ctx *h, MulWs &w, const u64 *x, size_t sx, const u64 *y, size_t sy, u32 nb, bool relin,
                 const u64 *mask, u64 *out, bool xq_ready, bool out_is_result)
{
    const u32 N = h->hp.N, L = h->hp.L, M = h->hp.M;
    const size_t LN = h->LN();
    const double W = 8.0 * N;
    const NttPlan &pl = h->plan;
    {
        ProfScope ps(h, PIEHIP_K_EXPAND, W * nb * (4.0 * L + 4.0 * M));
        launch_expand_both(h->d_dc, N, L, x, sx, y, sy, LN, nb, w.eqp, h->stream, pl.small_moduli, pl.fold, xq_ready);
    }
    {
        NttExtra ex;
        ex.lazy_out = true;
        if (xq_ready) {
            ex.skip_L = L;
            ex.skip_M = M;
        }
        ntt(h, w.eqp, nb * (xq_ready ? 4 * M - 2 * L : 4 * M), 0, M, false, true, true, &ex);
    }
    if (pl.fused_tensor) {
        ProfScope ps(h, PIEHIP_K_TENSOR_NTT_INV, W * nb * 7.0 * M);
        launch_ntt16_tensor(pl, w.eqp, w.dqp, nb, M, h->stream);
    } else {
        {
            ProfScope ps(h, PIEHIP_K_TENSOR, W * nb * 7.0 * M);
            launch_tensor(h->d_dc, N, M, w.eqp, w.dqp, nb, h->stream, pl.small_moduli);
        }
        ntt(h, w.dqp, nb * 3 * M, 0, M, true, true, true);
    }
    if (relin) {
        {
            ProfScope ps(h, PIEHIP_K_SCALE, W * nb * (3.0 * M + 3.0 * L));
            launch_scale_round(h->d_dc, N, L, w.dqp, nb, w.d01, 2 * LN, w.d2c, LN, h->stream, pl.small_moduli, pl.fold, false);
        }
        NttExtra ex;
        ex.lazy_out = true;
        if (pl.digits_with_d01) {
            ProfScope ps(h, PIEHIP_K_NTT_FWD, 16.0 * N * nb * (2.0 * L + (double)L * L));
            Ntt16Digits dg = {w.d2c, LN, w.dig, nb, L};
            launch_ntt16(pl, w.d01, nb * 2 * L, 0, L, false, true, h->stream, &ex, &dg);
        } else {
            ntt(h, w.d01, nb * 2 * L, 0, L, false, true, true, &ex);
        }
        const RunKey k = run_key(h);
        enqueue_keyswitch(h, w, nb, k.key, mask, out, true, k.stride, k.group, out_is_result, pl.digits_with_d01);
    } else {
        {
            ProfScope ps(h, PIEHIP_K_SCALE, W * nb * (3.0 * M + 3.0 * L));
            launch_scale_round(h->d_dc, N, L, w.dqp, nb, out, 3 * LN, out + 2 * LN, 3 * LN, h->stream, pl.small_moduli, pl.fold, true);
        }
        ntt(h, out, nb * 3 * L, 0, L, false, false, true);
    }
}

void enqueue_mod_reduce(piehip_ctx *h, u64 *full, u32 rows, u32 keep, u64 *out, bool out_is_result)
{
    const u32 N = h->hp.N, L = h->hp.L;
    const double W = 8.0 * N;
    {
        ProfScope ps(h, PIEHIP_K_RESULT_NTT_INV, 2 * W * rows * 2 * L);
        launch_ntt(h->plan, full, rows * 2 * L, 0, L, true, h->stream);
    }
    if (out_is_result) {
        if (h->wait_before_results) (void)hipStreamWaitEvent(h->stream, h->wait_before_results, 0);
        if (h->chain_armed) {
            h->chain_armed = false;
            (void)hipEventRecord(h->ev_chain, h->stream);
        }
    }
    {
        ProfScope ps(h, PIEHIP_K_LIMB_DROP, W * rows * 2 * (L + keep));
        launch_limb_drop(h->d_dc, N, L, keep, full, out, rows * 2, h->stream);
    }
    {
        ProfScope ps(h, PIEHIP_K_RESULT_NTT_FWD, 2 * W * rows * 2 * keep);
        launch_ntt(h->plan, out, rows * 2 * keep, 0, keep, false, h->stream);
    }
}

static const u32 MAX_RUN_QUEUES = 2;
u32 run_queue_count(const piehip_ctx *h)
{
    const u32 want = h->run_streams ? h->run_streams : (h->b >= 8 ? 2u : 1u);
    return std::min(want, std::min(MAX_RUN_QUEUES, h->b));
}

int ensure_run_queues(piehip_ctx *h, u32 ng)
{
    while (h->side_streams.size() < ng) {
        hipStream_t s = nullptr;
        hipEvent_t e = nullptr;
        HIPCHK(hipStreamCreateWithFlags(&s, hipStreamNonBlocking));
        h->side_streams.push_back(s);
        HIPCHK(hipEventCreateWithFlags(&e, hipEventDisableTiming));
        h->ev_join.push_back(e);
    }
    return PIEHIP_OK;
}

u32 run_group_size(u32 b, u32 ng, u32 g)
{
    if (ng == 2) {
        const u32 first = (4 * b + 3) / 7;
        return g == 0 ? first : b - first;
    }
    return b / ng + (g < b % ng ? 1 : 0);
}

}

extern "C" {

static void enqueue_run_bins_full(piehip_ctx *h, u32 b0, u32 nb, u64 *results);
static void enqueue_run_bins(piehip_ctx *h, u32 b0, u32 nb, u64 *results)
{
    const u32 keep = h->res_limbs, nq = h->nq;
    if (keep >= h->hp.L) {
        enqueue_run_bins_full(h, b0, nb, results);
        return;
    }
    const hipEvent_t wait = h->wait_before_results;
    const bool chain = h->chain_armed;
    h->wait_before_results = nullptr;
    h->chain_armed = false;
    enqueue_run_bins_full(h, b0, nb, h->d_full);
    h->wait_before_results = wait;
    h->chain_armed = chain;
    const size_t r0 = (size_t)b0 * nq;
    enqueue_mod_reduce(h, h->d_full + r0 * 2 * h->LN(), nb * nq, keep, results + r0 * h->res_ct_words(), true);
}
static void enqueue_run_bins_full(piehip_ctx *h, u32 b0, u32 nb, u64 *results)
{
    const u32 N = h->hp.N, L = h->hp.L, M = h->hp.M, K = h->K, b = h->b, E = h->E, nq = h->nq;
    const size_t LN = h->LN();
    const double W = 8.0 * N;
    const size_t r0 = (size_t)b0 * nq;
    const u32 layers = nb;
    nb *= nq;
    MulWs w = h->ws;
    w.nb = nb;
    w.eqp += r0 * 4 * M * N;
    w.dqp += r0 * 3 * M * N;
    w.d01 += r0 * 2 * LN;
    w.d2c += r0 * LN;
    w.dig += r0 * L * LN;
    u64 *acc = h->d_acc + r0 * K * 2 * LN;
    u64 *prod = h->d_prod ? h->d_prod + r0 * 2 * LN : nullptr;
    u64 *out = results + r0 * 2 * LN;
    const u64 *masks = (h->plan.lane_order ? h->d_masks_sigma : h->d_masks) + (size_t)b0 * LN;
    struct MaskDiv {
        piehip_ctx *h;
        ~MaskDiv() { h->mask_div = h->key_group = 1; }
    } mask_div_scope{h};
    h->mask_div = nq;
    h->key_group = (nq > 1 && h->d_evkq && h->evkq_n == nq) ? nq : 1;
    const bool x_direct = K > 1 && nq > 1 && h->plan.x_direct;
    if (h->profiling) {
        ProfScope ps(h, PIEHIP_K_EVENT_PAIR, 0.0);
    }
    {
        ProfScope ps(h, PIEHIP_K_STAGE_A, W * ((double)layers * K * E * L + nq * ((double)K * E * 2 * L + 2.0 * L + (double)layers * K * 2 * L)));
        StageAQueries qs = {};
        for (u32 q = 0; q < nq; q++) qs.idx[q] = h->query[q].idx, qs.minus[q] = h->query[q].minus;
        const u64 *db = h->d_db + (size_t)b0 * E * LN;
        StageAXOut xo;
        if (x_direct) xo.out = w.eqp, xo.M = M, xo.logns = h->plan.lane_logn;
        if (nq > 1) {
            launch_stage_a_batch(h->d_dc, N, L, K, layers, E, qs, nq, db, acc, h->stream, h->plan.small_moduli, b, 0, 0, x_direct ? &xo : nullptr);
        } else {
            launch_stage_a(h->d_dc, N, L, K, nb, E, qs.idx[0], qs.minus[0], db, acc, h->stream, h->plan.small_moduli, b, 0, 0, 1, 0,
                           x_direct ? &xo : nullptr);
        }
    }
    if (K == 1) {
        if (h->wait_before_results) (void)hipStreamWaitEvent(h->stream, h->wait_before_results, 0);
        ProfScope ps(h, PIEHIP_K_MASK, W * nb * 5.0 * L);
        launch_ct_mul_plain(h->d_dc, N, L, acc, h->d_masks + (size_t)b0 * LN, LN, out, nb, h->stream, nq);
        return;
    }
    const bool xq = h->plan.xq_reuse;
    NttExtra ex;
    ex.copy_out = w.eqp;
    ex.copy_K = K;
    ex.copy_L = L;
    ex.copy_M = M;
    ex.x_lane_in = x_direct;
    ntt(h, acc, nb * K * 2 * L, 0, L, true, false, true, xq ? &ex : nullptr);
    ex.x_lane_in = false;
    const u64 *x = acc;
    size_t sx = (size_t)K * 2 * LN;
    for (u32 hf = 1; hf < K; hf++) {
        const bool last = hf + 1 == K;
        u64 *dst = last ? out : prod;
        enqueue_mul(h, w, x, sx, acc + (size_t)hf * 2 * LN, (size_t)K * 2 * LN, nb, true, last ? masks : nullptr, dst, xq, last);
        if (!last) {
            ex.copy_K = 1;
            ntt(h, prod, nb * 2 * L, 0, L, true, false, true, xq ? &ex : nullptr);
            x = prod;
            sx = 2 * LN;
        }
    }
}

static hipError_t download_rows(piehip_ctx *h, const u64 *d_results, u32 b0, u32 nb)
{
    const size_t row = (size_t)h->nq * h->res_ct_words();
    return hipMemcpyAsync(h->host_results + (size_t)b0 * row, d_results + (size_t)b0 * row, (size_t)nb * row * sizeof(u64),
                          hipMemcpyDeviceToHost, h->stream);
}

int piehip_run_into(piehip_handle h, void *d_results)
{
    if (!h) return fail(PIEHIP_EINVAL, "null handle");
    if (!d_results) return fail(PIEHIP_EINVAL, "null result buffer");
    if (!h->K || !h->d_db) return fail(PIEHIP_ESTATE, "run: database not loaded");
    if (!h->d_acc || !h->ws.eqp) return fail(PIEHIP_ESTATE, "run: no workspace (an earlier allocation failed: piehip_set_query_batch / load)");
    if (!run_keys_loaded(h)) return fail(PIEHIP_ESTATE, "run: relinearisation key not loaded");
    if (h->res_limbs < h->hp.L && !h->d_full) return fail(PIEHIP_ESTATE, "run: no rows for the result reduction (an earlier allocation failed: piehip_set_result_limbs)");
    for (u32 q = 0; q < h->nq; q++) {
        if (h->query[q].idx && h->query[q].minus) continue;
        if (q) return fail(PIEHIP_ESTATE, "run: a query of the batch has no index matrix or minus element");
        return fail(PIEHIP_ESTATE, "run: setIndex / setMinusCompareElement not called");
    }
    HIPCHK(hipSetDevice(h->device));
    const u32 b = h->b;
    h->recs.clear();
    h->pool_used = 0;
    const u32 ng = run_queue_count(h);
    if (ng > 1) {
        const int qrc = ensure_run_queues(h, ng);
        if (qrc) return qrc;
    }
    if (h->use_graph && !h->profiling && !h->host_results && h->nq == 1) {
        if (!h->gexec || h->g_idx != h->query[0].idx || h->g_minus != h->query[0].minus || h->g_res != d_results || h->g_ng != ng) {
            drop_graph(h);
            join_pending(h);
            struct Restore {
                piehip_ctx *h;
                hipStream_t s;
                ~Restore() { h->stream = s; }
            } restore{h, h->stream};
            hipGraph_t graph = nullptr;
            HIPCHK(hipStreamBeginCapture(restore.s, hipStreamCaptureModeThreadLocal));
            hipError_t ce = hipSuccess;
            if (ng > 1) {
                ce = hipEventRecord(h->ev_fork, restore.s);
                u32 b0 = 0;
                for (u32 g = 0; g < ng && ce == hipSuccess; g++) {
                    const u32 nb = run_group_size(b, ng, g);
                    ce = hipStreamWaitEvent(h->side_streams[g], h->ev_fork, 0);
                    h->stream = h->side_streams[g];
                    enqueue_run_bins(h, b0, nb, (u64 *)d_results);
                    if (ce == hipSuccess) ce = hipEventRecord(h->ev_join[g], h->side_streams[g]);
                    if (ce == hipSuccess) ce = hipStreamWaitEvent(restore.s, h->ev_join[g], 0);
                    b0 += nb;
                }
                h->stream = restore.s;
            } else {
                enqueue_run_bins(h, 0, b, (u64 *)d_results);
            }
            const hipError_t ee = hipStreamEndCapture(restore.s, &graph);
            if (ce != hipSuccess || ee != hipSuccess || !graph) {
                if (graph) (void)hipGraphDestroy(graph);
                return fail(PIEHIP_EHIP, std::string("run: graph capture failed: ") + hipGetErrorString(ce != hipSuccess ? ce : ee));
            }
            const hipError_t ie = hipGraphInstantiate(&h->gexec, graph, nullptr, nullptr, 0);
            (void)hipGraphDestroy(graph);
            if (ie != hipSuccess) {
                h->gexec = nullptr;
                return fail(PIEHIP_EHIP, std::string("run: hipGraphInstantiate: ") + hipGetErrorString(ie));
            }
            h->g_idx = h->query[0].idx, h->g_minus = h->query[0].minus, h->g_res = d_results, h->g_ng = ng;
        }
        join_pending(h);
        HIPCHK(hipGraphLaunch(h->gexec, h->stream));
        mark_dirty(h);
        return PIEHIP_OK;
    }
    if (ng > 1) {
        struct Restore {
            piehip_ctx *h;
            hipStream_t s;
            ~Restore()
            {
                h->stream = s;
                h->wait_before_results = nullptr;
            }
        } restore{h, h->stream};
        HIPCHK(hipEventRecord(h->ev_fork, restore.s));
        u32 b0 = 0;
        for (u32 g = 0; g < ng; g++) {
            const u32 nb = run_group_size(b, ng, g);
            if (h->inputs_dirty) HIPCHK(hipStreamWaitEvent(h->side_streams[g], h->ev_fork, 0));
            h->stream = h->side_streams[g];
            h->wait_before_results = h->inputs_dirty ? nullptr : h->ev_fork;
            if (h->host_results && g > 0) HIPCHK(hipStreamWaitEvent(h->side_streams[g], h->ev_chain, 0));
            if (h->host_results && g + 1 < ng) {
                if (!h->ev_chain) HIPCHK(hipEventCreateWithFlags(&h->ev_chain, hipEventDisableTiming));
                h->chain_armed = true;
            }
            enqueue_run_bins(h, b0, nb, (u64 *)d_results);
            if (h->chain_armed) {
                h->chain_armed = false;
                HIPCHK(hipEventRecord(h->ev_chain, h->side_streams[g]));
            }
            if (h->host_results) HIPCHK(download_rows(h, (const u64 *)d_results, b0, nb));
            HIPCHK(hipEventRecord(h->ev_join[g], h->side_streams[g]));
            b0 += nb;
        }
        h->pending_join = true;
        h->inputs_dirty = false;
    } else {
        join_pending(h);
        enqueue_run_bins(h, 0, b, (u64 *)d_results);
        if (h->host_results) HIPCHK(download_rows(h, (const u64 *)d_results, 0, b));
        mark_dirty(h);
    }
    HIPCHK(hipGetLastError());
    return PIEHIP_OK;
}

int piehip_run(piehip_handle h)
{
    if (!h) return fail(PIEHIP_EINVAL, "null handle");
    if (!h->d_out) return fail(PIEHIP_ESTATE, "run: database not loaded");
    return piehip_run_into(h, h->d_out);
}

int piehip_join(piehip_handle h)
{
    NEED_RO(h);
    return PIEHIP_OK;
}

int piehip_set_graph(piehip_handle h, int on)
{
    NEED_RO(h);
    if (on && h->res_limbs < h->hp.L)
        return fail(PIEHIP_ESTATE, "set_graph: the captured graph hands out full results (piehip_set_result_limbs is below L)");
    h->use_graph = on != 0;
    if (!on) drop_graph(h);
    return PIEHIP_OK;
}

int piehip_set_run_streams(piehip_handle h, uint32_t n)
{
    NEED_RO(h);
    h->run_streams = n;
    return PIEHIP_OK;
}

}
```

Measured before the change: 74320.

## Compute d0/d1 Q-limb tensor terms in evaluation form inside relin MAC

For relinearised multiplies, the inverse NTT after the fused tensor now skips the Q-limbs of components d0 and d1, and scale-round computes only the P-part contribution for them. The relin MAC kernel adds the missing own-limb term by multiplying the forward-NTT inputs directly in evaluation form and scaling by t/P mod q. This removes inverse transforms and scale-round work on the Q limbs, but adds extra reads of the expanded inputs and more arithmetic in the relin kernel. It also relies on the linearity of the scale-round split being exact under lazy reductions.

Result: faster. 78110, median of 6 (+5.1%).

```diff
diff --git a/nested_hashing_psi_amd/csrc/kernels.hpp b/nested_hashing_psi_amd/csrc/kernels.hpp
--- a/nested_hashing_psi_amd/csrc/kernels.hpp
+++ b/nested_hashing_psi_amd/csrc/kernels.hpp
@@ -47,6 +47,7 @@
     bool xq_reuse = false;
     bool x_direct = false;
     bool fused_tensor = false;
+    bool d01_eval_q = false;
     bool digits_with_d01 = false;
     bool digit_lift_lane = false;
     bool digit_lift_std = false;
@@ -87,7 +88,10 @@
 #ifndef PIEHIP_FUSE_TENSOR
 #define PIEHIP_FUSE_TENSOR 1
 #endif
-void launch_ntt16_tensor(const NttPlan &pl, const u64 *e, u64 *d, u32 nb, u32 M, hipStream_t st);
+#ifndef PIEHIP_D01_EVAL_Q
+#define PIEHIP_D01_EVAL_Q 1
+#endif
+void launch_ntt16_tensor(const NttPlan &pl, const u64 *e, u64 *d, u32 nb, u32 M, hipStream_t st, u32 eval_q_L = 0);
 void launch_ntt_digits(const NttPlan &pl, const u64 *d2, u64 *dig, u32 nb, u32 L, bool sigma, hipStream_t st);
 
 struct StageAXOut {
@@ -116,12 +120,12 @@
                         u64 *out, hipStream_t st, bool small_moduli, bool fold = false, bool skip_q = false);
 void launch_tensor(const DevConsts *dc, u32 N, u32 M, const u64 *e, u64 *d, u32 nb, hipStream_t st, bool small_moduli);
 void launch_scale_round(const DevConsts *dc, u32 N, u32 L, const u64 *d, u32 nb, u64 *out01, size_t stride01, u64 *out2,
-                        size_t stride2, hipStream_t st, bool small_moduli, bool fold = false, bool fold_comp2 = false);
+                        size_t stride2, hipStream_t st, bool small_moduli, bool fold = false, bool fold_comp2 = false, bool p_only01 = false);
 void launch_digits(const DevConsts *dc, u32 N, u32 L, const u64 *d2, size_t stride2, u32 nb, u64 *dig, hipStream_t st,
                    bool fold = false);
 void launch_relin_mac(const DevConsts *dc, u32 N, u32 L, const u64 *d01, size_t stride01, const u64 *dig, const u64 *key,
                       const u64 *mask, u64 *out, u32 nb, hipStream_t st, bool small_moduli, const u32 *out_map = nullptr, size_t key_stride = 0,
-                      u32 key_group = 1, u32 sigma_T = 0, u32 sigma_kp = 16, u32 mask_div = 1);
+                      u32 key_group = 1, u32 sigma_T = 0, u32 sigma_kp = 16, u32 mask_div = 1, const u64 *eqp = nullptr, u32 eqp_M = 0);
 void launch_bcast_mul_plain(const DevConsts *dc, u32 N, u32 L, const u64 *x, size_t xs, u32 group, const u64 *pt, size_t ps_outer,
                             size_t ps_inner, u64 *out, u32 nct, hipStream_t st);
 void launch_rot_prepare(const DevConsts *dc, u32 N, u32 L, const u64 *x, const u32 *maps, u32 map_group, bool acc, bool identity_first,
diff --git a/nested_hashing_psi_amd/csrc/kernels_ntt.hip b/nested_hashing_psi_amd/csrc/kernels_ntt.hip
--- a/nested_hashing_psi_amd/csrc/kernels_ntt.hip
+++ b/nested_hashing_psi_amd/csrc/kernels_ntt.hip
@@ -142,6 +142,7 @@
     pl.lane_kp = k16 ? 8 : 16;
     pl.xq_reuse = ntt_route(pl, true, false, pl.fold).extra();
     pl.fused_tensor = PIEHIP_FUSE_TENSOR && k16 && small_moduli;
+    pl.d01_eval_q = PIEHIP_D01_EVAL_Q && pl.fused_tensor;
     pl.digits_with_d01 = k16 && small_moduli;
     pl.x_direct = pl.xq_reuse && k16 && small_moduli;
     const NttRoute std_fwd = ntt_route(pl, false, false, false);
diff --git a/nested_hashing_psi_amd/csrc/kernels_ntt16.hip b/nested_hashing_psi_amd/csrc/kernels_ntt16.hip
--- a/nested_hashing_psi_amd/csrc/kernels_ntt16.hip
+++ b/nested_hashing_psi_amd/csrc/kernels_ntt16.hip
@@ -81,6 +81,8 @@
     a.lift_stride = 0;
     a.lift_L = 1;
     a.tsrc = nullptr;
+    a.tq_L = 0;
+    a.tq_first = 0;
     if (dg && !inverse) {
         a.lift_first = a.nitems;
         a.nitems += (dg->nb * dg->L * dg->L) << s0;
@@ -96,9 +98,9 @@
         launch_ntt16_t<13>(a, inverse, lift, pl.transform_cus(), st);
 }
 
-void launch_ntt16_tensor(const NttPlan &pl, const u64 *e, u64 *d, u32 nb, u32 M, hipStream_t st)
+void launch_ntt16_tensor(const NttPlan &pl, const u64 *e, u64 *d, u32 nb, u32 M, hipStream_t st, u32 eval_q_L)
 {
-    assert(pl.fused_tensor);
+    assert(pl.fused_tensor && (!eval_q_L || (pl.d01_eval_q && eval_q_L < M)));
     const bool folded = pl.fold;
     const u32 s0 = folded ? 1u : 0u;
     ntt16::Args a = {};
@@ -108,7 +110,9 @@
     a.dc = pl.dc;
     a.N = pl.N;
     a.s0 = s0;
-    a.nitems = (nb * 3 * M) << s0;
+    a.tq_L = eval_q_L;
+    a.tq_first = (nb * 3 * (M - eval_q_L)) << s0;
+    a.nitems = a.tq_first + ((nb * eval_q_L) << s0);
     a.mod_base = 0;
     a.mod_count = M;
     a.flags = folded ? ntt16::F_FOLDED : 0;
diff --git a/nested_hashing_psi_amd/csrc/kernels_pie.hip b/nested_hashing_psi_amd/csrc/kernels_pie.hip
--- a/nested_hashing_psi_amd/csrc/kernels_pie.hip
+++ b/nested_hashing_psi_amd/csrc/kernels_pie.hip
@@ -1,4 +1,6 @@
 #include <stdlib.h>
+
+#include <cassert>
 
 #include <algorithm>
 
@@ -966,7 +968,7 @@
         hipLaunchKernelGGL(tensor_kernel<false>, grid, dim3(TPB), 0, st, dc, N, M, e, d);
 }
 
-template <u32 L, bool MAD, int NP, bool PRE = false>
+template <u32 L, bool MAD, int NP, bool PRE = false, bool PONLY = false>
 __device__ __forceinline__ void scale_round_core(const DevConsts *dc, const u64 (&d)[NP][2 * L + 1], u64 (&out)[NP][L], bool lz = false)
 {
     constexpr u32 Lp = L + 1;
@@ -1007,14 +1009,18 @@
                 ColAcc a = {itot[p].lo, 0, 0};
 #pragma unroll
                 for (u32 j = 0; j < Lp; j++) colacc_mac(a, split30(yp[p][j]), split30(col[j]));
-                if (PRE)
+                if (PONLY)
+                    ;
+                else if (PRE)
                     a.c0 += d[p][k];
                 else
                     colacc_mac(a, split30(d[p][k]), split30(tp));
                 out[p][k] = (L <= 5 && lz) ? colacc_reduce123_lazy(a, qk, nq) : colacc_reduce<(L > 5)>(a, qk, nq);
             } else {
                 U128 acc = dot128<Lp, MAD>(yp[p], col);
-                if (PRE)
+                if (PONLY)
+                    ;
+                else if (PRE)
                     add128(acc, U128{d[p][k], 0});
                 else
                     mac128(acc, d[p][k], tp);
@@ -1025,22 +1031,16 @@
     }
 }
 
-template <bool FOLD, u32 L, bool MAD>
-__global__ void __launch_bounds__(TPB) scale_round_kernel(const DevConsts *__restrict__ dc, u32 N, const u64 *__restrict__ d,
-                                                          u64 *__restrict__ out01, size_t stride01,
-                                                          u64 *__restrict__ out2, size_t stride2, u32 fold_comp2)
-{
-    const u32 n = blockIdx.x * TPB + threadIdx.x;
+template <bool FOLD, u32 L, bool MAD, bool PONLY>
+__device__ __forceinline__ void scale_round_comp(const DevConsts *__restrict__ dc, u32 N, u32 n, const u64 *__restrict__ pin,
+                                                 u64 *__restrict__ pout, bool fold_out, bool lz)
+{
     const u32 H = N / 2;
-    if (n >= (FOLD ? H : N)) return;
-    const u32 comp = blockIdx.y, bin = blockIdx.z;
     constexpr u32 M = 2 * L + 1;
-    const u64 *pin = d + ((size_t)(bin * 3 + comp) * M) * N + n;
-    u64 *pout = comp < 2 ? out01 + (size_t)bin * stride01 + (size_t)comp * L * N + n : out2 + (size_t)bin * stride2 + n;
     constexpr int NP = FOLD ? 2 : 1;
     u64 x[NP][M], y[NP][L];
 #pragma unroll
-    for (u32 a = 0; a < M; a++) {
+    for (u32 a = PONLY ? L : 0; a < M; a++) {
         if (FOLD) {
             PIE_ITER_FENCE();
             const DcC c = dc_iter(dc);
@@ -1054,13 +1054,13 @@
             x[0][a] = pin[(size_t)a * N];
         }
     }
-    scale_round_core<L, MAD, NP, FOLD>(dc, x, y, FOLD && MAD && comp < 2 && !fold_comp2);
+    scale_round_core<L, MAD, NP, FOLD, PONLY>(dc, x, y, lz);
 #pragma unroll
     for (u32 k = 0; k < L; k++) {
         PIE_ITER_FENCE();
         if (FOLD) {
             u64 y0 = y[0][k], y1 = y[NP - 1][k];
-            if (comp < 2 || fold_comp2) fold_store(dc, k, y[0][k], y[NP - 1][k], y0, y1);
+            if (fold_out) fold_store(dc, k, y[0][k], y[NP - 1][k], y0, y1);
             pout[(size_t)k * N] = y0;
             pout[(size_t)k * N + H] = y1;
         } else {
@@ -1068,24 +1068,42 @@
         }
     }
 }
+template <bool FOLD, u32 L, bool MAD, bool P01 = false>
+__global__ void __launch_bounds__(TPB) scale_round_kernel(const DevConsts *__restrict__ dc, u32 N, const u64 *__restrict__ d,
+                                                          u64 *__restrict__ out01, size_t stride01,
+                                                          u64 *__restrict__ out2, size_t stride2, u32 fold_comp2)
+{
+    const u32 n = blockIdx.x * TPB + threadIdx.x;
+    if (n >= (FOLD ? N / 2 : N)) return;
+    const u32 comp = blockIdx.y, bin = blockIdx.z;
+    constexpr u32 M = 2 * L + 1;
+    const u64 *pin = d + ((size_t)(bin * 3 + comp) * M) * N + n;
+    u64 *pout = comp < 2 ? out01 + (size_t)bin * stride01 + (size_t)comp * L * N + n : out2 + (size_t)bin * stride2 + n;
+    const bool lz = FOLD && MAD && comp < 2 && !fold_comp2;
+    if (P01 && comp < 2)
+        scale_round_comp<FOLD, L, MAD, true>(dc, N, n, pin, pout, true, lz);
+    else
+        scale_round_comp<FOLD, L, MAD, false>(dc, N, n, pin, pout, comp < 2 || fold_comp2, lz);
+}
 void launch_scale_round(const DevConsts *dc, u32 N, u32 L, const u64 *d, u32 nb, u64 *out01, size_t stride01, u64 *out2,
-                        size_t stride2, hipStream_t st, bool small_moduli, bool fold, bool fold_comp2)
-{
+                        size_t stride2, hipStream_t st, bool small_moduli, bool fold, bool fold_comp2, bool p_only01)
+{
+    assert(!p_only01 || (small_moduli && !fold_comp2));
     dim3 grid(((fold ? N / 2 : N) + TPB - 1) / TPB, 3, nb);
-#define SRL(L_)                                                                                                              \
-    case L_:                                                                                                                 \
-        if (fold && small_moduli)                                                                                          \
-            hipLaunchKernelGGL((scale_round_kernel<true, L_, true>), grid, dim3(TPB), 0, st, dc, N, d, out01, stride01, out2, stride2, \
-                               fold_comp2 ? 1u : 0u);                                                                        \
-        else if (fold)                                                                                                       \
-            hipLaunchKernelGGL((scale_round_kernel<true, L_, false>), grid, dim3(TPB), 0, st, dc, N, d, out01, stride01, out2, stride2, \
-                               fold_comp2 ? 1u : 0u);                                                                        \
-        else if (small_moduli)                                                                                             \
-            hipLaunchKernelGGL((scale_round_kernel<false, L_, true>), grid, dim3(TPB), 0, st, dc, N, d, out01, stride01, out2, stride2, 0u); \
-        else                                                                                                                 \
-            hipLaunchKernelGGL((scale_round_kernel<false, L_, false>), grid, dim3(TPB), 0, st, dc, N, d, out01, stride01, out2, stride2, 0u); \
+#define SRK(F_, L_, M_, P_) \
+    hipLaunchKernelGGL((scale_round_kernel<F_, L_, M_, P_>), grid, dim3(TPB), 0, st, dc, N, d, out01, stride01, out2, stride2, (fold_comp2 && F_) ? 1u : 0u)
+#define SRL(L_)                                                                        \
+    case L_:                                                                           \
+        if (p_only01) {                                                                \
+            if (fold) SRK(true, L_, true, true); else SRK(false, L_, true, true);      \
+        } else if (small_moduli) {                                                     \
+            if (fold) SRK(true, L_, true, false); else SRK(false, L_, true, false);    \
+        } else {                                                                       \
+            if (fold) SRK(true, L_, false, false); else SRK(false, L_, false, false);  \
+        }                                                                              \
         break;
     switch (L) { SRL(1) SRL(2) SRL(3) SRL(4) SRL(5) SRL(6) SRL(7) }
+#undef SRK
 #undef SRL
 }
 
@@ -1125,14 +1143,16 @@
         hipLaunchKernelGGL(digits_kernel<false>, grid, dim3(TPB), 0, st, dc, N, L, d2, stride2, dig);
 }
 
-template <bool MAD, int KP, int RPT = 1>
+template <bool MAD, int KP, int RPT = 1, bool EQ = false>
 __global__ void __launch_bounds__(TPB) relin_mac_kernel(const DevConsts *__restrict__ dc, u32 N, u32 L, const u64 *__restrict__ d01,
                                                         size_t stride01, const u64 *__restrict__ dig,
                                                         const u64 *__restrict__ key0, const u64 *__restrict__ mask,
                                                         u64 *__restrict__ out, const u32 *__restrict__ out_map,
-                                                        size_t key_stride, u32 key_group, u32 T, u32 mask_div, u32 nb)
+                                                        size_t key_stride, u32 key_group, u32 T, u32 mask_div, u32 nb,
+                                                        const u64 *__restrict__ eqp, u32 eqp_M)
 {
     static_assert(RPT == 1 || MAD, "two rows per thread: the column-accumulator path");
+    static_assert(!EQ || MAD, "the own-limb term: the column-accumulator path");
     constexpr bool TILE = KP > 0;
     constexpr u32 TT = TILE ? TPB / (KP ? KP : 1) : 1;
     __shared__ u64x2 s_tile[TILE ? 2 * RPT : 1][TILE ? TPB : 1];
@@ -1184,6 +1204,32 @@
             }
         }
         const u64 nq = 0 - m.q;
+        if (EQ) {
+            const u64 n2q = neg_u(2 * m.q), n4q = neg_u(4 * m.q);
+            const u64 tp = dc->tPinv_modq[j], tpsh = dc->tPinv_modq_sh[j];
+            const size_t MN = (size_t)eqp_M * N;
+#pragma unroll
+            for (int r = 0; r < RPT; r++) {
+                if (r && !has[r]) continue;
+                const u64 *pe = eqp + (size_t)rows[r] * 4 * MN + (size_t)j * N + n;
+                const u64x2 va0 = *reinterpret_cast<const u64x2 *>(pe), va1 = *reinterpret_cast<const u64x2 *>(pe + MN),
+                            vb0 = *reinterpret_cast<const u64x2 *>(pe + 2 * MN), vb1 = *reinterpret_cast<const u64x2 *>(pe + 3 * MN);
+#pragma unroll
+                for (int k = 0; k < 2; k++) {
+                    const Split30 sa0 = split30(csub_u(csub_u(k ? va0.y : va0.x, n4q), n2q)), sa1 = split30(csub_u(csub_u(k ? va1.y : va1.x, n4q), n2q));
+                    const Split30 sb0 = split30(csub_u(csub_u(k ? vb0.y : vb0.x, n4q), n2q)), sb1 = split30(csub_u(csub_u(k ? vb1.y : vb1.x, n4q), n2q));
+                    ColAcc t = {0, 0, 0};
+                    colacc_mac(t, sa0, sb0);
+                    const u64 v0 = shoup63_lazy(colacc_reduce123_lazy(t, m, nq), tp, tpsh, nq);
+                    t = ColAcc{0, 0, 0};
+                    colacc_mac(t, sa0, sb1);
+                    colacc_mac(t, sa1, sb0);
+                    const u64 v1 = shoup63_lazy(colacc_reduce123_lazy(t, m, nq), tp, tpsh, nq);
+                    a[r][0][k].c0 += v0 & 0x3FFFFFFFull, a[r][0][k].c1 += v0 >> 30;
+                    a[r][1][k].c0 += v1 & 0x3FFFFFFFull, a[r][1][k].c1 += v1 >> 30;
+                }
+            }
+        }
 #pragma unroll
         for (int r = 0; r < RPT; r++) {
             if (r && !has[r]) continue;
@@ -1259,8 +1305,9 @@
 }
 void launch_relin_mac(const DevConsts *dc, u32 N, u32 L, const u64 *d01, size_t stride01, const u64 *dig, const u64 *key,
                       const u64 *mask, u64 *out, u32 nb, hipStream_t st, bool small_moduli, const u32 *out_map, size_t key_stride,
-                      u32 key_group, u32 sigma_T, u32 sigma_kp, u32 mask_div)
-{
+                      u32 key_group, u32 sigma_T, u32 sigma_kp, u32 mask_div, const u64 *eqp, u32 eqp_M)
+{
+    assert(!eqp || (small_moduli && eqp_M >= L));
     if (!key_group) key_group = 1;
     if (!mask_div) mask_div = 1;
     const bool tile = out_map && (sigma_kp == 16 || sigma_kp == 8) && sigma_T >= TPB / sigma_kp && sigma_T % (TPB / sigma_kp) == 0 &&
@@ -1269,17 +1316,25 @@
     const bool two = small_moduli && nb >= 2 * key_group;
     const u32 zrows = two ? ((nb + 2 * key_group - 1) / (2 * key_group)) * key_group : nb;
     dim3 grid((N / 2 + TPB - 1) / TPB, L, zrows);
-#define RM(M_, K_, R_)                                                                                                              \
-    hipLaunchKernelGGL((relin_mac_kernel<M_, K_, R_>), grid, dim3(TPB), 0, st, dc, N, L, d01, stride01, dig, key, mask, out, out_map, \
-                       key_stride, key_group, sigma_T, mask_div, nb)
-    if (two) {
+#define RME(M_, K_, R_, E_)                                                                                                            \
+    hipLaunchKernelGGL((relin_mac_kernel<M_, K_, R_, E_>), grid, dim3(TPB), 0, st, dc, N, L, d01, stride01, dig, key, mask, out, out_map, \
+                       key_stride, key_group, sigma_T, mask_div, nb, eqp, eqp_M)
+#define RM(M_, K_, R_) RME(M_, K_, R_, false)
+#define RQ(K_, R_) RME(true, K_, R_, true)
+    if (eqp && two) {
+        if (kp == 16) RQ(16, 2); else if (kp == 8) RQ(8, 2); else RQ(0, 2);
+    } else if (eqp) {
+        if (kp == 16) RQ(16, 1); else if (kp == 8) RQ(8, 1); else RQ(0, 1);
+    } else if (two) {
         if (kp == 16) RM(true, 16, 2); else if (kp == 8) RM(true, 8, 2); else RM(true, 0, 2);
     } else if (small_moduli) {
         if (kp == 16) RM(true, 16, 1); else if (kp == 8) RM(true, 8, 1); else RM(true, 0, 1);
     } else {
         if (kp == 16) RM(false, 16, 1); else if (kp == 8) RM(false, 8, 1); else RM(false, 0, 1);
     }
+#undef RQ
 #undef RM
+#undef RME
 }
 
 __global__ void host_flag_kernel(volatile u64 *flag, u64 value)
diff --git a/nested_hashing_psi_amd/csrc/ntt16_kernel.h b/nested_hashing_psi_amd/csrc/ntt16_kernel.h
--- a/nested_hashing_psi_amd/csrc/ntt16_kernel.h
+++ b/nested_hashing_psi_amd/csrc/ntt16_kernel.h
@@ -191,6 +191,7 @@
     size_t lift_stride;
     u32 lift_first, lift_L;
     const u64 *tsrc;
+    u32 tq_L, tq_first;
 };
 enum : u32 {
     F_STD_IN = 1,
@@ -394,18 +395,26 @@
         }
         u32 t_d = 0, t_row = 0, t_blk = 0, t_limb = 0;
         if (TENSOR) {
-            const u32 M_ = a.mod_count;
+            const u32 M_ = a.mod_count, TL = a.tq_L, TM = M_ - TL;
+            if (item < a.tq_first) {
 #if NTT16_TENSOR_XCD
-            u32 il = item;
-            const u32 within = il % 24;
-            if (il - within + 24 <= a.nitems) il = il - within + (within & 7) * 3 + (within >> 3);
-            const u32 u = il / 3, lm = u >> a.s0;
-            t_d = il % 3, t_blk = u & ((1u << a.s0) - 1), t_row = lm / M_;
-            t_limb = (t_row * 3 + t_d) * M_ + lm % M_;
+                u32 il = item;
+                const u32 within = il % 24;
+                if (il - within + 24 <= a.tq_first) il = il - within + (within & 7) * 3 + (within >> 3);
+                const u32 u = il / 3, lm = u >> a.s0;
+                t_d = il % 3, t_blk = u & ((1u << a.s0) - 1), t_row = lm / TM;
+                t_limb = (t_row * 3 + t_d) * M_ + TL + lm % TM;
 #else
-            t_limb = item >> a.s0, t_blk = item & ((1u << a.s0) - 1);
-            t_row = t_limb / (3 * M_), t_d = (t_limb / M_) % 3;
-#endif
+                const u32 lm = item >> a.s0;
+                t_blk = item & ((1u << a.s0) - 1);
+                t_row = lm / (3 * TM), t_d = (lm / TM) % 3;
+                t_limb = (t_row * 3 + t_d) * M_ + TL + lm % TM;
+#endif
+            } else {
+                const u32 v = item - a.tq_first, lm = v >> a.s0;
+                t_d = 2, t_blk = v & ((1u << a.s0) - 1), t_row = lm / TL;
+                t_limb = (t_row * 3 + 2) * M_ + lm % TL;
+            }
             t_d = __builtin_amdgcn_readfirstlane(t_d), t_row = __builtin_amdgcn_readfirstlane(t_row);
             t_blk = __builtin_amdgcn_readfirstlane(t_blk), t_limb = __builtin_amdgcn_readfirstlane(t_limb);
         }
diff --git a/nested_hashing_psi_amd/csrc/params.cpp b/nested_hashing_psi_amd/csrc/params.cpp
--- a/nested_hashing_psi_amd/csrc/params.cpp
+++ b/nested_hashing_psi_amd/csrc/params.cpp
@@ -195,6 +195,7 @@
         dc.P_modq[i] = prod_mod(P, Lp, -1, qi);
         dc.P_modq_sh[i] = shoup(dc.P_modq[i], qi);
         dc.tPinv_modq[i] = mm(t % qi, invmod(dc.P_modq[i], qi), qi);
+        dc.tPinv_modq_sh[i] = shoup(dc.tPinv_modq[i], qi);
         for (u32 j = 0; j < Lp; j++) {
             const u64 pj = P[j];
             dc.qhat_modp[i][j] = prod_mod(Q, L, (int)i, pj);
diff --git a/nested_hashing_psi_amd/csrc/params.hpp b/nested_hashing_psi_amd/csrc/params.hpp
--- a/nested_hashing_psi_amd/csrc/params.hpp
+++ b/nested_hashing_psi_amd/csrc/params.hpp
@@ -26,6 +26,7 @@
     u64 qp_hat_inv[16];
     u64 qp_hat_inv_sh[16];
     u64 tPinv_modq[8];
+    u64 tPinv_modq_sh[8];
     u64 tQ_modp[8];
     u64 tQ_modp_sh[8];
     u64 tQF_modq[8][8];
diff --git a/nested_hashing_psi_amd/csrc/piehip_ctx.hpp b/nested_hashing_psi_amd/csrc/piehip_ctx.hpp
--- a/nested_hashing_psi_amd/csrc/piehip_ctx.hpp
+++ b/nested_hashing_psi_amd/csrc/piehip_ctx.hpp
@@ -232,7 +232,8 @@
 void ntt(piehip_ctx *h, u64 *data, u32 nlimbs, u32 mod_base, u32 mod_count, bool inv, bool sigma = false, bool fold = false,
          const NttExtra *ex = nullptr);
 void enqueue_keyswitch(piehip_ctx *h, MulWs &w, u32 nb, const u64 *key, const u64 *mask, u64 *out, bool lane = false,
-                       size_t key_stride = 0, u32 key_group = 1, bool out_is_result = false, bool digits_ready = false);
+                       size_t key_stride = 0, u32 key_group = 1, bool out_is_result = false, bool digits_ready = false,
+                       bool d01_eval_q = false);
 void enqueue_mul(piehip_ctx *h, MulWs &w, const u64 *x, size_t sx, const u64 *y, size_t sy, u32 nb, bool relin,
                  const u64 *mask, u64 *out, bool xq_ready = false, bool out_is_result = false);
 int encode_on_device(piehip_ctx *h, const int64_t *d_slots, u32 npt, u32 B, u64 *d_out);
diff --git a/nested_hashing_psi_amd/csrc/piehip_run.cpp b/nested_hashing_psi_amd/csrc/piehip_run.cpp
--- a/nested_hashing_psi_amd/csrc/piehip_run.cpp
+++ b/nested_hashing_psi_amd/csrc/piehip_run.cpp
@@ -1,3 +1,5 @@
+#include <cassert>
+
 #include "piehip_ctx.hpp"
 
 using namespace piehip;
@@ -11,7 +13,7 @@
 }
 
 void enqueue_keyswitch(piehip_ctx *h, MulWs &w, u32 nb, const u64 *key, const u64 *mask, u64 *out, bool lane, size_t key_stride,
-                       u32 key_group, bool out_is_result, bool digits_ready)
+                       u32 key_group, bool out_is_result, bool digits_ready, bool d01_eval_q)
 {
     const NttPlan &pl = h->plan;
     const u32 N = h->hp.N, L = h->hp.L;
@@ -35,9 +37,12 @@
             h->chain_armed = false;
             (void)hipEventRecord(h->ev_chain, h->stream);
         }
-        ProfScope ps(h, PIEHIP_K_RELIN, W * (nb * ((double)L * L + 2 * L + 2 * L + (mask ? L : 0)) + 2.0 * L * L));
+        assert(!d01_eval_q || (pl.d01_eval_q && lane));
+        ProfScope ps(h, PIEHIP_K_RELIN,
+                     W * (nb * ((double)L * L + 2 * L + 2 * L + (mask ? L : 0) + (d01_eval_q ? 4 * L : 0)) + 2.0 * L * L));
         launch_relin_mac(h->d_dc, N, L, w.d01, 2 * LN, w.dig, key, mask, out, nb, h->stream, pl.small_moduli,
-                         lane ? h->d_sigma_inv : nullptr, key_stride, key_group, lane ? pl.lane_T : 0, pl.lane_kp, mask ? h->mask_div : 1);
+                         lane ? h->d_sigma_inv : nullptr, key_stride, key_group, lane ? pl.lane_T : 0, pl.lane_kp, mask ? h->mask_div : 1,
+                         d01_eval_q ? w.eqp : nullptr, h->hp.M);
     }
 }
 
@@ -73,9 +78,10 @@
         }
         ntt(h, w.eqp, nb * (xq_ready ? 4 * M - 2 * L : 4 * M), 0, M, false, true, true, &ex);
     }
+    const bool eval_q = relin && pl.d01_eval_q;
     if (pl.fused_tensor) {
         ProfScope ps(h, PIEHIP_K_TENSOR_NTT_INV, W * nb * 7.0 * M);
-        launch_ntt16_tensor(pl, w.eqp, w.dqp, nb, M, h->stream);
+        launch_ntt16_tensor(pl, w.eqp, w.dqp, nb, M, h->stream, eval_q ? L : 0);
     } else {
         {
             ProfScope ps(h, PIEHIP_K_TENSOR, W * nb * 7.0 * M);
@@ -86,7 +92,7 @@
     if (relin) {
         {
             ProfScope ps(h, PIEHIP_K_SCALE, W * nb * (3.0 * M + 3.0 * L));
-            launch_scale_round(h->d_dc, N, L, w.dqp, nb, w.d01, 2 * LN, w.d2c, LN, h->stream, pl.small_moduli, pl.fold, false);
+            launch_scale_round(h->d_dc, N, L, w.dqp, nb, w.d01, 2 * LN, w.d2c, LN, h->stream, pl.small_moduli, pl.fold, false, eval_q);
         }
         NttExtra ex;
         ex.lazy_out = true;
@@ -98,7 +104,7 @@
             ntt(h, w.d01, nb * 2 * L, 0, L, false, true, true, &ex);
         }
         const RunKey k = run_key(h);
-        enqueue_keyswitch(h, w, nb, k.key, mask, out, true, k.stride, k.group, out_is_result, pl.digits_with_d01);
+        enqueue_keyswitch(h, w, nb, k.key, mask, out, true, k.stride, k.group, out_is_result, pl.digits_with_d01, eval_q);
     } else {
         {
             ProfScope ps(h, PIEHIP_K_SCALE, W * nb * (3.0 * M + 3.0 * L));
```
